# clovaai/assembled-cnn

Measured on NVIDIA H100. Metric: images/sec Assemble-ResNet-50 224^2 bf16 train step, higher is better.
Workload: dtype bf16

## Files before the change

assembled_cnn_b200/csrc/gemm.cu:

```cuda
#include <stdlib.h>

#include <algorithm>

#include "common.h"
#include "ptx.cuh"

namespace acnn {

static void input_pitches(const acnn_conv_geom& g, int64_t* pix, int64_t* row, int64_t* img) {
  *pix = g.x_pix_stride > 0 ? g.x_pix_stride : g.Cin;
  *row = g.x_row_pitch > 0 ? g.x_row_pitch : (int64_t)g.W * *pix;
  *img = g.x_img_pitch > 0 ? g.x_img_pitch : (int64_t)g.H * *row;
}

static bool is_plain(const acnn_conv_geom& g) {
  return g.kh == 1 && g.kw == 1 && g.stride == 1 && g.pad_h_lo == 0 && g.pad_w_lo == 0 &&
         g.pad_h_hi == 0 && g.pad_w_hi == 0 && g.x_pix_stride <= 0 && g.x_row_pitch <= 0 &&
         g.x_img_pitch <= 0;
}

static int make_map_im2col(CUtensorMap* m, const void* base, const acnn_conv_geom& g, int cw,
                           int pixels) {
  int64_t pix, row, img;
  input_pitches(g, &pix, &row, &img);
  cuuint64_t dims[4] = {(cuuint64_t)g.Cin, (cuuint64_t)g.W, (cuuint64_t)g.H, (cuuint64_t)g.B};
  cuuint64_t strides[3] = {(cuuint64_t)pix * 2, (cuuint64_t)row * 2, (cuuint64_t)img * 2};
  int lower[2] = {-g.pad_w_lo, -g.pad_h_lo};
  int upper[2] = {g.pad_w_hi - (g.kw - 1), g.pad_h_hi - (g.kh - 1)};
  cuuint32_t estr[4] = {1, (cuuint32_t)g.stride, (cuuint32_t)g.stride, 1};
  CUresult r = g_encode_im2col(m, CU_TENSOR_MAP_DATA_TYPE_BFLOAT16, 4, const_cast<void*>(base),
                               dims, strides, lower, upper, (cuuint32_t)cw, (cuuint32_t)pixels,
                               estr, CU_TENSOR_MAP_INTERLEAVE_NONE, swizzle_enum(cw * 2),
                               CU_TENSOR_MAP_L2_PROMOTION_L2_128B,
                               CU_TENSOR_MAP_FLOAT_OOB_FILL_NONE);
  if (r != CUDA_SUCCESS) {
    set_error("cuTensorMapEncodeIm2col failed (%d): B=%d H=%d W=%d C=%d k=%dx%d s=%d cw=%d px=%d "
              "pitches=%lld/%lld/%lld", (int)r, g.B, g.H, g.W, g.Cin, g.kh, g.kw, g.stride, cw,
              pixels, (long long)pix, (long long)row, (long long)img);
    return ACNN_ERR_CUDA;
  }
  if (g_driver_version <= 13010 && (int64_t)g.B * img * 2 < 131072) {
    reinterpret_cast<uint64_t*>(m)[1] &= ~(1ull << 21);
  }
  return ACNN_OK;
}

struct ConvGemmParams {
  int M;
  int Cout;
  int Cin;
  int Ktot;
  int kw;
  int HoWo, Wo;
  int stride, pad_h_lo, pad_w_lo;
  int b_sw_bytes;
  int stages;
  int m_tiles, n_tiles;
  void* y;
  float* ch_part;
  const float* bias;
  int has_add, has_mask;
  int out_f32;
};

constexpr int kBM = 128;
constexpr int kStageK = 64;
constexpr int kThreads = 384;
constexpr int kConsumerThreads = 256;
constexpr int kConsumerWarps = 8;
constexpr int kMaxStages = 8;
constexpr int kSmemBudget = 224 * 1024;

__host__ __device__ constexpr int plane_term_a(int t) { return t == 0 ? 2 : ((t == 1 || t == 3) ? 1 : 0); }
__host__ __device__ constexpr int plane_term_b(int t) { return t == 2 ? 2 : ((t == 1 || t == 4) ? 1 : 0); }

static inline int fprop_stage_bytes(int bn, int np) { return np * (kBM * kStageK * 2 + bn * kStageK * 2); }
static inline int fprop_stages(int bn, int np, bool has_add, bool has_mask, bool out_f32) {
  const int half_n = bn > 128 ? 128 : bn;
  const int tile = kBM * half_n * 2;
  const int fixed = 1024 + (out_f32 ? 0 : tile) + (has_add ? tile : 0) + (has_mask ? tile : 0);
  int st = (kSmemBudget - fixed) / fprop_stage_bytes(bn, np);
  if (st > kMaxStages) st = kMaxStages;
  if (st < 2) st = 2;
  return st;
}

template <int BN, int NP = 1>
struct FpropCfg {
  static constexpr int kABytes = kBM * kStageK * 2;
  static constexpr int kBBytes = BN * kStageK * 2;
  static constexpr int kStageBytes = NP * (kABytes + kBBytes);
  static_assert(2 * kStageBytes + 1024 <= kSmemBudget, "two pipeline stages must fit");
  static constexpr int kHalfN = BN > 128 ? 128 : BN;
  static constexpr int kNHalf = BN / kHalfN;
  static constexpr int kSubW = kHalfN < 64 ? kHalfN : 64;
  static constexpr int kTileBytes = kBM * kHalfN * 2;
  static_assert(NP == 1 || BN <= 128, "fp32 mode: N tile <= 128 (registers)");
  static int stages_for(bool has_add, bool has_mask, bool out_f32) {
    return fprop_stages(BN, NP, has_add, has_mask, out_f32);
  }
  static int smem_bytes(int stages, bool has_add, bool has_mask, bool out_f32) {
    return 1024 + stages * kStageBytes + (out_f32 ? 0 : kTileBytes) + (has_add ? kTileBytes : 0) +
           (has_mask ? kTileBytes : 0);
  }
};

template <int kSubW>
__device__ __forceinline__ int staged_offset(int r, int c) {
  constexpr int kRowBytes = kSubW * 2;
  const int sub = c / kSubW, cb = (c % kSubW) * 2;
  const int swz = (kRowBytes == 128) ? (r & 7) : ((r >> 1) & 3);
  return sub * (kBM * kRowBytes) + r * kRowBytes + ((((cb >> 4) ^ swz)) << 4) + (cb & 15);
}

template <int BN, int CW, bool IM2COL, int NP, bool CG2>
__global__ void __launch_bounds__(kThreads, 1)
conv_gemm_kernel(const __grid_constant__ CUtensorMap tmA, const __grid_constant__ CUtensorMap tmB,
                 const __grid_constant__ CUtensorMap tmC, const __grid_constant__ CUtensorMap tmAdd,
                 const __grid_constant__ CUtensorMap tmMask, const __grid_constant__ CUtensorMap tmA1,
                 const __grid_constant__ CUtensorMap tmA2, const __grid_constant__ CUtensorMap tmB1,
                 const __grid_constant__ CUtensorMap tmB2, const ConvGemmParams p) {
  using Cfg = FpropCfg<BN, NP>;
  constexpr int kChunks = kStageK / CW;
  constexpr int kChunkBytes = kBM * CW * 2;
  constexpr int kKSteps = CW / 16;
  constexpr int kHalfN = Cfg::kHalfN;
  constexpr int kNHalf = Cfg::kNHalf;
  constexpr int kSubW = Cfg::kSubW;
  constexpr int kSubBytes = kBM * kSubW * 2;
  constexpr int kNSub = kHalfN / kSubW;

  extern __shared__ uint8_t smem_raw[];
  __shared__ uint64_t full_bar[kMaxStages];
  __shared__ uint64_t empty_bar[kMaxStages];
  __shared__ uint64_t aux_bar;

  uint8_t* smem = reinterpret_cast<uint8_t*>((reinterpret_cast<uintptr_t>(smem_raw) + 1023) &
                                             ~static_cast<uintptr_t>(1023));
  const int kStages = p.stages;
  uint8_t* s_out = smem + kStages * Cfg::kStageBytes;
  uint8_t* s_add = s_out + (p.out_f32 ? 0 : Cfg::kTileBytes);
  uint8_t* s_mask = s_add + (p.has_add ? Cfg::kTileBytes : 0);

  const int warp = threadIdx.x >> 5;
  const int lane = threadIdx.x & 31;
  const int num_kb = (p.Ktot + kStageK - 1) / kStageK;
  constexpr int kTileM = (CG2 ? 2 : 1) * kBM;
  const uint32_t cta_rank = CG2 ? cluster_ctarank() : 0u;
  const int unit = CG2 ? static_cast<int>(blockIdx.x >> 1) : static_cast<int>(blockIdx.x);
  const int units = CG2 ? static_cast<int>(gridDim.x >> 1) : static_cast<int>(gridDim.x);
  const int n_tile = unit % p.n_tiles;
  const int m_first = unit / p.n_tiles;
  const int m_step = units / p.n_tiles;
  const int n0 = n_tile * BN;
  const int my_tiles = m_first < p.m_tiles ? (p.m_tiles - m_first + m_step - 1) / m_step : 0;
  const int m_rank_off = static_cast<int>(cta_rank) * kBM;

  if (warp == 0 && lane == 0) {
    tma_prefetch_desc(&tmA);
    tma_prefetch_desc(&tmB);
    if (NP == 3) {
      tma_prefetch_desc(&tmA1);
      tma_prefetch_desc(&tmA2);
      tma_prefetch_desc(&tmB1);
      tma_prefetch_desc(&tmB2);
    }
    if (!p.out_f32) tma_prefetch_desc(&tmC);
    if (p.has_add) tma_prefetch_desc(&tmAdd);
    if (p.has_mask) tma_prefetch_desc(&tmMask);
    for (int s = 0; s < kStages; ++s) {
      mbar_init(&full_bar[s], 1);
      mbar_init(&empty_bar[s], kConsumerWarps * (CG2 ? 2 : 1));
    }
    mbar_init(&aux_bar, 1);
    fence_barrier_init();
  }
  if (CG2) cluster_sync();
  else __syncthreads();
  pdl_entry();

  const uint32_t smem_a0 = smem_u32(smem);
  const uint32_t full0 = smem_u32(full_bar), empty0 = smem_u32(empty_bar);
  const int tail_chunks = kChunks == 1 ? 1 : ((p.Ktot - (num_kb - 1) * kStageK + CW - 1) / CW);

  if (warp == 0) {
    uint32_t stage = 0, phase = 0;
    const uint32_t b_bytes = BN * (p.b_sw_bytes < 128 ? p.b_sw_bytes : 128);
    const uint32_t full_bytes = NP * (kChunks * kChunkBytes + b_bytes);
    const uint32_t tail_bytes = NP * (tail_chunks * kChunkBytes + b_bytes);
    const int Cin = p.Cin, fkw = p.kw;
    for (int it = 0; it < my_tiles; ++it) {
      const int m0 = (m_first + it * m_step) * kTileM + m_rank_off;
      int img = 0, h0 = 0, w0 = 0;
      if (IM2COL) {
        img = m0 / p.HoWo;
        const int rem = m0 - img * p.HoWo;
        const int po = rem / p.Wo;
        const int qo = rem - po * p.Wo;
        h0 = po * p.stride - p.pad_h_lo;
        w0 = qo * p.stride - p.pad_w_lo;
      }
      int tr = 0, ts = 0, tc = 0, k0 = 0;
      for (int kb = 0; kb < num_kb; ++kb) {
        const bool last = kb == num_kb - 1;
        const int nch = (kChunks > 1 && last) ? tail_chunks : kChunks;
        mbar_wait_a(empty0 + stage * 8, phase ^ 1);
        const bool leader = elect_one();
        const uint32_t fb = full0 + stage * 8;
        const uint32_t sa = smem_a0 + stage * Cfg::kStageBytes;
        if (leader) {
          mbar_expect_tx_a(fb, (kChunks > 1 && last) ? tail_bytes : full_bytes);
          if (CG2) {
            const int half = BN / 2;
            tma_load_2d_multicast(sa + NP * Cfg::kABytes + cta_rank * half * (b_bytes / BN), &tmB,
                                  fb, k0, n0 + static_cast<int>(cta_rank) * half, (uint16_t)3);
          } else {
#pragma unroll
            for (int pl = 0; pl < NP; ++pl)
              tma_load_2d_a(sa + NP * Cfg::kABytes + pl * Cfg::kBBytes,
                            pl == 0 ? &tmB : (pl == 1 ? &tmB1 : &tmB2), fb, k0, n0);
          }
        }
#pragma unroll
        for (int j = 0; j < kChunks; ++j) {
          if (j < nch) {
            if (leader) {
#pragma unroll
              for (int pl = 0; pl < NP; ++pl) {
                const CUtensorMap* mA = pl == 0 ? &tmA : (pl == 1 ? &tmA1 : &tmA2);
                const uint32_t dst = sa + pl * Cfg::kABytes + j * kChunkBytes;
                if (IM2COL)
                  tma_load_im2col_4d_a(dst, mA, fb, tc, w0, h0, img, (uint16_t)ts, (uint16_t)tr);
                else
                  tma_load_2d_a(dst, mA, fb, k0 + j * CW, m0);
              }
            }
            tc += CW;
            if (tc >= Cin) {
              tc = 0;
              if (++ts == fkw) { ts = 0; ++tr; }
            }
          }
        }
        __syncwarp();
        k0 += kStageK;
        if (++stage == static_cast<uint32_t>(kStages)) { stage = 0; phase ^= 1; }
      }
    }
  } else if (warp >= 4) {
    const int cg = (warp >> 2) - 1;
    const int ct = static_cast<int>(threadIdx.x) - 128;
    const bool leader = ct == 0;
    const bool stats = p.ch_part != nullptr;
    const bool has_aux = p.has_add || p.has_mask;
    const int r0 = cg * 64 + (warp & 3) * 16 + (lane >> 2);
    const int cq = (lane & 3) * 2;
    const uint64_t a_desc0 = make_smem_desc(smem_a0 + cg * 64 * CW * 2, 16, 8 * CW * 2,
                                            swizzle_layout_type(CW * 2));
    const uint64_t b_desc0 = make_smem_desc(smem_a0 + NP * Cfg::kABytes, 16, 8 * p.b_sw_bytes,
                                            swizzle_layout_type(p.b_sw_bytes));
    float acc[BN / 2];
    float acc2[NP == 3 ? BN / 2 : 1];
    constexpr int kNChunk = kHalfN / 8;
    constexpr int kStatThreads = (BN == 32) ? 128 : kConsumerThreads;
    constexpr int kNRg = kStatThreads / kNChunk;
    const bool st_on = ct < kStatThreads;
    const int st_chunk = ct % kNChunk, st_rg = ct / kNChunk;
    float acc_s[kNHalf][8], acc_q[kNHalf][8];
#pragma unroll
    for (int hf = 0; hf < kNHalf; ++hf)
#pragma unroll
      for (int e = 0; e < 8; ++e) acc_s[hf][e] = acc_q[hf][e] = 0.f;
    uint32_t aux_n = 0;
    auto issue_aux = [&](int am0, int anh) {
      mbar_expect_tx(&aux_bar, (p.has_add ? Cfg::kTileBytes : 0) +
                                   (p.has_mask ? Cfg::kTileBytes : 0));
#pragma unroll
      for (int sub = 0; sub < kNSub; ++sub) {
        if (p.has_add)
          tma_load_2d(s_add + sub * kSubBytes, &tmAdd, &aux_bar, anh + sub * kSubW, am0);
        if (p.has_mask)
          tma_load_2d(s_mask + sub * kSubBytes, &tmMask, &aux_bar, anh + sub * kSubW, am0);
      }
    };
    if (leader && has_aux && my_tiles > 0) issue_aux(m_first * kTileM + m_rank_off, n0);
    const uint32_t empty_peer = CG2 ? mapa_shared(empty0, cta_rank ^ 1u) : 0u;
    auto release = [&](int st) {
      if (CG2) {
        mbar_arrive_cluster(mapa_shared(empty0, cta_rank) + st * 8);
        mbar_arrive_cluster(empty_peer + st * 8);
      } else {
        mbar_arrive(&empty_bar[st]);
      }
    };

    uint32_t stage = 0, phase = 0;
    for (int it = 0; it < my_tiles; ++it) {
      const int m0 = (m_first + it * m_step) * kTileM + m_rank_off;
      int prev = -1;
      for (int kb = 0; kb < num_kb; ++kb) {
        const bool last = kb == num_kb - 1;
        const int nch = (kChunks > 1 && last) ? tail_chunks : kChunks;
        mbar_wait_a(full0 + stage * 8, phase);
        wgmma_fence_operand(acc);
        if (NP == 3) wgmma_fence_operand(acc2);
        wgmma_fence();
        const uint64_t da0 = a_desc0 + ((stage * Cfg::kStageBytes) >> 4);
        const uint64_t db0 = b_desc0 + ((stage * Cfg::kStageBytes) >> 4);
#pragma unroll
        for (int j = 0; j < kChunks; ++j) {
          if (j < nch) {
#pragma unroll
            for (int ks = 0; ks < kKSteps; ++ks) {
#pragma unroll
              for (int t = 0; t < (NP == 3 ? 6 : 1); ++t) {
                const int pa = NP == 3 ? plane_term_a(t) : 0;
                const int pb = NP == 3 ? plane_term_b(t) : 0;
                const bool small = NP == 3 && t < 5;
                const uint64_t da = da0 + ((pa * Cfg::kABytes + j * kChunkBytes + ks * 32) >> 4);
                const uint64_t db = db0 + ((pb * Cfg::kBBytes + (j * kKSteps + ks) * 32) >> 4);
                const uint32_t accum = (j | ks | (small ? t : 0)) ? 1u : static_cast<uint32_t>(kb != 0);
                if constexpr (NP == 3) {
                  if (small) Wgmma<BN>::template mma<0, 0>(acc2, da, db, accum);
                  else Wgmma<BN>::template mma<0, 0>(acc, da, db, accum);
                } else {
                  Wgmma<BN>::template mma<0, 0>(acc, da, db, accum);
                }
              }
            }
          }
        }
        wgmma_commit();
        wgmma_fence_operand(acc);
        if (NP == 3) wgmma_fence_operand(acc2);
        wgmma_wait<1>();
        __syncwarp();
        if (prev >= 0 && lane == 0) release(prev);
        prev = static_cast<int>(stage);
        if (++stage == static_cast<uint32_t>(kStages)) { stage = 0; phase ^= 1; }
      }
      wgmma_wait<0>();
      wgmma_fence_operand(acc);
      if (NP == 3) {
        wgmma_fence_operand(acc2);
#pragma unroll
        for (int i = 0; i < BN / 2; ++i) acc[i] += acc2[i];
      }
      __syncwarp();
      if (lane == 0) release(prev);

#pragma unroll
      for (int hf = 0; hf < kNHalf; ++hf) {
        const int nh = n0 + hf * kHalfN;
        if (leader && !p.out_f32) tma_store_wait_read();
        named_bar_sync(1, kConsumerThreads);
        if (has_aux) {
          mbar_wait(&aux_bar, aux_n & 1);
          ++aux_n;
        }
#pragma unroll
        for (int jj = 0; jj < kHalfN / 8; ++jj) {
          const int j = hf * (kHalfN / 8) + jj;
          const int c = jj * 8 + cq;
          float b0 = 0.f, b1 = 0.f;
          if (p.bias) {
            b0 = __ldg(p.bias + nh + c);
            b1 = __ldg(p.bias + nh + c + 1);
          }
#pragma unroll
          for (int h = 0; h < 2; ++h) {
            const int r = r0 + h * 8;
            float v0 = acc[j * 4 + h * 2] + b0, v1 = acc[j * 4 + h * 2 + 1] + b1;
            const int off = staged_offset<kSubW>(r, c);
            if (p.has_add) bf16x2_add(v0, v1, *reinterpret_cast<const uint32_t*>(s_add + off));
            if (p.out_f32) {
              if (p.has_mask) {
                const uint32_t k2 = bf16x2_gt0_mask(*reinterpret_cast<const uint32_t*>(s_mask + off));
                if (!(k2 & 0xffffu)) v0 = 0.f;
                if (!(k2 >> 16)) v1 = 0.f;
              }
              if (m0 + r < p.M)
                *reinterpret_cast<float2*>(reinterpret_cast<float*>(p.y) +
                                           static_cast<size_t>(m0 + r) * p.Cout + nh + c) =
                    make_float2(v0, v1);
            } else {
              uint32_t pk = pack_bf16x2(v0, v1);
              if (p.has_mask) pk &= bf16x2_gt0_mask(*reinterpret_cast<const uint32_t*>(s_mask + off));
              *reinterpret_cast<uint32_t*>(s_out + off) = pk;
            }
          }
        }
        if (!p.out_f32) fence_proxy_async();
        named_bar_sync(1, kConsumerThreads);
        if (leader) {
          if (!p.out_f32) {
#pragma unroll
            for (int sub = 0; sub < kNSub; ++sub)
              tma_store_2d(&tmC, s_out + sub * kSubBytes, nh + sub * kSubW, m0);
            tma_store_commit();
          }
          if (has_aux) {
            if (hf + 1 < kNHalf) issue_aux(m0, nh + kHalfN);
            else if (it + 1 < my_tiles) issue_aux((m_first + (it + 1) * m_step) * kTileM + m_rank_off, n0);
          }
        }
        if (stats && st_on) {
          constexpr int kRowBytes = kSubW * 2;
          const int sub = st_chunk / (kSubW / 8), jj = st_chunk % (kSubW / 8);
#pragma unroll 4
          for (int i = 0; i < kBM / kNRg; ++i) {
            const int rr = st_rg + i * kNRg;
            const int sw = (kRowBytes == 128) ? (rr & 7) : ((rr >> 1) & 3);
            const uint4 u = *reinterpret_cast<const uint4*>(s_out + sub * kSubBytes +
                                                            rr * kRowBytes + ((jj ^ sw) << 4));
            const uint32_t w4[4] = {u.x, u.y, u.z, u.w};
#pragma unroll
            for (int e = 0; e < 4; ++e)
              bf16x2_sum_sq(acc_s[hf][2 * e], acc_q[hf][2 * e], acc_s[hf][2 * e + 1],
                            acc_q[hf][2 * e + 1], w4[e]);
          }
        }
      }
    }
    if (leader && !p.out_f32) tma_store_wait_all();
    if (stats && my_tiles > 0) {
      float* red_sum = reinterpret_cast<float*>(s_out);
      float* red_sq = red_sum + kNRg * BN;
      static_assert(2 * kNRg * BN * 4 <= Cfg::kTileBytes, "staging buffer too small for stats");
      named_bar_sync(1, kConsumerThreads);
      if (st_on) {
#pragma unroll
        for (int hf = 0; hf < kNHalf; ++hf)
#pragma unroll
          for (int e = 0; e < 8; ++e) {
            red_sum[st_rg * BN + hf * kHalfN + st_chunk * 8 + e] = acc_s[hf][e];
            red_sq[st_rg * BN + hf * kHalfN + st_chunk * 8 + e] = acc_q[hf][e];
          }
      }
      named_bar_sync(1, kConsumerThreads);
      for (int col = ct; col < BN; col += kConsumerThreads) {
        float ss = 0.f, qq = 0.f;
        for (int g2 = 0; g2 < kNRg; ++g2) {
          ss += red_sum[g2 * BN + col];
          qq += red_sq[g2 * BN + col];
        }
        float* row = p.ch_part +
                     static_cast<size_t>(CG2 ? m_first * 2 + static_cast<int>(cta_rank) : m_first) * 2 *
                         p.Cout;
        row[n0 + col] = ss;
        row[p.Cout + n0 + col] = qq;
      }
    }
  }
  if (CG2) cluster_sync();
}

constexpr int kHaloH = 18, kHaloW = 10, kPatchH = 16, kPatchW = 8;
constexpr int kHaloMaxB = 32;

struct HaloParams {
  int H, W, B;
  int Cin, Cout;
  int n_tiles, ph, pw;
  int m_tiles;
  int a_stages, b_slots, stationary;
  float* ch_part;
  int has_add, has_mask;
};

template <int BN, int CW>
struct HaloCfg {
  static constexpr int kRowB = CW * 2;
  static constexpr int kABytes = kHaloH * kHaloW * kRowB;
  static constexpr int kAStage = (kABytes + 1023) / 1024 * 1024;
  static constexpr int kBTile = BN * kRowB;
  static constexpr int kSubW = BN < 64 ? BN : 64;
  static constexpr int kTileBytes = kBM * BN * 2;
  static_assert(BN <= 128 && kBTile % 512 == 0, "halo kernel: N tile <= 128");
};

struct PatchIter {
  int img, row, col;
  int d_img, d_row, d_col;
  int ph, pw;
  __device__ __forceinline__ PatchIter(int first, int step, int ph_, int pw_) : ph(ph_), pw(pw_) {
    const int tpi = ph * pw;
    img = first / tpi;
    int rem = first - img * tpi;
    row = rem / pw;
    col = rem - row * pw;
    d_img = step / tpi;
    rem = step - d_img * tpi;
    d_row = rem / pw;
    d_col = rem - d_row * pw;
  }
  __device__ __forceinline__ void next() {
    col += d_col;
    if (col >= pw) { col -= pw; ++row; }
    row += d_row;
    if (row >= ph) { row -= ph; ++img; }
    img += d_img;
  }
};

template <int BN, int CW>
__global__ void __launch_bounds__(kThreads, 1)
conv_halo_kernel(const __grid_constant__ CUtensorMap tmA, const __grid_constant__ CUtensorMap tmB,
                 const __grid_constant__ CUtensorMap tmC, const __grid_constant__ CUtensorMap tmAdd,
                 const __grid_constant__ CUtensorMap tmMask, const HaloParams p) {
  using Cfg = HaloCfg<BN, CW>;
  constexpr int kRowB = Cfg::kRowB;
  constexpr int kKSteps = CW / 16;
  constexpr uint32_t kLayout = swizzle_layout_type(kRowB);
  constexpr int kSubW = Cfg::kSubW;
  constexpr int kSubBytes = kBM * kSubW * 2;
  constexpr int kNSub = BN / kSubW;

  extern __shared__ uint8_t smem_raw[];
  __shared__ uint64_t a_full[4], a_empty[4];
  __shared__ uint64_t b_full[kHaloMaxB], b_empty[kHaloMaxB];
  __shared__ uint64_t aux_bar;

  uint8_t* smem = reinterpret_cast<uint8_t*>((reinterpret_cast<uintptr_t>(smem_raw) + 1023) &
                                             ~static_cast<uintptr_t>(1023));
  const int AS = p.a_stages, NB = p.b_slots;
  uint8_t* s_out = smem + AS * Cfg::kAStage + NB * Cfg::kBTile;
  uint8_t* s_add = s_out + Cfg::kTileBytes;
  uint8_t* s_mask = s_add + (p.has_add ? Cfg::kTileBytes : 0);

  const int warp = threadIdx.x >> 5;
  const int lane = threadIdx.x & 31;
  const int nchunks = p.Cin / CW;
  const int n_tile = blockIdx.x % p.n_tiles;
  const int m_first = blockIdx.x / p.n_tiles;
  const int m_step = gridDim.x / p.n_tiles;
  const int n0 = n_tile * BN;
  const int my_tiles = m_first < p.m_tiles ? (p.m_tiles - m_first + m_step - 1) / m_step : 0;
  const int tpi = p.ph * p.pw;

  if (warp == 0 && lane == 0) {
    tma_prefetch_desc(&tmA);
    tma_prefetch_desc(&tmB);
    tma_prefetch_desc(&tmC);
    if (p.has_add) tma_prefetch_desc(&tmAdd);
    if (p.has_mask) tma_prefetch_desc(&tmMask);
    for (int s = 0; s < AS; ++s) {
      mbar_init(&a_full[s], 1);
      mbar_init(&a_empty[s], kConsumerWarps);
    }
    for (int s = 0; s < NB; ++s) {
      mbar_init(&b_full[s], 1);
      mbar_init(&b_empty[s], kConsumerWarps);
    }
    mbar_init(&aux_bar, 1);
    fence_barrier_init();
  }
  __syncthreads();
  pdl_entry();
  const uint32_t a_base = smem_u32(smem), b_base = a_base + AS * Cfg::kAStage;
  const uint32_t afull0 = smem_u32(a_full), bfull0 = smem_u32(b_full);

  if (warp == 0) {
    const uint32_t aempty0 = smem_u32(a_empty), bempty0 = smem_u32(b_empty);
    uint32_t sa = 0, a_ph = 0, sb = 0, b_ph = 0;
    if (p.stationary && my_tiles > 0) {
      if (elect_one()) {
        mbar_expect_tx_a(bfull0, static_cast<uint32_t>(nchunks) * 9 * Cfg::kBTile);
        for (int kc = 0; kc < nchunks; ++kc)
          for (int t = 0; t < 9; ++t)
            tma_load_2d_a(b_base + (kc * 9 + t) * Cfg::kBTile, &tmB, bfull0, t * p.Cin + kc * CW, n0);
      }
      __syncwarp();
    }
    for (int it = 0; it < my_tiles; ++it) {
      const int tile = m_first + it * m_step;
      const int img = tile / tpi;
      const int rem = tile - img * tpi;
      const int h0 = (rem / p.pw) * kPatchH, w0 = (rem % p.pw) * kPatchW;
      for (int kc = 0; kc < nchunks; ++kc) {
        mbar_wait_a(aempty0 + sa * 8, a_ph ^ 1);
        if (elect_one()) {
          mbar_expect_tx_a(afull0 + sa * 8, Cfg::kABytes);
          tma_load_4d_tile_a(a_base + sa * Cfg::kAStage, &tmA, afull0 + sa * 8, kc * CW, w0 - 1,
                             h0 - 1, img);
        }
        __syncwarp();
        if (++sa == static_cast<uint32_t>(AS)) { sa = 0; a_ph ^= 1; }
        if (!p.stationary) {
          for (int t = 0; t < 9; ++t) {
            mbar_wait_a(bempty0 + sb * 8, b_ph ^ 1);
            if (elect_one()) {
              mbar_expect_tx_a(bfull0 + sb * 8, Cfg::kBTile);
              tma_load_2d_a(b_base + sb * Cfg::kBTile, &tmB, bfull0 + sb * 8, t * p.Cin + kc * CW,
                            n0);
            }
            __syncwarp();
            if (++sb == static_cast<uint32_t>(NB)) { sb = 0; b_ph ^= 1; }
          }
        }
      }
    }
  } else if (warp >= 4) {
    const int cg = (warp >> 2) - 1;
    const int ct = static_cast<int>(threadIdx.x) - 128;
    const bool leader = ct == 0;
    const bool stats = p.ch_part != nullptr;
    const bool has_aux = p.has_add || p.has_mask;
    const int r0 = cg * 64 + (warp & 3) * 16 + (lane >> 2);
    const int cq = (lane & 3) * 2;
    const uint64_t a_desc0 = make_smem_desc(a_base + cg * 8 * kHaloW * kRowB, 16, kHaloW * kRowB, kLayout);
    const uint64_t b_desc0 = make_smem_desc(b_base, 16, 8 * kRowB, kLayout);
    float acc[BN / 2];
    constexpr int kNChunk = BN / 8;
    constexpr int kStatThreads = (BN == 32) ? 128 : kConsumerThreads;
    constexpr int kNRg = kStatThreads / kNChunk;
    const bool st_on = ct < kStatThreads;
    const int st_chunk = ct % kNChunk, st_rg = ct / kNChunk;
    float acc_s[8], acc_q[8];
#pragma unroll
    for (int e = 0; e < 8; ++e) acc_s[e] = acc_q[e] = 0.f;
    uint32_t aux_n = 0;
    auto issue_aux = [&](int img, int h0, int w0) {
      mbar_expect_tx(&aux_bar, (p.has_add ? Cfg::kTileBytes : 0) + (p.has_mask ? Cfg::kTileBytes : 0));
#pragma unroll
      for (int sub = 0; sub < kNSub; ++sub) {
        if (p.has_add)
          tma_load_4d_tile_a(smem_u32(s_add + sub * kSubBytes), &tmAdd, smem_u32(&aux_bar),
                             n0 + sub * kSubW, w0, h0, img);
        if (p.has_mask)
          tma_load_4d_tile_a(smem_u32(s_mask + sub * kSubBytes), &tmMask, smem_u32(&aux_bar),
                             n0 + sub * kSubW, w0, h0, img);
      }
    };
    int pend_a = -1, pend_b = -1;
    auto release_pending = [&]() {
      __syncwarp();
      if (lane == 0) {
        if (pend_a >= 0) mbar_arrive(&a_empty[pend_a]);
        if (pend_b >= 0) mbar_arrive(&b_empty[pend_b]);
      }
      pend_a = pend_b = -1;
    };
    PatchIter pi(m_first, m_step, p.ph, p.pw);
    if (leader && has_aux && my_tiles > 0) issue_aux(pi.img, pi.row * kPatchH, pi.col * kPatchW);
    if (p.stationary && my_tiles > 0) mbar_wait_a(bfull0, 0);
    uint32_t sa = 0, a_ph = 0, sb = 0, b_ph = 0;
    for (int it = 0; it < my_tiles; ++it) {
      const int img = pi.img, h0 = pi.row * kPatchH, w0 = pi.col * kPatchW;
      pi.next();
      for (int kc = 0; kc < nchunks; ++kc) {
        mbar_wait_a(afull0 + sa * 8, a_ph);
        const uint64_t a_st = a_desc0 + ((sa * Cfg::kAStage) >> 4);
        if (p.stationary) {
          wgmma_fence_operand(acc);
          wgmma_fence();
          const uint64_t b_st = b_desc0 + ((static_cast<uint32_t>(kc) * 9 * Cfg::kBTile) >> 4);
#pragma unroll
          for (int t = 0; t < 9; ++t)
#pragma unroll
            for (int ks = 0; ks < kKSteps; ++ks)
              Wgmma<BN>::template mma<0, 0>(
                  acc, a_st + ((((t / 3) * kHaloW + (t % 3)) * kRowB + ks * 32) >> 4),
                  b_st + ((t * Cfg::kBTile + ks * 32) >> 4), (t | ks) ? 1u : static_cast<uint32_t>(kc != 0));
          wgmma_commit();
          wgmma_fence_operand(acc);
          wgmma_wait<1>();
          release_pending();
          pend_a = static_cast<int>(sa);
        } else {
#pragma unroll 1
          for (int t = 0; t < 9; ++t) {
            mbar_wait_a(bfull0 + sb * 8, b_ph);
            wgmma_fence_operand(acc);
            wgmma_fence();
            const uint64_t a_tap = a_st + ((((t / 3) * kHaloW + (t % 3)) * kRowB) >> 4);
            const uint64_t b_tap = b_desc0 + ((sb * Cfg::kBTile) >> 4);
#pragma unroll
            for (int ks = 0; ks < kKSteps; ++ks)
              Wgmma<BN>::template mma<0, 0>(acc, a_tap + ((ks * 32) >> 4), b_tap + ((ks * 32) >> 4),
                                            (kc | t | ks) ? 1u : 0u);
            wgmma_commit();
            wgmma_fence_operand(acc);
            wgmma_wait<1>();
            release_pending();
            pend_b = static_cast<int>(sb);
            if (t == 8) pend_a = static_cast<int>(sa);
            if (++sb == static_cast<uint32_t>(NB)) { sb = 0; b_ph ^= 1; }
          }
        }
        if (++sa == static_cast<uint32_t>(AS)) { sa = 0; a_ph ^= 1; }
      }
      wgmma_wait<0>();
      wgmma_fence_operand(acc);
      release_pending();

      if (leader) tma_store_wait_read();
      named_bar_sync(1, kConsumerThreads);
      if (has_aux) {
        mbar_wait(&aux_bar, aux_n & 1);
        ++aux_n;
      }
#pragma unroll
      for (int j = 0; j < BN / 8; ++j) {
        const int c = j * 8 + cq;
#pragma unroll
        for (int h = 0; h < 2; ++h) {
          const int r = r0 + h * 8;
          float v0 = acc[j * 4 + h * 2], v1 = acc[j * 4 + h * 2 + 1];
          const int off = staged_offset<kSubW>(r, c);
          if (p.has_add) bf16x2_add(v0, v1, *reinterpret_cast<const uint32_t*>(s_add + off));
          uint32_t pk = pack_bf16x2(v0, v1);
          if (p.has_mask) pk &= bf16x2_gt0_mask(*reinterpret_cast<const uint32_t*>(s_mask + off));
          *reinterpret_cast<uint32_t*>(s_out + off) = pk;
        }
      }
      fence_proxy_async();
      named_bar_sync(1, kConsumerThreads);
      if (leader) {
#pragma unroll
        for (int sub = 0; sub < kNSub; ++sub)
          tma_store_4d(&tmC, s_out + sub * kSubBytes, n0 + sub * kSubW, w0, h0, img);
        tma_store_commit();
        if (has_aux && it + 1 < my_tiles) issue_aux(pi.img, pi.row * kPatchH, pi.col * kPatchW);
      }
      if (stats && st_on) {
        constexpr int kRowBytes = kSubW * 2;
        const int sub = st_chunk / (kSubW / 8), jj = st_chunk % (kSubW / 8);
#pragma unroll 4
        for (int rr = st_rg; rr < kBM; rr += kNRg) {
          if (h0 + (rr >> 3) >= p.H || w0 + (rr & 7) >= p.W) continue;
          const int sw = (kRowBytes == 128) ? (rr & 7) : ((rr >> 1) & 3);
          const uint4 u = *reinterpret_cast<const uint4*>(s_out + sub * kSubBytes + rr * kRowBytes +
                                                          ((jj ^ sw) << 4));
          const uint32_t w4[4] = {u.x, u.y, u.z, u.w};
#pragma unroll
          for (int e = 0; e < 4; ++e)
            bf16x2_sum_sq(acc_s[2 * e], acc_q[2 * e], acc_s[2 * e + 1], acc_q[2 * e + 1], w4[e]);
        }
      }
    }
    if (leader) tma_store_wait_all();
    if (stats && my_tiles > 0) {
      float* red_sum = reinterpret_cast<float*>(s_out);
      float* red_sq = red_sum + kNRg * BN;
      static_assert(2 * kNRg * BN * 4 <= Cfg::kTileBytes, "staging buffer too small for stats");
      named_bar_sync(1, kConsumerThreads);
      if (st_on) {
#pragma unroll
        for (int e = 0; e < 8; ++e) {
          red_sum[st_rg * BN + st_chunk * 8 + e] = acc_s[e];
          red_sq[st_rg * BN + st_chunk * 8 + e] = acc_q[e];
        }
      }
      named_bar_sync(1, kConsumerThreads);
      for (int col = ct; col < BN; col += kConsumerThreads) {
        float ss = 0.f, qq = 0.f;
        for (int g2 = 0; g2 < kNRg; ++g2) {
          ss += red_sum[g2 * BN + col];
          qq += red_sq[g2 * BN + col];
        }
        float* row = p.ch_part + static_cast<size_t>(m_first) * 2 * p.Cout;
        row[n0 + col] = ss;
        row[p.Cout + n0 + col] = qq;
      }
    }
  }
}

struct WgradParams {
  int P;
  int Cout;
  int Cin;
  int Ktot;
  int kw;
  int HoWo, Wo;
  int stride, pad_h_lo, pad_w_lo;
  int pix;
  int stages_total;
  int stages_per_split;
  int splits;
  float* dw;
  float* part;
};

constexpr int kWgPix = 64;

template <int BN, int NP = 1, int PIX = kWgPix>
struct WgradCfg {
  static constexpr int kABytes = PIX * 128 * 2;
  static constexpr int kBBytes = PIX * BN * 2;
  static constexpr int kStageBytes = NP * (kABytes + kBBytes);
  static constexpr int kStagesFit = (kSmemBudget - 1024) / kStageBytes;
  static constexpr int kStages =
      PIX != kWgPix ? (kStagesFit > 4 ? 4 : kStagesFit)
      : NP == 3 ? (kStagesFit > 3 ? 3 : kStagesFit)
              : ((BN >= 256) ? 4 : ((BN == 128) ? 3 : 4));
  static constexpr int kSmemBytes = kStages * kStageBytes + 1024;
  static_assert((NP == 1 || BN <= 128) && kStages >= (NP == 3 ? 2 : 3), "wgrad tile does not fit");
};

template <int BN, int CW, int CWB, bool IM2COL, int NP, int PIX>
__global__ void __launch_bounds__(kThreads, 1)
wgrad_gemm_kernel(const __grid_constant__ CUtensorMap tmX, const __grid_constant__ CUtensorMap tmDY,
                  const __grid_constant__ CUtensorMap tmX1, const __grid_constant__ CUtensorMap tmX2,
                  const __grid_constant__ CUtensorMap tmDY1,
                  const __grid_constant__ CUtensorMap tmDY2, const WgradParams p) {
  using Cfg = WgradCfg<BN, NP, PIX>;
  constexpr int kStages = Cfg::kStages;
  constexpr int kAChunks = 128 / CW;
  constexpr int kAChunkBytes = PIX * CW * 2;
  constexpr int kBChunkBytes = PIX * CWB * 2;

  extern __shared__ uint8_t smem_raw[];
  __shared__ uint64_t full_bar[kStages];
  __shared__ uint64_t empty_bar[kStages];

  uint8_t* smem = reinterpret_cast<uint8_t*>((reinterpret_cast<uintptr_t>(smem_raw) + 1023) &
                                             ~static_cast<uintptr_t>(1023));
  const int warp = threadIdx.x >> 5;
  const int lane = threadIdx.x & 31;
  const int m0 = blockIdx.x * 128;
  const int co0 = blockIdx.y * BN;
  const int ks_begin = blockIdx.z * p.stages_per_split;
  int ks_end = ks_begin + p.stages_per_split;
  if (ks_end > p.stages_total) ks_end = p.stages_total;
  const int num_ks = ks_end - ks_begin;

  int a_chunks = 0;
#pragma unroll
  for (int j = 0; j < kAChunks; ++j) a_chunks += (m0 + j * CW < p.Ktot) ? 1 : 0;
  const int b_chunks = (p.Cout - co0 < BN ? p.Cout - co0 : BN) / CWB;

  if (warp == 0 && lane == 0) {
    tma_prefetch_desc(&tmDY);
    tma_prefetch_desc(&tmX);
    for (int s = 0; s < kStages; ++s) {
      mbar_init(&full_bar[s], 1);
      mbar_init(&empty_bar[s], kConsumerWarps);
    }
    fence_barrier_init();
  }
  __syncthreads();
  pdl_entry();

  if (warp == 0) {
    int stage = 0;
    uint32_t phase = 0;
    int ch_r[kAChunks], ch_s[kAChunks], ch_c[kAChunks];
#pragma unroll
    for (int j = 0; j < kAChunks; ++j) {
      const int n = m0 + j * CW;
      const int tap = n / p.Cin;
      ch_c[j] = n - tap * p.Cin;
      ch_r[j] = tap / p.kw;
      ch_s[j] = tap - ch_r[j] * p.kw;
    }
    for (int it = 0; it < num_ks; ++it) {
      const int p0 = (ks_begin + it) * PIX;
      mbar_wait(&empty_bar[stage], phase ^ 1);
      if (elect_one()) {
        uint8_t* sa = smem + stage * Cfg::kStageBytes;
        uint8_t* sb = sa + NP * Cfg::kABytes;
        mbar_expect_tx(&full_bar[stage], NP * (a_chunks * kAChunkBytes + b_chunks * kBChunkBytes));
        int img = 0, h0 = 0, w0 = 0;
        if (IM2COL) {
          img = p0 / p.HoWo;
          const int rem = p0 - img * p.HoWo;
          const int po = rem / p.Wo;
          const int qo = rem - po * p.Wo;
          h0 = po * p.stride - p.pad_h_lo;
          w0 = qo * p.stride - p.pad_w_lo;
        }
#pragma unroll
        for (int pl = 0; pl < NP; ++pl) {
          const CUtensorMap* mX = pl == 0 ? &tmX : (pl == 1 ? &tmX1 : &tmX2);
          const CUtensorMap* mDY = pl == 0 ? &tmDY : (pl == 1 ? &tmDY1 : &tmDY2);
#pragma unroll
          for (int j = 0; j < kAChunks; ++j) {
            if (j < a_chunks) {
              uint8_t* dst = sa + pl * Cfg::kABytes + j * kAChunkBytes;
              if (IM2COL) {
                tma_load_im2col_4d(dst, mX, &full_bar[stage], ch_c[j], w0, h0, img,
                                   (uint16_t)ch_s[j], (uint16_t)ch_r[j]);
              } else {
                tma_load_2d(dst, mX, &full_bar[stage], ch_c[j], p0);
              }
            }
          }
          for (int i = 0; i < b_chunks; ++i)
            tma_load_2d(sb + pl * Cfg::kBBytes + i * kBChunkBytes, mDY, &full_bar[stage],
                        co0 + i * CWB, p0);
        }
      }
      __syncwarp();
      if (++stage == kStages) { stage = 0; phase ^= 1; }
    }
  } else if (warp >= 4) {
    const int cg = (warp >> 2) - 1;
    const uint32_t sbase = smem_u32(smem);
    const uint64_t a_desc0 = make_smem_desc(sbase + (cg * 64 / CW) * kAChunkBytes, kAChunkBytes,
                                            8 * CW * 2, swizzle_layout_type(CW * 2));
    const uint64_t b_desc0 = make_smem_desc(sbase + NP * Cfg::kABytes, kBChunkBytes, 8 * CWB * 2,
                                            swizzle_layout_type(CWB * 2));
    float acc[BN / 2];
    float acc2[NP == 3 ? BN / 2 : 1];
    int stage = 0, prev = -1;
    uint32_t phase = 0;
    for (int it = 0; it < num_ks; ++it) {
      mbar_wait(&full_bar[stage], phase);
      wgmma_fence_operand(acc);
      if (NP == 3) wgmma_fence_operand(acc2);
      wgmma_fence();
      const uint64_t da0 = a_desc0 + static_cast<uint64_t>(stage * (Cfg::kStageBytes >> 4));
      const uint64_t db0 = b_desc0 + static_cast<uint64_t>(stage * (Cfg::kStageBytes >> 4));
#pragma unroll
      for (int ks = 0; ks < PIX / 16; ++ks) {
#pragma unroll
        for (int t = 0; t < (NP == 3 ? 6 : 1); ++t) {
          const int pa = NP == 3 ? plane_term_a(t) : 0;
          const int pb = NP == 3 ? plane_term_b(t) : 0;
          const bool small = NP == 3 && t < 5;
          const uint64_t da = da0 + ((pa * Cfg::kABytes + ks * 16 * CW * 2) >> 4);
          const uint64_t db = db0 + ((pb * Cfg::kBBytes + ks * 16 * CWB * 2) >> 4);
          const uint32_t accum = (it | ks | (small ? t : 0)) ? 1u : 0u;
          if constexpr (NP == 3) {
            if (small) Wgmma<BN>::template mma<1, 1>(acc2, da, db, accum);
            else Wgmma<BN>::template mma<1, 1>(acc, da, db, accum);
          } else {
            Wgmma<BN>::template mma<1, 1>(acc, da, db, accum);
          }
        }
      }
      wgmma_commit();
      wgmma_fence_operand(acc);
      if (NP == 3) wgmma_fence_operand(acc2);
      wgmma_wait<1>();
      __syncwarp();
      if (prev >= 0 && lane == 0) mbar_arrive(&empty_bar[prev]);
      prev = stage;
      if (++stage == kStages) { stage = 0; phase ^= 1; }
    }
    wgmma_wait<0>();
    wgmma_fence_operand(acc);
    if (NP == 3) {
      wgmma_fence_operand(acc2);
#pragma unroll
      for (int i = 0; i < BN / 2; ++i) acc[i] += acc2[i];
    }
    const int rl = cg * 64 + (warp & 3) * 16 + (lane >> 2);
    const int rb = m0 + rl;
    const int cq = (lane & 3) * 2;
    float* part = p.part ? p.part + static_cast<size_t>(blockIdx.z) * p.Cout * p.Ktot : nullptr;
#pragma unroll
    for (int j = 0; j < BN / 8; ++j) {
#pragma unroll
      for (int h = 0; h < 2; ++h) {
        const int n = rb + h * 8;
#pragma unroll
        for (int e = 0; e < 2; ++e) {
          const int co = co0 + j * 8 + cq + e;
          if (n < p.Ktot && co < p.Cout) {
            const size_t i = static_cast<size_t>(co) * p.Ktot + n;
            if (part) part[i] = acc[j * 4 + h * 2 + e];
            else atomicAdd(p.dw + i, acc[j * 4 + h * 2 + e]);
          }
        }
      }
    }
  }
}

constexpr int kWgRedThreads = 128;
constexpr int kWgRedDepth = 16;

__global__ void __launch_bounds__(kWgRedThreads)
wgrad_reduce_kernel(const float* __restrict__ part, float* dw, int64_t n, int splits) {
  pdl_entry();
  const int64_t i = blockIdx.x * static_cast<int64_t>(kWgRedThreads) + threadIdx.x;
  if (i >= n) return;
  const float* src = part + i;
  float t = 0.f;
  int s = 0;
  for (; s + kWgRedDepth <= splits; s += kWgRedDepth) {
    float v[kWgRedDepth];
#pragma unroll
    for (int u = 0; u < kWgRedDepth; ++u) v[u] = __ldcs(src + (s + u) * n);
#pragma unroll
    for (int u = 0; u < kWgRedDepth; ++u) t += v[u];
  }
  for (; s < splits; ++s) t += __ldcs(src + s * n);
  dw[i] += t;
}

struct ConvMaps {
  CUtensorMap a[3], b[3], c, add, mask;
};

static int g_conv_out_bufs = 1;
static int g_conv_split_epi = 1;
static int g_conv_split_mt2 = 1;
static int g_conv_mtiles_mode = -1;
static int g_conv_pairs = 0;

template <int BN, int CW, bool IM2COL, int NP, bool CG2 = false>
static int launch_conv_gemm(const ConvMaps& tm, const ConvGemmParams& p, int per_n,
                            cudaStream_t stream) {
  using Cfg = FpropCfg<BN, NP>;
  static bool attr_set = false;
  auto kern = conv_gemm_kernel<BN, CW, IM2COL, NP, CG2>;
  if (!attr_set) {
    cudaError_t e = cudaFuncSetAttribute(kern, cudaFuncAttributeMaxDynamicSharedMemorySize,
                                         kSmemBudget + 2048);
    if (e != cudaSuccess) {
      set_error("cudaFuncSetAttribute(conv_gemm): %s", cudaGetErrorString(e));
      return ACNN_ERR_CUDA;
    }
    attr_set = true;
  }
  ConvGemmParams q = p;
  q.stages = Cfg::stages_for(p.has_add, p.has_mask, p.out_f32);
  q.m_tiles = ceil_div(p.M, (CG2 ? 2 : 1) * kBM);
  q.n_tiles = p.Cout / BN;
  const int smem = Cfg::smem_bytes(q.stages, p.has_add, p.has_mask, p.out_f32);
  if (CG2) {
    cudaLaunchConfig_t cfg{};
    cfg.gridDim = dim3(2 * per_n * q.n_tiles);
    cfg.blockDim = dim3(kThreads);
    cfg.dynamicSmemBytes = smem;
    cfg.stream = stream;
    cudaLaunchAttribute at[1];
    at[0].id = cudaLaunchAttributeClusterDimension;
    at[0].val.clusterDim.x = 2;
    at[0].val.clusterDim.y = 1;
    at[0].val.clusterDim.z = 1;
    cfg.attrs = at;
    cfg.numAttrs = 1;
    (void)cudaLaunchKernelEx(&cfg, kern, tm.a[0], tm.b[0], tm.c, tm.add, tm.mask, tm.a[1], tm.a[2],
                             tm.b[1], tm.b[2], q);
  } else {
    launch_k(kern, dim3(per_n * q.n_tiles), dim3(kThreads), smem, stream, tm.a[0], tm.b[0], tm.c,
             tm.add, tm.mask, tm.a[1], tm.a[2], tm.b[1], tm.b[2], q);
  }
  count_launch();
  return check_launch("conv_gemm_kernel");
}

struct ConvTiling {
  int bn;
  int per_n;
  int pair;
  int parts;
};

static ConvTiling conv_tiling(int M, int Cout, int Ktot, int cw, bool has_add, bool has_mask,
                              bool out_f32, int np) {
  (void)has_add;
  (void)has_mask;
  ConvTiling t;
  t.bn = (Cout % 128 == 0) ? 128 : ((Cout % 64 == 0) ? 64 : 32);
  const int n_tiles = Cout / t.bn;
  t.pair = (g_conv_pairs && t.bn == 128 && np == 1 && !out_f32 && cw == 64 && Ktot >= 512 &&
            (int64_t)ceil_div(M, 2 * kBM) * n_tiles >= num_sms() / 2) ? 1 : 0;
  const int m_tiles = ceil_div(M, (t.pair ? 2 : 1) * kBM);
  t.per_n = (t.pair ? num_sms() / 2 : num_sms()) / n_tiles;
  if (t.per_n < 1) t.per_n = 1;
  if (t.per_n > m_tiles) t.per_n = m_tiles;
  t.parts = t.pair ? 2 * t.per_n : t.per_n;
  return t;
}

template <int BN, int NP>
static int dispatch_conv_cw(int cw, bool im2col, const ConvMaps& tm, const ConvGemmParams& p,
                            int per_n, cudaStream_t s) {
  if (im2col) {
    if (cw == 64) return launch_conv_gemm<BN, 64, true, NP>(tm, p, per_n, s);
    if (cw == 32) return launch_conv_gemm<BN, 32, true, NP>(tm, p, per_n, s);
    return launch_conv_gemm<BN, 16, true, NP>(tm, p, per_n, s);
  }
  if (cw == 64) return launch_conv_gemm<BN, 64, false, NP>(tm, p, per_n, s);
  if (cw == 32) return launch_conv_gemm<BN, 32, false, NP>(tm, p, per_n, s);
  return launch_conv_gemm<BN, 16, false, NP>(tm, p, per_n, s);
}

template <int BN>
static int dispatch_conv_gemm(const ConvTiling& t, int np, int cw, bool im2col, const ConvMaps& tm,
                              const ConvGemmParams& p, cudaStream_t s) {
  if constexpr (BN == 128) {
    if (t.pair) {
      if (im2col) return launch_conv_gemm<128, 64, true, 1, true>(tm, p, t.per_n, s);
      return launch_conv_gemm<128, 64, false, 1, true>(tm, p, t.per_n, s);
    }
  }
  if constexpr (BN <= 128) {
    if (np == 3) return dispatch_conv_cw<BN, 3>(cw, im2col, tm, p, t.per_n, s);
  }
  return dispatch_conv_cw<BN, 1>(cw, im2col, tm, p, t.per_n, s);
}

static int chunk_width(int cin) { return cin % 64 == 0 ? 64 : (cin % 32 == 0 ? 32 : 16); }

static int out_hw(const acnn_conv_geom& g, int* Ho, int* Wo) {
  *Ho = (g.H + g.pad_h_lo + g.pad_h_hi - g.kh) / g.stride + 1;
  *Wo = (g.W + g.pad_w_lo + g.pad_w_hi - g.kw) / g.stride + 1;
  return (*Ho > 0 && *Wo > 0) ? 1 : 0;
}

static int64_t input_elems(const acnn_conv_geom& g) {
  int64_t pix, row, img;
  input_pitches(g, &pix, &row, &img);
  return (int64_t)g.B * img;
}

static int g_conv_halo = 1;

static int halo_bn(int Cout) { return Cout % 128 == 0 ? 128 : (Cout % 64 == 0 ? 64 : 32); }

struct HaloPlan {
  int a_stages, b_slots, stationary, smem;
};
static int g_conv_halo_split = 1;

static HaloPlan halo_plan(int bn, int cw, int Cin, bool has_add, bool has_mask) {
  HaloPlan h;
  const int row_b = cw * 2;
  const int a_stage = (kHaloH * kHaloW * row_b + 1023) / 1024 * 1024;
  const int b_tile = bn * row_b;
  const int tile = kBM * bn * 2;
  const int nchunks = Cin / cw;
  const int fixed = 1024 + tile * (1 + (has_add ? 1 : 0) + (has_mask ? 1 : 0));
  h.a_stages = 3;
  h.b_slots = (kSmemBudget - fixed - h.a_stages * a_stage) / b_tile;
  if (h.b_slots < nchunks * 9) {
    const int b2 = (kSmemBudget - fixed - 2 * a_stage) / b_tile;
    if (b2 >= nchunks * 9 || h.b_slots < 3) {
      h.a_stages = 2;
      h.b_slots = b2;
    }
  }
  if (h.b_slots > kHaloMaxB) h.b_slots = kHaloMaxB;
  h.stationary = (h.b_slots >= 2 && nchunks * 9 <= h.b_slots) ? 1 : 0;
  if (h.stationary) h.b_slots = nchunks * 9;
  h.smem = fixed + h.a_stages * a_stage + h.b_slots * b_tile;
  return h;
}

static bool use_halo(const acnn_conv_geom& g, int np, bool out_f32, bool has_bias, bool has_add,
                     bool has_mask) {
  if (g_conv_halo <= 0) return false;
  const bool applies = g.kh == 3 && g.kw == 3 && g.stride == 1 && g.pad_h_lo == 1 &&
                       g.pad_h_hi == 1 && g.pad_w_lo == 1 && g.pad_w_hi == 1 &&
                       g.x_pix_stride <= 0 && g.x_row_pitch <= 0 && g.x_img_pitch <= 0 && np == 1 &&
                       !out_f32 && !has_bias && (g.Cin % 64 == 0 || g.Cin == 32) &&
                       g.Cout % 32 == 0;
  if (!applies) return false;
  if (g_conv_halo >= 2) return true;
  const HaloPlan h = halo_plan(halo_bn(g.Cout), g.Cin % 64 == 0 ? 64 : 32, g.Cin, has_add, has_mask);
  return h.stationary && g.H >= 56;
}

static int halo_per_n(const acnn_conv_geom& g) {
  const int n_tiles = g.Cout / halo_bn(g.Cout);
  const int m_tiles = g.B * ceil_div(g.H, kPatchH) * ceil_div(g.W, kPatchW);
  int per_n = num_sms() / n_tiles;
  if (per_n < 1) per_n = 1;
  return per_n > m_tiles ? m_tiles : per_n;
}

static int make_map_4d(CUtensorMap* m, const void* base, int C, int W, int H, int B, int box_c,
                       int box_w, int box_h) {
  cuuint64_t dims[4] = {(cuuint64_t)C, (cuuint64_t)W, (cuuint64_t)H, (cuuint64_t)B};
  cuuint64_t strides[3] = {(cuuint64_t)C * 2, (cuuint64_t)W * C * 2, (cuuint64_t)H * W * C * 2};
  cuuint32_t box[4] = {(cuuint32_t)box_c, (cuuint32_t)box_w, (cuuint32_t)box_h, 1};
  cuuint32_t estr[4] = {1, 1, 1, 1};
  CUresult r = g_encode_tiled(m, CU_TENSOR_MAP_DATA_TYPE_BFLOAT16, 4, const_cast<void*>(base), dims,
                              strides, box, estr, CU_TENSOR_MAP_INTERLEAVE_NONE,
                              swizzle_enum(box_c * 2), CU_TENSOR_MAP_L2_PROMOTION_L2_128B,
                              CU_TENSOR_MAP_FLOAT_OOB_FILL_NONE);
  if (r != CUDA_SUCCESS) {
    set_error("cuTensorMapEncodeTiled (4-d) failed (%d): C=%d W=%d H=%d B=%d box=%dx%dx%d", (int)r,
              C, W, H, B, box_c, box_w, box_h);
    return ACNN_ERR_CUDA;
  }
  return ACNN_OK;
}

template <int BN, int CW>
static int launch_conv_halo(const acnn_conv_geom& g, const void* x, const void* w, void* y,
                            float* ch_part, const void* add_src, const void* mask_src,
                            cudaStream_t stream) {
  using Cfg = HaloCfg<BN, CW>;
  static bool attr_set = false;
  auto kern = conv_halo_kernel<BN, CW>;
  if (!attr_set) {
    cudaError_t e = cudaFuncSetAttribute(kern, cudaFuncAttributeMaxDynamicSharedMemorySize,
                                         kSmemBudget + 2048);
    if (e != cudaSuccess) {
      set_error("cudaFuncSetAttribute(conv_halo): %s", cudaGetErrorString(e));
      return ACNN_ERR_CUDA;
    }
    attr_set = true;
  }
  HaloParams p;
  p.H = g.H; p.W = g.W; p.B = g.B; p.Cin = g.Cin; p.Cout = g.Cout;
  p.n_tiles = g.Cout / BN;
  p.ph = ceil_div(g.H, kPatchH);
  p.pw = ceil_div(g.W, kPatchW);
  p.m_tiles = g.B * p.ph * p.pw;
  p.ch_part = ch_part;
  p.has_add = add_src != nullptr;
  p.has_mask = mask_src != nullptr;
  const HaloPlan hp = halo_plan(BN, CW, g.Cin, p.has_add != 0, p.has_mask != 0);
  p.a_stages = hp.a_stages;
  p.b_slots = hp.b_slots;
  p.stationary = hp.stationary;
  ACNN_REQUIRE(p.b_slots >= 2, "conv (halo): shared memory does not fit");
  const int smem = hp.smem;
  CUtensorMap tmA, tmB, tmC, tmAdd, tmMask;
  int rc = make_map_4d(&tmA, x, g.Cin, g.W, g.H, g.B, CW, kHaloW, kHaloH);
  if (rc) return rc;
  if ((rc = make_map_2d(&tmB, w, g.Cout, 9 * g.Cin, 9 * g.Cin, BN, CW))) return rc;
  if ((rc = make_map_4d(&tmC, y, g.Cout, g.W, g.H, g.B, Cfg::kSubW, kPatchW, kPatchH))) return rc;
  tmAdd = tmMask = tmC;
  if (add_src && (rc = make_map_4d(&tmAdd, add_src, g.Cout, g.W, g.H, g.B, Cfg::kSubW, kPatchW,
                                   kPatchH)))
    return rc;
  if (mask_src && (rc = make_map_4d(&tmMask, mask_src, g.Cout, g.W, g.H, g.B, Cfg::kSubW, kPatchW,
                                    kPatchH)))
    return rc;
  launch_k(kern, dim3(halo_per_n(g) * p.n_tiles), dim3(kThreads), smem, stream, tmA, tmB, tmC,
           tmAdd, tmMask, p);
  count_launch();
  return check_launch("conv_halo_kernel");
}

static int conv_halo_host(const acnn_conv_geom& g, const void* x, const void* w, void* y,
                          float* ch_part, const void* add_src, const void* mask_src,
                          cudaStream_t stream) {
  const int bn = halo_bn(g.Cout);
  const bool c64 = g.Cin % 64 == 0;
  if (bn == 128) {
    return c64 ? launch_conv_halo<128, 64>(g, x, w, y, ch_part, add_src, mask_src, stream)
               : launch_conv_halo<128, 32>(g, x, w, y, ch_part, add_src, mask_src, stream);
  }
  if (bn == 64) {
    return c64 ? launch_conv_halo<64, 64>(g, x, w, y, ch_part, add_src, mask_src, stream)
               : launch_conv_halo<64, 32>(g, x, w, y, ch_part, add_src, mask_src, stream);
  }
  return c64 ? launch_conv_halo<32, 64>(g, x, w, y, ch_part, add_src, mask_src, stream)
             : launch_conv_halo<32, 32>(g, x, w, y, ch_part, add_src, mask_src, stream);
}

static int conv_gemm_host(const acnn_conv_geom& g, const void* x, const void* w, void* y,
                          float* ch_part, const void* add_src, const void* mask_src,
                          const float* bias, int out_f32, int precision, int64_t w_plane_stride,
                          cudaStream_t stream) {
  ACNN_REQUIRE(g.B > 0 && g.H > 0 && g.W > 0 && g.Cin > 0 && g.Cout > 0, "conv: empty geometry");
  ACNN_REQUIRE(g.Cin % 16 == 0, "conv: Cin=%d must be a multiple of 16", g.Cin);
  ACNN_REQUIRE(g.Cout % 32 == 0, "conv: Cout=%d must be a multiple of 32", g.Cout);
  ACNN_REQUIRE(g.stride >= 1 && g.kh >= 1 && g.kw >= 1, "conv: bad kernel/stride");
  ACNN_REQUIRE(!(ch_part && out_f32), "conv: statistics only with bf16 output");
  ACNN_REQUIRE(precision == 0 || precision == 1, "conv: precision must be 0 (bf16) or 1 (fp32)");
  ACNN_REQUIRE(precision == 0 || (out_f32 && !add_src && !mask_src && !ch_part && w_plane_stride > 0),
               "conv: the fp32 (3-plane) mode needs fp32 output, a weight plane stride and no "
               "fused add / mask / statistics epilogue");
  int Ho, Wo;
  ACNN_REQUIRE(out_hw(g, &Ho, &Wo), "conv: empty output");
  ACNN_REQUIRE(g.pad_h_lo <= 128 && g.pad_w_lo <= 128 && g.kh <= 128 && g.kw <= 128,
               "conv: padding / filter exceed the TMA im2col corner range");
  int rc = load_driver_fns();
  if (rc) return rc;
  if (use_halo(g, precision ? 3 : 1, out_f32 != 0, bias != nullptr, add_src != nullptr,
               mask_src != nullptr))
    return conv_halo_host(g, x, w, y, ch_part, add_src, mask_src, stream);
  const bool plain = is_plain(g);
  const int cw = chunk_width(g.Cin);
  const int np = precision ? 3 : 1;
  ConvGemmParams p;
  p.M = g.B * Ho * Wo;
  p.Cout = g.Cout;
  p.Cin = g.Cin;
  p.Ktot = g.kh * g.kw * g.Cin;
  p.kw = g.kw;
  p.HoWo = Ho * Wo;
  p.Wo = Wo;
  p.stride = g.stride;
  p.pad_h_lo = g.pad_h_lo;
  p.pad_w_lo = g.pad_w_lo;
  p.b_sw_bytes = p.Ktot >= 64 ? 128 : p.Ktot * 2;
  p.y = y;
  p.ch_part = ch_part;
  p.bias = bias;
  p.has_add = add_src != nullptr;
  p.has_mask = mask_src != nullptr;
  p.out_f32 = out_f32;
  p.stages = p.m_tiles = p.n_tiles = 0;
  ACNN_REQUIRE(p.b_sw_bytes == 128 || p.b_sw_bytes == 64 || p.b_sw_bytes == 32,
               "conv: unsupported K=%d", p.Ktot);

  const ConvTiling t =
      conv_tiling(p.M, g.Cout, p.Ktot, cw, p.has_add, p.has_mask, out_f32 != 0, np);
  const int bn = t.bn;
  ConvMaps tm;
  const int64_t x_plane = input_elems(g);
  for (int pl = 0; pl < np; ++pl) {
    const __nv_bfloat16* xp = static_cast<const __nv_bfloat16*>(x) + pl * x_plane;
    const __nv_bfloat16* wp = static_cast<const __nv_bfloat16*>(w) + pl * w_plane_stride;
    if (plain) {
      rc = make_map_2d(&tm.a[pl], xp, p.M, g.Cin, g.Cin, kBM, cw);
    } else {
      rc = make_map_im2col(&tm.a[pl], xp, g, cw, kBM);
    }
    if (rc) return rc;
    rc = make_map_2d(&tm.b[pl], wp, g.Cout, p.Ktot, p.Ktot, t.pair ? bn / 2 : bn,
                     p.Ktot >= 64 ? 64 : p.Ktot);
    if (rc) return rc;
  }
  for (int pl = np; pl < 3; ++pl) {
    tm.a[pl] = tm.a[0];
    tm.b[pl] = tm.b[0];
  }
  tm.c = tm.add = tm.mask = tm.b[0];
  const int subw = bn < 64 ? bn : 64;
  if (!out_f32 && (rc = make_map_2d(&tm.c, y, p.M, g.Cout, g.Cout, kBM, subw))) return rc;
  if (add_src && (rc = make_map_2d(&tm.add, add_src, p.M, g.Cout, g.Cout, kBM, subw))) return rc;
  if (mask_src && (rc = make_map_2d(&tm.mask, mask_src, p.M, g.Cout, g.Cout, kBM, subw))) return rc;
  if (bn == 128) return dispatch_conv_gemm<128>(t, np, cw, !plain, tm, p, stream);
  if (bn == 64) return dispatch_conv_gemm<64>(t, np, cw, !plain, tm, p, stream);
  return dispatch_conv_gemm<32>(t, np, cw, !plain, tm, p, stream);
}

struct WgradMaps {
  CUtensorMap x[3], dy[3];
};

static int g_wgrad_overhead_stages = 16;

constexpr size_t kWgPartFloats = size_t(16) << 20;

static int g_wgrad_splits = 0;

static int g_wgrad_pix = 0;
static bool wgrad_wants_pix128(int) {
  return true;
}

struct WgradPlan {
  int P;
  int bn;
  int n_tiles, m_tiles;
  int pix;
  int stages_total;
  int splits;
  int stages_per_split;
};

static int wgrad_plan(const acnn_conv_geom& g, int precision, int deterministic, WgradPlan* w) {
  ACNN_REQUIRE(g.Cin % 16 == 0 && g.Cout % 32 == 0, "wgrad: Cin %% 16 / Cout %% 32 required");
  ACNN_REQUIRE(precision == 0 || precision == 1, "wgrad: precision must be 0 (bf16) or 1 (fp32)");
  int Ho, Wo;
  ACNN_REQUIRE(out_hw(g, &Ho, &Wo), "wgrad: empty output");
  const int np = precision ? 3 : 1;
  w->P = g.B * Ho * Wo;
  int bn = g.Cout >= 256 ? 256 : (g.Cout >= 128 ? 128 : (g.Cout >= 64 ? 64 : 32));
  if (np == 3 && bn > 128) bn = 128;
  ACNN_REQUIRE(g.Cout % bn == 0, "wgrad: Cout=%d not a multiple of its N tile %d", g.Cout, bn);
  w->bn = bn;
  w->n_tiles = g.Cout / bn;
  w->m_tiles = ceil_div(g.kh * g.kw * g.Cin, 128);
  w->pix = kWgPix;
  if (np == 1 && bn <= 128 && w->P >= 4096 &&
      (g_wgrad_pix == 128 || (g_wgrad_pix == 0 && wgrad_wants_pix128(bn))))
    w->pix = 128;
  w->stages_total = ceil_div(w->P, w->pix);
  const int tiles = w->m_tiles * w->n_tiles;
  const int64_t tile_floats = (int64_t)tiles * 128 * bn;
  int cap = (int)std::min<int64_t>(w->stages_total, (int64_t)kWgPartFloats / tile_floats);
  if (cap < 1) cap = 1;
  const int max_splits = std::min(cap, w->stages_total >= 8 ? w->stages_total / 4 : 1);
  int splits;
  if (g_wgrad_splits > 0) {
    splits = std::min(g_wgrad_splits, cap);
  } else if (g_wgrad_overhead_stages <= 0) {
    splits = std::min(ceil_div(2 * num_sms(), tiles), max_splits);
  } else {
    splits = 1;
    int64_t best = -1;
    for (int s = 1; s <= max_splits; ++s) {
      const int per = ceil_div(w->stages_total, s);
      const int s_eff = ceil_div(w->stages_total, per);
      if (s_eff != s) continue;
      const int per_sm = ceil_div(tiles * s, num_sms());
      const int64_t t = (int64_t)per_sm * per + (int64_t)per_sm * g_wgrad_overhead_stages;
      if (best < 0 || t < best) { best = t; splits = s; }
    }
  }
  if (splits < 1 || deterministic) splits = 1;
  w->stages_per_split = ceil_div(w->stages_total, splits);
  w->splits = ceil_div(w->stages_total, w->stages_per_split);
  return ACNN_OK;
}

template <int BN, int CW, int CWB, bool IM2COL, int NP, int PIX = kWgPix>
static int launch_wgrad(const WgradMaps& tm, WgradParams p, int m_tiles, int n_tiles,
                        cudaStream_t stream) {
  using Cfg = WgradCfg<BN, NP, PIX>;
  static bool attr_set = false;
  auto kern = wgrad_gemm_kernel<BN, CW, CWB, IM2COL, NP, PIX>;
  if (!attr_set) {
    cudaError_t e = cudaFuncSetAttribute(kern, cudaFuncAttributeMaxDynamicSharedMemorySize,
                                         Cfg::kSmemBytes);
    if (e != cudaSuccess) {
      set_error("cudaFuncSetAttribute(wgrad): %s", cudaGetErrorString(e));
      return ACNN_ERR_CUDA;
    }
    attr_set = true;
  }
  const int splits = p.splits;
  const int64_t n = (int64_t)p.Cout * p.Ktot;
  p.part = nullptr;
  if (splits > 1) {
    void* scratch = nullptr;
    int rc = scratch_alloc(&scratch, (size_t)splits * n * sizeof(float), stream, "wgrad");
    if (rc) return rc;
    p.part = static_cast<float*>(scratch);
  }
  dim3 grid(m_tiles, n_tiles, splits);
  launch_k(kern, dim3(grid), dim3(kThreads), Cfg::kSmemBytes, stream, tm.x[0], tm.dy[0], tm.x[1],
           tm.x[2], tm.dy[1], tm.dy[2], p);
  count_launch();
  int rc = check_launch("wgrad_gemm_kernel");
  if (!p.part) return rc;
  if (rc == ACNN_OK) {
    launch_k(wgrad_reduce_kernel, dim3((unsigned)ceil_div64(n, kWgRedThreads)), dim3(kWgRedThreads),
             0, stream, static_cast<const float*>(p.part), p.dw, n, splits);
    count_launch();
    rc = check_launch("wgrad_reduce_kernel");
  }
  const int rc2 = scratch_free(p.part, stream, "wgrad");
  return rc ? rc : rc2;
}

template <int BN, int CW, bool IM2COL>
static int dispatch_wgrad_cwb(int cwb, int np, const WgradMaps& tm, const WgradParams& p, int mt,
                              int nt, cudaStream_t s) {
  if constexpr (BN <= 128) {
    if (np == 3) {
      if constexpr (BN >= 64) {
        if (cwb == 64) return launch_wgrad<BN, CW, 64, IM2COL, 3>(tm, p, mt, nt, s);
      }
      return launch_wgrad<BN, CW, 32, IM2COL, 3>(tm, p, mt, nt, s);
    }
  }
  if constexpr (BN >= 64) {
    if (cwb == 64) {
      if constexpr (BN <= 128) {
        if (p.pix == 128) return launch_wgrad<BN, CW, 64, IM2COL, 1, 128>(tm, p, mt, nt, s);
      }
      return launch_wgrad<BN, CW, 64, IM2COL, 1>(tm, p, mt, nt, s);
    }
  }
  if constexpr (BN <= 128) {
    if (p.pix == 128) return launch_wgrad<BN, CW, 32, IM2COL, 1, 128>(tm, p, mt, nt, s);
  }
  return launch_wgrad<BN, CW, 32, IM2COL, 1>(tm, p, mt, nt, s);
}

template <int BN, bool IM2COL>
static int dispatch_wgrad_cw(int cw, int cwb, int np, const WgradMaps& tm, const WgradParams& p,
                             int mt, int nt, cudaStream_t s) {
  if (cw == 64) return dispatch_wgrad_cwb<BN, 64, IM2COL>(cwb, np, tm, p, mt, nt, s);
  if (cw == 32) return dispatch_wgrad_cwb<BN, 32, IM2COL>(cwb, np, tm, p, mt, nt, s);
  return dispatch_wgrad_cwb<BN, 16, IM2COL>(cwb, np, tm, p, mt, nt, s);
}

template <bool IM2COL>
static int dispatch_wgrad(int bn, int cw, int cwb, int np, const WgradMaps& tm, const WgradParams& p,
                          int mt, int nt, cudaStream_t s) {
  if (bn == 256) return dispatch_wgrad_cw<256, IM2COL>(cw, cwb, np, tm, p, mt, nt, s);
  if (bn == 128) return dispatch_wgrad_cw<128, IM2COL>(cw, cwb, np, tm, p, mt, nt, s);
  if (bn == 64) return dispatch_wgrad_cw<64, IM2COL>(cw, cwb, np, tm, p, mt, nt, s);
  return dispatch_wgrad_cw<32, IM2COL>(cw, cwb, np, tm, p, mt, nt, s);
}

static int conv_wgrad_host(const acnn_conv_geom& g, const void* x, const void* dy, float* dw,
                           int precision, int deterministic, cudaStream_t stream) {
  WgradPlan w;
  int rc = wgrad_plan(g, precision, deterministic, &w);
  if (rc) return rc;
  rc = load_driver_fns();
  if (rc) return rc;
  int Ho, Wo;
  out_hw(g, &Ho, &Wo);
  const bool plain = is_plain(g);
  const int np = precision ? 3 : 1;
  WgradParams p;
  p.P = w.P;
  p.Cout = g.Cout;
  p.Cin = g.Cin;
  p.Ktot = g.kh * g.kw * g.Cin;
  p.kw = g.kw;
  p.HoWo = Ho * Wo;
  p.Wo = Wo;
  p.stride = g.stride;
  p.pad_h_lo = g.pad_h_lo;
  p.pad_w_lo = g.pad_w_lo;
  p.pix = w.pix;
  p.stages_total = w.stages_total;
  p.stages_per_split = w.stages_per_split;
  p.splits = w.splits;
  p.dw = dw;
  const int cw = chunk_width(g.Cin);
  const int cwb = (g.Cout % 64 == 0) ? 64 : 32;
  WgradMaps tm;
  const int64_t x_plane = input_elems(g), dy_plane = (int64_t)p.P * g.Cout;
  for (int pl = 0; pl < np; ++pl) {
    const __nv_bfloat16* xp = static_cast<const __nv_bfloat16*>(x) + pl * x_plane;
    const __nv_bfloat16* dp = static_cast<const __nv_bfloat16*>(dy) + pl * dy_plane;
    rc = make_map_2d(&tm.dy[pl], dp, p.P, g.Cout, g.Cout, p.pix, cwb);
    if (rc) return rc;
    if (plain) {
      rc = make_map_2d(&tm.x[pl], xp, p.P, g.Cin, g.Cin, p.pix, cw);
    } else {
      rc = make_map_im2col(&tm.x[pl], xp, g, cw, p.pix);
    }
    if (rc) return rc;
  }
  for (int pl = np; pl < 3; ++pl) {
    tm.x[pl] = tm.x[0];
    tm.dy[pl] = tm.dy[0];
  }
  if (plain) return dispatch_wgrad<false>(w.bn, cw, cwb, np, tm, p, w.m_tiles, w.n_tiles, stream);
  return dispatch_wgrad<true>(w.bn, cw, cwb, np, tm, p, w.m_tiles, w.n_tiles, stream);
}

}

extern "C" {

int acnn_set_conv_mtiles(int mode) {
  const int prev = acnn::g_conv_mtiles_mode;
  acnn::g_conv_mtiles_mode = (mode == 1 || mode == 2) ? mode : -1;
  return prev;
}

int acnn_set_conv_halo(int mode) {
  const int prev = acnn::g_conv_halo;
  acnn::g_conv_halo = mode < 0 ? 0 : (mode > 2 ? 2 : mode);
  return prev;
}

int acnn_set_conv_split_epilogue(int mode) {
  const int prev = acnn::g_conv_split_epi;
  acnn::g_conv_split_epi = mode < 0 ? 0 : (mode > 2 ? 2 : mode);
  return prev;
}

int acnn_set_conv_split_mt2(int mode) {
  const int prev = acnn::g_conv_split_mt2;
  acnn::g_conv_split_mt2 = mode < 0 ? 0 : (mode > 2 ? 2 : mode);
  return prev;
}

int acnn_set_conv_halo_split(int on) {
  const int prev = acnn::g_conv_halo_split;
  acnn::g_conv_halo_split = on ? 1 : 0;
  return prev;
}

int acnn_set_conv_out_bufs(int mode) {
  const int prev = acnn::g_conv_out_bufs;
  acnn::g_conv_out_bufs = mode < 0 ? 0 : (mode > 2 ? 2 : mode);
  return prev;
}

int acnn_set_wgrad_overhead_stages(int stages) {
  const int prev = acnn::g_wgrad_overhead_stages;
  acnn::g_wgrad_overhead_stages = stages < 0 ? 0 : stages;
  return prev;
}

int acnn_set_wgrad_pixels(int pix) {
  const int prev = acnn::g_wgrad_pix;
  acnn::g_wgrad_pix = (pix == 64 || pix == 128) ? pix : 0;
  return prev;
}

int acnn_set_wgrad_splits(int n) {
  const int prev = acnn::g_wgrad_splits;
  acnn::g_wgrad_splits = n < 0 ? 0 : n;
  return prev;
}

int acnn_conv_wgrad_plan(const acnn_conv_geom* g, int precision, int deterministic, int* pix,
                         int* splits, int* stages_per_split) {
  if (!g) {
    acnn::set_error("acnn_conv_wgrad_plan: null geometry");
    return ACNN_ERR_INVALID;
  }
  acnn::WgradPlan w;
  const int rc = acnn::wgrad_plan(*g, precision, deterministic, &w);
  if (rc) return rc;
  if (pix) *pix = w.pix;
  if (splits) *splits = w.splits;
  if (stages_per_split) *stages_per_split = w.stages_per_split;
  return ACNN_OK;
}

int acnn_conv_stats_parts(const acnn_conv_geom* g) {
  if (!g) return 0;
  int Ho, Wo;
  if (!acnn::out_hw(*g, &Ho, &Wo) || g->Cout % 32 != 0) return 0;
  if (acnn::use_halo(*g, 1, false, false, false, false)) return acnn::halo_per_n(*g);
  return acnn::conv_tiling(g->B * Ho * Wo, g->Cout, g->kh * g->kw * g->Cin,
                           acnn::chunk_width(g->Cin), false, false, false, 1).parts;
}

int acnn_set_conv_cta_pairs(int on) {
  const int prev = acnn::g_conv_pairs;
  acnn::g_conv_pairs = on ? 1 : 0;
  return prev;
}

int acnn_conv_fprop(const acnn_conv_geom* g, const void* x, const void* w, void* y,
                    float* ch_part, const void* add_src, const void* mask_src, const float* bias,
                    int out_f32, int precision, int64_t w_plane_stride, void* stream) {
  if (!g || !x || !w || !y) {
    acnn::set_error("acnn_conv_fprop: null argument");
    return ACNN_ERR_INVALID;
  }
  return acnn::conv_gemm_host(*g, x, w, y, ch_part, add_src, mask_src, bias, out_f32, precision,
                              w_plane_stride, static_cast<cudaStream_t>(stream));
}

int acnn_conv_dgrad(const acnn_conv_geom* g, const void* dy, const void* w_dgrad, void* dx,
                    const void* add_src, const void* mask_src, int precision,
                    int64_t w_plane_stride, void* stream) {
  if (!g || !dy || !w_dgrad || !dx) {
    acnn::set_error("acnn_conv_dgrad: null argument");
    return ACNN_ERR_INVALID;
  }
  if (g->stride != 1) {
    acnn::set_error("acnn_conv_dgrad: stride %d (zero-insert dy first, then call with stride 1)",
                    g->stride);
    return ACNN_ERR_UNSUPPORTED;
  }
  const int Ho = g->H + g->pad_h_lo + g->pad_h_hi - g->kh + 1;
  const int Wo = g->W + g->pad_w_lo + g->pad_w_hi - g->kw + 1;
  acnn_conv_geom t;
  t.B = g->B;
  t.H = Ho;
  t.W = Wo;
  t.Cin = g->Cout;
  t.Cout = g->Cin;
  t.kh = g->kh;
  t.kw = g->kw;
  t.stride = 1;
  t.pad_h_lo = g->kh - 1 - g->pad_h_lo;
  t.pad_h_hi = g->kh - 1 - g->pad_h_hi;
  t.pad_w_lo = g->kw - 1 - g->pad_w_lo;
  t.pad_w_hi = g->kw - 1 - g->pad_w_hi;
  t.x_pix_stride = t.x_row_pitch = t.x_img_pitch = t.reserved_ = 0;
  return acnn::conv_gemm_host(t, dy, w_dgrad, dx, nullptr, add_src, mask_src, nullptr,
                              precision ? 1 : 0, precision, w_plane_stride,
                              static_cast<cudaStream_t>(stream));
}

int acnn_conv_wgrad(const acnn_conv_geom* g, const void* x, const void* dy, float* dw,
                    int precision, int deterministic, void* stream) {
  if (!g || !x || !dy || !dw) {
    acnn::set_error("acnn_conv_wgrad: null argument");
    return ACNN_ERR_INVALID;
  }
  return acnn::conv_wgrad_host(*g, x, dy, dw, precision, deterministic,
                               static_cast<cudaStream_t>(stream));
}

}
```

assembled_cnn_b200/csrc/model_plan.cu:

```cuda
#include "model_plan.h"

#include <math.h>
#include <stdarg.h>
#include <stdio.h>

#include <algorithm>

#include "common.h"

namespace acnn {
namespace model {

namespace {

struct PlanError {
  int code;
  std::string msg;
};

[[noreturn]] void fail(int code, const char* fmt, ...) {
  char buf[512];
  va_list ap;
  va_start(ap, fmt);
  vsnprintf(buf, sizeof(buf), fmt, ap);
// ... 99 lines not shown
    Variable v;
    v.name = name;
    v.kind = kind;
    v.tf_shape = tf_shape;
    v.store_shape = store_shape;
    v.size = numel(store_shape);
    for (const auto& o : p_.vars) PLAN_ASSERT(o.name != name, "duplicate variable %s", name.c_str());
    if (trainable) {
      v.buffer = ACNN_BUF_PARAMS;
      v.offset = p_.param_elems;
      v.decay = decay;
      v.zero_init = zero_init;
      p_.param_elems += round_up(v.size);
      if (need_dgrad) {
        v.dgrad_off = p_.dgrad_elems;
        p_.dgrad_elems += round_up(v.size);
      }
    } else {
      v.buffer = ACNN_BUF_STATE;
      v.offset = p_.state_elems;
      p_.state_elems += round_up(v.size);
    }
    p_.vars.push_back(v);
    return (int)p_.vars.size() - 1;
  }

  Slot slot(int buf, int64_t size) {
    Slot s;
    s.buf = buf;
    s.size = size;
    int64_t& top = buf == BUF_ZERO ? p_.zero_elems : p_.work_elems;
    s.offset = top;
    top += round_up(size, 32);
    return s;
  }

  void emit(const char* kind, std::initializer_list<KV> a) {
    Op op;
    op.kind = kind;
    for (const auto& kv : a) op.a.emplace_back(kv.first, kv.second);
    ops_->push_back(std::move(op));
  }

  int planes(int t) {
    if (!fp32_) return -1;
    auto it = planes_.find(t);
    if (it != planes_.end()) return it->second;
    Shape s{3};
    s.insert(s.end(), T(t).shape.begin(), T(t).shape.end());
    const int64_t n = numel(T(t).shape);
    const int pt = tensor("planes", s, ACNN_BF16);
    emit("split3", {{"src", vten(t)}, {"dst", vten(pt)}, {"n", vint(n)}});
    planes_[t] = pt;
    return pt;
  }

  int use(int t) {
    T(t).consumers++;
    return t;
  }
  void contribute(int t, const EmitFn& fn) {
    T(t).contribs++;
    const bool last = T(t).contribs == T(t).consumers;
    PLAN_ASSERT(T(t).contribs <= T(t).consumers, "too many gradient contributions to %s", T(t).name.c_str());
    const int out = tensor("d_" + base_of(t), T(t).shape);
    fn(out, T(t).grad, (last && T(t).relu) ? t : -1);
    T(t).grad = out;
  }
  void contribute_alias(int t, int buf) {
    T(t).contribs++;
    const bool last = T(t).contribs == T(t).consumers;
    if (T(t).grad < 0 && !(last && T(t).relu)) {
      T(t).grad = buf;
      return;
    }
    const int out = tensor("d_" + base_of(t), T(t).shape);
    emit("grad_combine", {{"a", vten(buf)}, {"add_src", vten(T(t).grad)},
                          {"mask_src", vten((last && T(t).relu) ? t : -1)}, {"out", vten(out)},
                          {"shape", vints(T(t).shape)}});
    T(t).grad = out;
  }
  int grad_of(int t) {
    PLAN_ASSERT(T(t).contribs == T(t).consumers && T(t).grad >= 0, "gradient of %s incomplete (%d/%d)",
                T(t).name.c_str(), T(t).contribs, T(t).consumers);
    return T(t).grad;
  }

  Geom geom_of(int x, int cout, int k, int stride) {
    const Shape& s = T(x).shape;
    const int lo = (k - 1) / 2, hi = k - 1 - lo;
    Geom g;
    g.B = (int)s[0]; g.H = (int)s[1]; g.W = (int)s[2]; g.Cin = (int)s[3];
    g.Cout = cout; g.kh = g.kw = k; g.stride = stride;
    g.pad_h_lo = g.pad_w_lo = lo; g.pad_h_hi = g.pad_w_hi = hi;
    return g;
  }

  int bn_layer(int C, int64_t count, bool zero_gamma = false, const char* layer_name = nullptr) {
    const std::string layer = layer_name ? layer_name : unique("batch_normalization");
    BatchNorm bn;
    bn.C = C;
    bn.count = count;
    bn.gamma = variable(full(layer + "/gamma"), {C}, "gamma", {C}, true, false, zero_gamma);
    bn.beta = variable(full(layer + "/beta"), {C}, "beta", {C});
    bn.mm = variable(full(layer + "/moving_mean"), {C}, "moving_mean", {C}, false);
    bn.mv = variable(full(layer + "/moving_variance"), {C}, "moving_variance", {C}, false);
    if (training_) bn.stats = slot(BUF_WORK, fp32_ ? 2 * C : kStatsPartsCap * 2 * C);
    bn.work = slot(BUF_WORK, 4 * C);
    p_.bns.push_back(bn);
    return (int)p_.bns.size() - 1;
  }
  Val stats_of(int bn) { return (bn >= 0 && training_ && !fp32_) ? vslot(p_.bns[bn].stats) : Val(); }

  ConvOut conv(int x, int filters, int k, int stride, bool with_bn = true, bool zero_gamma = false,
               bool need_dgrad = true) {
    const Shape xs = T(x).shape;
    if (filters % 32 || xs[3] % 16)
      fail(ACNN_ERR_UNSUPPORTED, "conv %d -> %d channels: the tensor-core tiles need input channels in "
           "multiples of 16 and output channels in multiples of 32", (int)xs[3], filters);
    const std::string layer = unique("conv2d");
    ConvOut co;
    co.x = x;
    co.geom = geom_of(x, filters, k, stride);
    co.w = variable(full(layer + "/kernel"), {k, k, xs[3], filters}, "conv_kernel", {filters, k, k, xs[3]},
                    true, true, false, need_dgrad && training_);
    co.y = tensor("y", {xs[0], co.geom.Ho(), co.geom.Wo(), filters});
    if (with_bn) co.bn = bn_layer(filters, xs[0] * co.geom.Ho() * co.geom.Wo(), zero_gamma);
    const int xp = planes(x);
    emit("conv", {{"x", vten(x)}, {"xp", vten(xp)}, {"w", vvar(co.w)}, {"y", vten(co.y)},
                  {"geom", vgeom(co.geom)}, {"stats", stats_of(co.bn)}, {"out_f32", vint(0)}});
    if (co.bn >= 0) emit_bn_finalize(co.bn, co.y, co.geom);
    if (need_dgrad) use(x);
    return co;
  }

  void emit_bn_finalize(int bn, int y, const Geom& g, const std::vector<int64_t>* x_wpad = nullptr) {
    int mode = 0;
    if (training_ && fp32_) {
      emit("bn_stats", {{"x", vten(y)}, {"bn", vbn(bn)}, {"M", vint(p_.bns[bn].count)},
                        {"C", vint(p_.bns[bn].C)}});
      mode = 1;
    }
    emit("bn_finalize", {{"bn", vbn(bn)}, {"stats_mode", vint(mode)}, {"geom", vgeom(g)},
                         {"x_wpad", x_wpad ? vints(*x_wpad) : Val()}});
  }

  static void stem_s2d_taps(int k, int* p, int* k2, int* lo2, int* hi2) {
    *p = (k - 1) / 2;
    const int rmin = (int)floor(-(double)*p / 2), rmax = (int)floor((double)(k - 1 - *p) / 2);
    *k2 = rmax - rmin + 1;
    *lo2 = -rmin;
    *hi2 = rmax;
  }

  ConvOut stem_conv(int x0, int filters, int k) {
    const Shape xs = T(x0).shape;
    const std::string layer = unique("conv2d");
    int p, k2, lo2, hi2;
    stem_s2d_taps(k, &p, &k2, &lo2, &hi2);
    const int H2 = (int)xs[1], W2 = (int)xs[2] - lo2 - hi2;
    ConvOut co;
    co.x = x0;
    co.w = variable(full(layer + "/kernel"), {k, k, 3, filters}, "conv_kernel", {filters, k, k, 3}, true,
                    true);
    Geom g;
    g.B = (int)xs[0]; g.H = H2; g.W = W2; g.Cin = 16; g.Cout = filters; g.kh = g.kw = k2; g.stride = 1;
    g.pad_h_lo = g.pad_w_lo = lo2; g.pad_h_hi = g.pad_w_hi = hi2;
    PLAN_ASSERT(g.Ho() == H2 && g.Wo() == W2, "stem geometry");
    co.geom = g;
    co.y = tensor("y", {xs[0], H2, W2, filters});
    co.bn = bn_layer(filters, xs[0] * H2 * W2);
    co.has_stem = true;
    Stem& st = co.stem;
    st.k = k; st.pad = p; st.k2 = k2; st.pad2 = lo2; st.hi2 = hi2;
    st.w2 = tensor("w_stem", {filters, k2, k2, 16});
    if (training_) st.dw2 = slot(BUF_ZERO, (int64_t)filters * k2 * k2 * 16);
    st.alg_macs = xs[0] * H2 * W2 * filters * k * k * 3;
    emit("s2d_weight_pack", {{"w", vvar(co.w)}, {"w2", vten(st.w2)}, {"cout", vint(filters)},
                             {"k", vint(k)}, {"pad", vint(p)}, {"k2", vint(k2)}, {"pad2", vint(lo2)}});
    const int xp = planes(x0);
    const int wp = planes(st.w2);
    const std::vector<int64_t> wpad{lo2, hi2};
    emit("conv", {{"x", vten(x0)}, {"xp", vten(xp)}, {"w", vten(st.w2)}, {"wp", vten(wp)},
                  {"y", vten(co.y)}, {"geom", vgeom(g)}, {"stats", stats_of(co.bn)}, {"out_f32", vint(0)},
                  {"w_is_tensor", vint(1)}, {"x_wpad", vints(wpad)}, {"alg_macs", vint(st.alg_macs)}});
    emit_bn_finalize(co.bn, co.y, g, &wpad);
    return co;
  }

  int bn_act(const ConvOut& co, bool relu, int b = -1, int bn_b = -1, int b_mode = 0, Slot gate = Slot(),
             const char* name = "u") {
    const int out = tensor(name, T(co.y).shape, -1, relu);
    emit("bn_act", {{"a", vten(co.y)}, {"bn_a", vbn(co.bn)}, {"b", vten(b)}, {"bn_b", vbn(bn_b)},
                    {"b_mode", vint(b_mode)}, {"gate", vslot(gate)}, {"relu", vint(relu)},
                    {"out", vten(out)}, {"shape", vints(T(co.y).shape)}});
    return out;
  }

  int identity_bn(int C) {
    auto it = identity_bns_.find(C);
    if (it != identity_bns_.end()) return it->second;
    BatchNorm bn;
    bn.C = C;
    bn.work = slot(BUF_WORK, 4 * C);
    p_.ones.emplace_back(bn.work.offset, C);
    p_.bns.push_back(bn);
    return identity_bns_[C] = (int)p_.bns.size() - 1;
  }

  DbMask dropblock_mask(int H, int W, int C, double gamma_scale, int block_size = 7) {
    if (H < block_size || W < block_size)
      fail(ACNN_ERR_INVALID, "dropblock: feature map %dx%d smaller than block_size %d (the reference fails "
           "the same way: nets/blocks.py:222-229)", H, W, block_size);
    const int hs = H - block_size + 1, ws = W - block_size + 1;
    DbMask m;
    m.u = tensor("dropblock_u", {hs, ws, C}, ACNN_F32);
    m.index = (int)p_.dropblock_u.size();
    p_.dropblock_u.push_back(m.u);
    m.keep = slot(BUF_WORK, (int64_t)H * W * C);
    m.scale = slot(BUF_WORK, 1);
    m.scratch = slot(BUF_WORK, (int64_t)hs * ws * C + ((int64_t)H * W * C + 255) / 256);
    m.H = H; m.W = W; m.C = C; m.gamma_scale = gamma_scale; m.block_size = block_size;
    emit("dropblock_mask", {{"keep", vslot(m.keep)}, {"scale", vslot(m.scale)}, {"scratch", vslot(m.scratch)},
                            {"H", vint(H)}, {"W", vint(W)}, {"C", vint(C)}, {"gamma_scale", vflt(gamma_scale)},
                            {"block_size", vint(block_size)}, {"u", vten(m.u)}, {"index", vint(m.index)}});
    return m;
  }
  void emit_db_apply(int x, const DbMask& m, bool relu, int out, const Shape& s) {
    emit("dropblock_apply", {{"x", vten(x)}, {"keep", vslot(m.keep)}, {"scale", vslot(m.scale)},
                             {"relu", vint(relu)}, {"out", vten(out)}, {"B", vint(s[0])},
                             {"HW", vint(s[1] * s[2])}, {"C", vint(s[3])}});
  }
  int dropblock_apply(int x, const DbMask& m, bool relu, const char* name) {
    const Shape s = T(x).shape;
    const int out = tensor(name, s, -1, relu);
    emit_db_apply(x, m, relu, out, s);
    return out;
  }
  int dropblock_bwd(int g, const DbMask& m, const Shape& shape) {
    const int dt = tensor("d_db", shape);
    emit_db_apply(g, m, false, dt, shape);
    return dt;
  }
  int cbr_db(int x, int filters, int k, int stride, double gamma_scale) {
    const ConvOut co = conv(x, filters, k, stride);
    const int t = bn_act(co, false, -1, -1, 0, Slot(), "t");
    const Shape ts = T(t).shape;
    const DbMask m = dropblock_mask((int)ts[1], (int)ts[2], (int)ts[3], gamma_scale);
    const int u = dropblock_apply(t, m, true, "u");
    tape_.push_back([=] { conv_backward(co, bn_backward(co, dropblock_bwd(grad_of(u), m, ts))); });
    return u;
  }

  int bn_backward(const ConvOut& co, int g, Slot gate = Slot(), Slot addbc = Slot()) {
    const BatchNorm& bn = p_.bns[co.bn];
    const Slot sums = slot(BUF_WORK, kBwdPartsCap * 2 * bn.C);
    const Slot coef = slot(BUF_WORK, 3 * bn.C);
    const Shape ys = T(co.y).shape;
    const int dy = tensor("dy", ys);
    emit("bn_bwd_reduce", {{"g", vten(g)}, {"y", vten(co.y)}, {"bn", vbn(co.bn)}, {"gate", vslot(gate)},
                           {"addbc", vslot(addbc)}, {"sums", vslot(sums)}, {"shape", vints(ys)}});
    emit("bn_bwd_finalize", {{"bn", vbn(co.bn)}, {"sums", vslot(sums)}, {"coef", vslot(coef)}});
    emit("bn_bwd_apply", {{"g", vten(g)}, {"y", vten(co.y)}, {"coef", vslot(coef)}, {"gate", vslot(gate)},
                          {"addbc", vslot(addbc)}, {"dy", vten(dy)}, {"shape", vints(ys)}});
    return dy;
  }
  std::pair<int, int> bn_backward2(const ConvOut& a, const ConvOut& b, int g) {
    PLAN_ASSERT(T(a.y).shape == T(b.y).shape, "bn_backward2 shapes");
    const Shape ys = T(a.y).shape;
    const Slot sa = slot(BUF_WORK, kBwdPartsCap * 2 * p_.bns[a.bn].C);
    const Slot ca = slot(BUF_WORK, 3 * p_.bns[a.bn].C);
    const int da = tensor("dy", ys);
    const Slot sb = slot(BUF_WORK, kBwdPartsCap * 2 * p_.bns[b.bn].C);
    const Slot cb = slot(BUF_WORK, 3 * p_.bns[b.bn].C);
    const int db = tensor("dy", ys);
    emit("bn_bwd_reduce2", {{"g", vten(g)}, {"y", vten(a.y)}, {"bn", vbn(a.bn)}, {"sums", vslot(sa)},
                            {"y2", vten(b.y)}, {"bn2", vbn(b.bn)}, {"sums2", vslot(sb)}, {"shape", vints(ys)}});
    emit("bn_bwd_finalize", {{"bn", vbn(a.bn)}, {"sums", vslot(sa)}, {"coef", vslot(ca)}});
    emit("bn_bwd_finalize", {{"bn", vbn(b.bn)}, {"sums", vslot(sb)}, {"coef", vslot(cb)}});
    emit("bn_bwd_apply2", {{"g", vten(g)}, {"y", vten(a.y)}, {"coef", vslot(ca)}, {"dy", vten(da)},
                           {"y2", vten(b.y)}, {"coef2", vslot(cb)}, {"dy2", vten(db)}, {"shape", vints(ys)}});
    return {da, db};
  }

  void conv_backward(const ConvOut& co, int dy, bool need_dgrad = true) {
    const Geom g = co.geom;
    const int dyp = planes(dy);
    if (co.has_stem) {
      const Stem& st = co.stem;
      const int xp = planes(co.x);
      emit("conv_wgrad", {{"x", vten(co.x)}, {"xp", vten(xp)}, {"dy", vten(dy)}, {"dyp", vten(dyp)},
                          {"geom", vgeom(g)}, {"dw_slot", vslot(st.dw2)},
                          {"x_wpad", vints({st.pad2, st.hi2})}, {"alg_macs", vint(st.alg_macs)}});
      emit("s2d_wgrad_unpack", {{"dw2", vslot(st.dw2)}, {"w", vvar(co.w)}, {"cout", vint(g.Cout)},
                                {"k", vint(st.k)}, {"pad", vint(st.pad)}, {"k2", vint(st.k2)},
                                {"pad2", vint(st.pad2)}});
      return;
    }
    const int xp = planes(co.x);
    emit("conv_wgrad", {{"x", vten(co.x)}, {"xp", vten(xp)}, {"dy", vten(dy)}, {"dyp", vten(dyp)},
                        {"geom", vgeom(g)}, {"w", vvar(co.w)}});
    if (!need_dgrad) return;
    const int w = co.w;
    if (g.stride == 1) {
      contribute(co.x, [=](int out, int add, int mask) { emit_dgrad(dy, w, out, g, add, mask, -1); });
      return;
    }
    PLAN_ASSERT(g.stride == 2, "conv stride %d", g.stride);
    const int dyz = tensor("dyz", {g.B, g.H, g.W, g.Cout});
    emit("zero_insert", {{"dy", vten(dy)}, {"out", vten(dyz)}, {"B", vint(g.B)}, {"Ho", vint(g.Ho())},
                         {"Wo", vint(g.Wo())}, {"H", vint(g.H)}, {"W", vint(g.W)}, {"C", vint(g.Cout)}});
    Geom g1 = g;
    g1.stride = 1;
    g1.pad_h_hi = g.kh - 1 - g.pad_h_lo;
    g1.pad_w_hi = g.kw - 1 - g.pad_w_lo;
    const int64_t alg = (int64_t)g.B * g.Ho() * g.Wo() * g.Cout * g.kh * g.kw * g.Cin;
    contribute(co.x, [=](int out, int add, int mask) { emit_dgrad(dyz, w, out, g1, add, mask, alg); });
  }

  void emit_dgrad(int dy, int w, int out, const Geom& g, int add, int mask, int64_t alg_macs) {
    const Val alg = alg_macs >= 0 ? vint(alg_macs) : Val();
    if (fp32_ && (add >= 0 || mask >= 0)) {
      const Shape shape = T(out).shape;
      const int tmp = tensor("dx_raw", shape);
      const int dyp = planes(dy);
      emit("conv_dgrad", {{"dy", vten(dy)}, {"dyp", vten(dyp)}, {"w", vvar(w)}, {"dx", vten(tmp)},
                          {"geom", vgeom(g)}, {"alg_macs", alg}});
      emit("grad_combine", {{"a", vten(tmp)}, {"add_src", vten(add)}, {"mask_src", vten(mask)},
                            {"out", vten(out)}, {"shape", vints(shape)}});
    } else {
      const int dyp = planes(dy);
      emit("conv_dgrad", {{"dy", vten(dy)}, {"dyp", vten(dyp)}, {"w", vvar(w)}, {"dx", vten(out)},
                          {"geom", vgeom(g)}, {"add_src", vten(add)}, {"mask_src", vten(mask)},
                          {"alg_macs", alg}});
    }
  }

  int cbr(int x, int filters, int k, int stride, bool need_dgrad = true) {
    const ConvOut co = conv(x, filters, k, stride, true, false, need_dgrad);
    const int u = bn_act(co, true);
    tape_.push_back([=] { conv_backward(co, bn_backward(co, grad_of(u)), need_dgrad); });
    return u;
  }

  int sk(int t, int filters, int stride) {
    const int B = (int)T(t).shape[0];
    const ConvOut co = conv(t, 2 * filters, 3, stride);
    const int H = (int)T(co.y).shape[1], W = (int)T(co.y).shape[2];
    const int f = filters, d = std::max(filters / 2, 32);
    int w1, w2, bnz;
    {
      Scope s(*this, "sk_block");
      w1 = variable(full("sk_fc_1/kernel"), {1, 1, f, d}, "conv_kernel", {d, 1, 1, f}, true, true);
      bnz = bn_layer(d, B, false, "batch_normalization");
      w2 = variable(full("sk_fc_2/kernel"), {1, 1, d, 2 * f}, "conv_kernel", {2 * f, 1, 1, d}, true, true);
    }
    const Slot s = slot(BUF_WORK, (int64_t)B * f), zpre = slot(BUF_WORK, (int64_t)B * d),
               z = slot(BUF_WORK, (int64_t)B * d), att = slot(BUF_WORK, (int64_t)B * f),
               scratch = slot(BUF_WORK, acnn_sk_fc_scratch_floats(B, f, d));
    const int v = tensor("v", {B, H, W, f});
    const int HW = H * W;
#define SK_DIMS {"B", vint(B)}, {"HW", vint(HW)}, {"f", vint(f)}, {"d", vint(d)}
    emit("sk_gap", {{"y", vten(co.y)}, {"bn", vbn(co.bn)}, {"s", vslot(s)}, SK_DIMS});
    emit("sk_fc", {{"s", vslot(s)}, {"w1", vvar(w1)}, {"bn", vbn(bnz)}, {"w2", vvar(w2)},
                   {"zpre", vslot(zpre)}, {"z", vslot(z)}, {"att", vslot(att)}, {"scratch", vslot(scratch)},
                   SK_DIMS});
    emit("sk_combine", {{"y", vten(co.y)}, {"bn", vbn(co.bn)}, {"att", vslot(att)}, {"v", vten(v)}, SK_DIMS});
    tape_.push_back([=] {
      const int gv = grad_of(v);
      const Slot dA = slot(BUF_WORK, (int64_t)B * f), ds = slot(BUF_WORK, (int64_t)B * f),
                 sums = slot(BUF_WORK, (kBwdPartsCap + B) * 4 * f), coef = slot(BUF_WORK, 6 * f);
      const int dy = tensor("dy", T(co.y).shape);
      emit("sk_bwd_gate", {{"dv", vten(gv)}, {"y", vten(co.y)}, {"bn", vbn(co.bn)}, {"dA", vslot(dA)}, SK_DIMS});
      emit("sk_fc_bwd", {{"dA", vslot(dA)}, {"att", vslot(att)}, {"z", vslot(z)}, {"zpre", vslot(zpre)},
                         {"bn", vbn(bnz)}, {"s", vslot(s)}, {"w1", vvar(w1)}, {"w2", vvar(w2)},
                         {"ds", vslot(ds)}, {"scratch", vslot(scratch)}, SK_DIMS});
      emit("sk_bn_bwd_reduce", {{"dv", vten(gv)}, {"y", vten(co.y)}, {"bn", vbn(co.bn)}, {"att", vslot(att)},
                                {"ds", vslot(ds)}, {"sums", vslot(sums)}, SK_DIMS});
      emit("bn_bwd_finalize", {{"bn", vbn(co.bn)}, {"sums", vslot(sums)}, {"coef", vslot(coef)}});
      emit("sk_bn_bwd_apply", {{"dv", vten(gv)}, {"y", vten(co.y)}, {"bn", vbn(co.bn)}, {"att", vslot(att)},
                               {"ds", vslot(ds)}, {"coef", vslot(coef)}, {"dy", vten(dy)}, SK_DIMS});
      conv_backward(co, dy);
    });
#undef SK_DIMS
    return v;
  }

  int blurpool(int x, int filt, int stride) {
    const Shape s = T(x).shape;
    const int B = (int)s[0], H = (int)s[1], W = (int)s[2], C = (int)s[3], pad = (filt - 1) / 2;
    if (pad >= H || pad >= W)
      fail(ACNN_ERR_INVALID, "anti-alias filter %d on a %dx%d feature map: REFLECT padding of %d needs a larger "
           "map (tf.pad fails the same way, nets/blocks.py:70-75)", filt, H, W, pad);
    const int Ho = (H + 2 * pad - filt) / stride + 1, Wo = (W + 2 * pad - filt) / stride + 1;
    const int out = tensor("blur", {B, Ho, Wo, C});
#define BLUR_A {"B", vint(B)}, {"H", vint(H)}, {"W", vint(W)}, {"C", vint(C)}, {"filt", vint(filt)}, \
               {"stride", vint(stride)}
    emit("blurpool", {{"x", vten(x)}, {"out", vten(out)}, BLUR_A});
    use(x);
    tape_.push_back([=] {
      contribute(x, [=](int o, int add, int mask) {
        emit("blurpool_bwd", {{"dout", vten(grad_of(out))}, {"dx", vten(o)}, {"add_src", vten(add)},
                              {"mask_src", vten(mask)}, BLUR_A});
      });
    });
#undef BLUR_A
    return out;
  }

  int avgpool(int x, int k, int stride, int pad_lo, int Ho, int Wo, int count_pad) {
    const Shape s = T(x).shape;
    const int B = (int)s[0], H = (int)s[1], W = (int)s[2], C = (int)s[3];
    const int out = tensor("avgp", {B, Ho, Wo, C});
#define AVG_A {"B", vint(B)}, {"H", vint(H)}, {"W", vint(W)}, {"C", vint(C)}, {"k", vint(k)},          \
              {"stride", vint(stride)}, {"pad_lo", vint(pad_lo)}, {"Ho", vint(Ho)}, {"Wo", vint(Wo)}, \
              {"count_pad", vint(count_pad)}
    emit("avgpool", {{"x", vten(x)}, {"out", vten(out)}, AVG_A});
    use(x);
    tape_.push_back([=] {
      contribute(x, [=](int o, int add, int mask) {
        emit("avgpool_bwd", {{"dout", vten(grad_of(out))}, {"dx", vten(o)}, {"add_src", vten(add)},
                             {"mask_src", vten(mask)}, AVG_A});
      });
    });
#undef AVG_A
    return out;
  }

  int maxpool(int x, int k, int stride) {
    const Shape s = T(x).shape;
    const int B = (int)s[0], H = (int)s[1], W = (int)s[2], C = (int)s[3];
    const int Ho = (H + stride - 1) / stride, Wo = (W + stride - 1) / stride;
    const int total = std::max((Ho - 1) * stride + k - H, 0);
    const int pad_lo = total / 2;
    const int out = tensor("maxp", {B, Ho, Wo, C});
#define MAX_A {"B", vint(B)}, {"H", vint(H)}, {"W", vint(W)}, {"C", vint(C)}, {"k", vint(k)},          \
              {"stride", vint(stride)}, {"pad_lo", vint(pad_lo)}, {"Ho", vint(Ho)}, {"Wo", vint(Wo)}
    emit("maxpool", {{"x", vten(x)}, {"out", vten(out)}, MAX_A});
    use(x);
    tape_.push_back([=] {
      contribute(x, [=](int o, int add, int mask) {
        emit("maxpool_bwd", {{"dout", vten(grad_of(out))}, {"x", vten(x)}, {"dx", vten(o)},
                             {"add_src", vten(add)}, {"mask_src", vten(mask)}, MAX_A});
      });
    });
#undef MAX_A
    return out;
  }

  int residual_tail_db(const ConvOut& co3, const ConvOut* sc, int x_ident, bool relu, double gamma_scale,
                       const DbMask& ms) {
    const Shape ys = T(co3.y).shape;
    const int C = (int)ys[3];
    const int t3 = bn_act(co3, false, -1, -1, 0, Slot(), "t3");
    const DbMask m3 = dropblock_mask((int)ys[1], (int)ys[2], C, gamma_scale);
    const int t3d = dropblock_apply(t3, m3, false, "t3d");
    const bool mode_bn = sc != nullptr;
    int r;
    if (mode_bn) {
      const int ts = bn_act(*sc, false, -1, -1, 0, Slot(), "ts");
      r = dropblock_apply(ts, ms, false, "tsd");
    } else {
      r = x_ident;
      use(x_ident);
    }
    ConvOut ident;
    ident.y = t3d;
    ident.bn = identity_bn(C);
    const int out = bn_act(ident, relu, r, -1, 2, Slot(), "out");
    const ConvOut scv = sc ? *sc : ConvOut();
    tape_.push_back([=] {
      const int g = grad_of(out);
      conv_backward(co3, bn_backward(co3, dropblock_bwd(g, m3, ys)));
      if (mode_bn)
        conv_backward(scv, bn_backward(scv, dropblock_bwd(g, ms, ys)));
      else
        contribute_alias(x_ident, g);
    });
    return out;
  }

  int residual_tail(const ConvOut& co3, const ConvOut* sc, int sc_tensor, int b_mode, bool relu,
                    const SeGate& se = SeGate()) {
    const int out = b_mode == 1
                        ? bn_act(co3, relu, sc->y, sc->bn, 1, se.on ? se.e : Slot(), "out")
                        : bn_act(co3, relu, sc_tensor, -1, b_mode, se.on ? se.e : Slot(), "out");
    if (b_mode == 2 || b_mode == 3) use(sc_tensor);
    const ConvOut scv = sc ? *sc : ConvOut();
    tape_.push_back([=] {
      const int g = grad_of(out);
      int dy3;
      if (se.on) {
        const Shape ys = T(co3.y).shape;
        const int B = (int)ys[0], HW = (int)(ys[1] * ys[2]), C = (int)ys[3];
        const Slot de = slot(BUF_WORK, (int64_t)B * C), dq = slot(BUF_WORK, (int64_t)B * C);
        emit("se_bwd_gate", {{"g", vten(g)}, {"y", vten(co3.y)}, {"bn", vbn(co3.bn)}, {"de", vslot(de)},
                             {"B", vint(B)}, {"HW", vint(HW)}, {"C", vint(C)}, {"r", vint(se.r)}});
        emit("se_fc_bwd", {{"de", vslot(de)}, {"e", vslot(se.e)}, {"h", vslot(se.h)}, {"q", vslot(se.q)},
                           {"w1", vvar(se.w1)}, {"w2", vvar(se.w2)}, {"dq", vslot(dq)},
                           {"scratch", vslot(se.scratch)}, {"B", vint(B)}, {"HW", vint(HW)}, {"C", vint(C)},
                           {"r", vint(se.r)}});
        dy3 = bn_backward(co3, g, se.e, dq);
      } else if (b_mode == 1 && cfg_.fuse_bn_pairs) {
        const auto d = bn_backward2(co3, scv, g);
        conv_backward(co3, d.first);
        conv_backward(scv, d.second);
        return;
      } else {
        dy3 = bn_backward(co3, g);
      }
      conv_backward(co3, dy3);
      if (b_mode == 1) {
        conv_backward(scv, bn_backward(scv, g));
      } else if (b_mode == 2) {
        contribute_alias(sc_tensor, g);
      } else if (b_mode == 3) {
        const Shape s = T(sc_tensor).shape;
        contribute(sc_tensor, [=](int o, int add, int mask) {
          emit("upsample2x_bwd", {{"dout", vten(g)}, {"dx", vten(o)}, {"add_src", vten(add)},
                                  {"mask_src", vten(mask)}, {"B", vint(s[0])}, {"H", vint(s[1])},
                                  {"W", vint(s[2])}, {"C", vint(s[3])}});
        });
      }
    });
    return out;
  }

  SeGate se(const ConvOut& co3) {
    const Shape ys = T(co3.y).shape;
    const int B = (int)ys[0], HW = (int)(ys[1] * ys[2]), C = (int)ys[3], r = C / 16;
    SeGate g;
    g.on = true;
    g.r = r;
    {
      Scope s(*this, "se_block");
      g.w1 = variable(full("seblock_dense_1/kernel"), {1, 1, C, r}, "conv_kernel", {r, 1, 1, C}, true, true);
      g.w2 = variable(full("seblock_dense_2/kernel"), {1, 1, r, C}, "conv_kernel", {C, 1, 1, r}, true, true);
    }
    g.q = slot(BUF_WORK, (int64_t)B * C);
    g.h = slot(BUF_WORK, (int64_t)B * r);
    g.e = slot(BUF_WORK, (int64_t)B * C);
    g.scratch = slot(BUF_WORK, (int64_t)B * (C + r));
    emit("se_gap", {{"y", vten(co3.y)}, {"bn", vbn(co3.bn)}, {"q", vslot(g.q)}, {"B", vint(B)},
                    {"HW", vint(HW)}, {"C", vint(C)}, {"r", vint(r)}});
    emit("se_fc", {{"q", vslot(g.q)}, {"w1", vvar(g.w1)}, {"w2", vvar(g.w2)}, {"h", vslot(g.h)},
                   {"e", vslot(g.e)}, {"B", vint(B)}, {"HW", vint(HW)}, {"C", vint(C)}, {"r", vint(r)}});
    return g;
  }

  enum Shortcut { SC_NONE, SC_PROJ, SC_RESNET_D, SC_BL };
  static bool contains(const std::string& s, const char* sub) { return s.find(sub) != std::string::npos; }

  int bottleneck(int x, int filters, Shortcut kind, int strides, bool last_relu = true, double db = -1) {
    if (!use_dropblock_) db = -1;
    const bool sconv = contains(cfg_.anti_alias_type, "sconv");
    ConvOut sc;
    bool has_sc = false;
    if (kind != SC_NONE) {
      int xs = x, k_s = 1;
      const Shape s = T(x).shape;
      const int H = (int)s[1], W = (int)s[2];
      if (kind == SC_PROJ) {
        if (contains(cfg_.anti_alias_type, "proj") && strides != 1)
          xs = blurpool(x, cfg_.anti_alias_filter_size, strides);
        else
          k_s = strides;
      } else if (kind == SC_RESNET_D) {
        xs = strides > 1 ? avgpool(x, 2, strides, 0, H / strides, W / strides, 1)
                         : avgpool(x, 2, 1, 0, H, W, 0);
      } else if (kind == SC_BL) {
        if (strides > 1)
          xs = avgpool(x, 3, strides, 1, (H + 2 - 3) / strides + 1, (W + 2 - 3) / strides + 1, 1);
      }
      sc = conv(xs, filters * 4, 1, k_s);
      has_sc = true;
    }
    DbMask ms;
    if (db >= 0 && has_sc) {
      const Shape s = T(sc.y).shape;
      ms = dropblock_mask((int)s[1], (int)s[2], (int)s[3], db);
    }
    int t = db < 0 ? cbr(x, filters, 1, 1) : cbr_db(x, filters, 1, 1, db);
    const int s3 = sconv ? 1 : strides;
    if (cfg_.use_sk_block) {
      t = sk(t, filters, s3);
      if (db >= 0) {
        const int v = t;
        const Shape vs = T(v).shape;
        const DbMask m = dropblock_mask((int)vs[1], (int)vs[2], (int)vs[3], db);
        t = dropblock_apply(v, m, false, "vd");
        use(v);
        const int td = t;
        tape_.push_back([=] {
          contribute(v, [=](int out, int add, int mask) {
            PLAN_ASSERT(add < 0 && mask < 0, "dropblock contribution with epilogue");
            emit_db_apply(grad_of(td), m, false, out, vs);
          });
        });
      }
    } else {
      t = db < 0 ? cbr(t, filters, 3, s3) : cbr_db(t, filters, 3, s3, db);
    }
    if (sconv && strides != 1) t = blurpool(t, cfg_.anti_alias_filter_size, strides);
    const ConvOut co3 = conv(t, filters * 4, 1, 1, true, cfg_.zero_gamma);
    if (db >= 0) return residual_tail_db(co3, has_sc ? &sc : nullptr, x, last_relu, db, ms);
    const SeGate g = cfg_.use_se_block ? se(co3) : SeGate();
    if (has_sc) return residual_tail(co3, &sc, -1, 1, last_relu, g);
// ... 440 lines not shown
```

assembled_cnn_b200/csrc/ptx.cuh:

```cuda
#pragma once
#include <cuda.h>
#include <cuda_runtime.h>
#include <cuda_bf16.h>
#include <stdint.h>

namespace acnn {

#ifndef ACNN_PDL_PRIMS
#define ACNN_PDL_PRIMS
__device__ __forceinline__ void pdl_trigger() {
  asm volatile("griddepcontrol.launch_dependents;\n" ::: "memory");
}
__device__ __forceinline__ void pdl_wait() { asm volatile("griddepcontrol.wait;\n" ::: "memory"); }
__device__ __forceinline__ void pdl_entry() {
  pdl_trigger();
  pdl_wait();
}
#endif

__device__ __forceinline__ uint32_t smem_u32(const void* p) {
  return static_cast<uint32_t>(__cvta_generic_to_shared(p));
}

__device__ __forceinline__ bool elect_one() {
  uint32_t pred;
  asm volatile(
      "{\n\t.reg .pred p;\n\t"
      "elect.sync _|p, 0xffffffff;\n\t"
      "selp.u32 %0, 1, 0, p;\n\t}\n"
      : "=r"(pred));
  return pred != 0;
}

__device__ __forceinline__ void mbar_init(uint64_t* bar, uint32_t count) {
  asm volatile("mbarrier.init.shared::cta.b64 [%0], %1;\n" ::"r"(smem_u32(bar)), "r"(count));
}
__device__ __forceinline__ void fence_barrier_init() {
  asm volatile("fence.mbarrier_init.release.cluster;\n" ::: "memory");
}
__device__ __forceinline__ void mbar_expect_tx(uint64_t* bar, uint32_t bytes) {
  asm volatile("mbarrier.arrive.expect_tx.shared::cta.b64 _, [%0], %1;\n" ::"r"(smem_u32(bar)),
               "r"(bytes)
               : "memory");
}
__device__ __forceinline__ void mbar_arrive(uint64_t* bar) {
  asm volatile("mbarrier.arrive.shared::cta.b64 _, [%0];\n" ::"r"(smem_u32(bar)) : "memory");
}
__device__ __forceinline__ bool mbar_try_wait(uint64_t* bar, uint32_t parity) {
  uint32_t ok;
  asm volatile(
      "{\n\t.reg .pred p;\n\t"
      "mbarrier.try_wait.parity.shared::cta.b64 p, [%1], %2;\n\t"
      "selp.u32 %0, 1, 0, p;\n\t}\n"
      : "=r"(ok)
      : "r"(smem_u32(bar)), "r"(parity)
      : "memory");
  return ok != 0;
}
__device__ __forceinline__ void mbar_wait(uint64_t* bar, uint32_t parity) {
  uint32_t spins = 0;
  while (!mbar_try_wait(bar, parity)) {
    if (++spins > (1u << 26)) __trap();
  }
}

__device__ __forceinline__ void mbar_expect_tx_a(uint32_t bar, uint32_t bytes) {
  asm volatile("mbarrier.arrive.expect_tx.shared::cta.b64 _, [%0], %1;\n" ::"r"(bar), "r"(bytes)
               : "memory");
}
__device__ __forceinline__ void mbar_wait_a(uint32_t bar, uint32_t parity) {
  uint32_t spins = 0;
  for (;;) {
    uint32_t ok;
    asm volatile(
        "{\n\t.reg .pred p;\n\t"
        "mbarrier.try_wait.parity.shared::cta.b64 p, [%1], %2;\n\t"
        "selp.u32 %0, 1, 0, p;\n\t}\n"
        : "=r"(ok)
        : "r"(bar), "r"(parity)
        : "memory");
    if (ok) break;
    if (++spins > (1u << 26)) __trap();
  }
}

__device__ __forceinline__ void fence_proxy_async() {
  asm volatile("fence.proxy.async.shared::cta;\n" ::: "memory");
}

__device__ __forceinline__ void tma_prefetch_desc(const CUtensorMap* m) {
  asm volatile("prefetch.tensormap [%0];\n" ::"l"(reinterpret_cast<uint64_t>(m)) : "memory");
}
__device__ __forceinline__ void tma_load_2d(void* smem_dst, const CUtensorMap* m, uint64_t* bar,
                                            int32_t c0, int32_t c1) {
  asm volatile(
      "cp.async.bulk.tensor.2d.shared::cluster.global.mbarrier::complete_tx::bytes"
      " [%0], [%1, {%3, %4}], [%2];\n" ::"r"(smem_u32(smem_dst)),
      "l"(reinterpret_cast<uint64_t>(m)), "r"(smem_u32(bar)), "r"(c0), "r"(c1)
      : "memory");
}
__device__ __forceinline__ void tma_load_im2col_4d(void* smem_dst, const CUtensorMap* m,
                                                   uint64_t* bar, int32_t c, int32_t w, int32_t h,
                                                   int32_t n, uint16_t off_w, uint16_t off_h) {
  asm volatile(
      "cp.async.bulk.tensor.4d.shared::cluster.global.im2col.mbarrier::complete_tx::bytes"
      " [%0], [%1, {%3, %4, %5, %6}], [%2], {%7, %8};\n" ::"r"(smem_u32(smem_dst)),
      "l"(reinterpret_cast<uint64_t>(m)), "r"(smem_u32(bar)), "r"(c), "r"(w), "r"(h), "r"(n),
      "h"(off_w), "h"(off_h)
      : "memory");
}

__device__ __forceinline__ void tma_load_2d_a(uint32_t smem_dst, const CUtensorMap* m, uint32_t bar,
                                              int32_t c0, int32_t c1) {
  asm volatile(
      "cp.async.bulk.tensor.2d.shared::cluster.global.mbarrier::complete_tx::bytes"
      " [%0], [%1, {%3, %4}], [%2];\n" ::"r"(smem_dst),
      "l"(reinterpret_cast<uint64_t>(m)), "r"(bar), "r"(c0), "r"(c1)
      : "memory");
}
__device__ __forceinline__ void tma_load_im2col_4d_a(uint32_t smem_dst, const CUtensorMap* m,
                                                     uint32_t bar, int32_t c, int32_t w, int32_t h,
                                                     int32_t n, uint16_t off_w, uint16_t off_h) {
  asm volatile(
      "cp.async.bulk.tensor.4d.shared::cluster.global.im2col.mbarrier::complete_tx::bytes"
      " [%0], [%1, {%3, %4, %5, %6}], [%2], {%7, %8};\n" ::"r"(smem_dst),
      "l"(reinterpret_cast<uint64_t>(m)), "r"(bar), "r"(c), "r"(w), "r"(h), "r"(n), "h"(off_w),
      "h"(off_h)
      : "memory");
}

__device__ __forceinline__ void tma_load_4d_tile_a(uint32_t smem_dst, const CUtensorMap* m,
                                                   uint32_t bar, int32_t c, int32_t w, int32_t h,
                                                   int32_t n) {
  asm volatile(
      "cp.async.bulk.tensor.4d.shared::cluster.global.tile.mbarrier::complete_tx::bytes"
      " [%0], [%1, {%3, %4, %5, %6}], [%2];\n" ::"r"(smem_dst),
      "l"(reinterpret_cast<uint64_t>(m)), "r"(bar), "r"(c), "r"(w), "r"(h), "r"(n)
      : "memory");
}
__device__ __forceinline__ void tma_store_4d(const CUtensorMap* m, const void* smem_src, int32_t c,
                                             int32_t w, int32_t h, int32_t n) {
  asm volatile(
      "cp.async.bulk.tensor.4d.global.shared::cta.tile.bulk_group [%0, {%2, %3, %4, %5}], [%1];\n" ::"l"(
          reinterpret_cast<uint64_t>(m)),
      "r"(smem_u32(smem_src)), "r"(c), "r"(w), "r"(h), "r"(n)
      : "memory");
}

__device__ __forceinline__ void tma_store_2d(const CUtensorMap* m, const void* smem_src, int32_t c0,
                                             int32_t c1) {
  asm volatile(
      "cp.async.bulk.tensor.2d.global.shared::cta.bulk_group [%0, {%2, %3}], [%1];\n" ::"l"(
          reinterpret_cast<uint64_t>(m)),
      "r"(smem_u32(smem_src)), "r"(c0), "r"(c1)
      : "memory");
}
__device__ __forceinline__ void tma_store_commit() {
  asm volatile("cp.async.bulk.commit_group;\n" ::: "memory");
}
__device__ __forceinline__ void tma_store_wait_read() {
  asm volatile("cp.async.bulk.wait_group.read 0;\n" ::: "memory");
}
__device__ __forceinline__ void tma_store_wait_read1() {
  asm volatile("cp.async.bulk.wait_group.read 1;\n" ::: "memory");
}
__device__ __forceinline__ void tma_store_wait_all() {
  asm volatile("cp.async.bulk.wait_group 0;\n" ::: "memory");
}

__device__ __forceinline__ void wgmma_fence() { asm volatile("wgmma.fence.sync.aligned;\n" ::: "memory"); }
__device__ __forceinline__ void wgmma_commit() {
  asm volatile("wgmma.commit_group.sync.aligned;\n" ::: "memory");
}
template <int N>
__device__ __forceinline__ void wgmma_wait() {
  asm volatile("wgmma.wait_group.sync.aligned %0;\n" ::"n"(N) : "memory");
}
template <int R>
__device__ __forceinline__ void wgmma_fence_operand(float (&d)[R]) {
#pragma unroll
  for (int i = 0; i < R; ++i) asm volatile("" : "+f"(d[i])::"memory");
}
template <int N>
struct Wgmma;
template <>
struct Wgmma<32> {
  template <int TA, int TB>
  __device__ static __forceinline__ void mma(float (&d)[16], uint64_t da, uint64_t db, uint32_t accumulate) {
    asm volatile(
        "{\n\t.reg .pred p;\n\t"
        "setp.ne.b32 p, %18, 0;\n\t"
        "wgmma.mma_async.sync.aligned.m64n32k16.f32.bf16.bf16 "
        "{%0, %1, %2, %3, %4, %5, %6, %7, %8, %9, %10, %11, %12, %13, %14, %15}, "
        "%16, %17, p, 1, 1, %19, %20;\n\t}\n"
        : "+f"(d[0]), "+f"(d[1]), "+f"(d[2]), "+f"(d[3]), "+f"(d[4]), "+f"(d[5]), "+f"(d[6]), "+f"(d[7]), "+f"(d[8]), "+f"(d[9]), "+f"(d[10]), "+f"(d[11]), "+f"(d[12]), "+f"(d[13]), "+f"(d[14]), "+f"(d[15])
        : "l"(da), "l"(db), "r"(accumulate), "n"(TA), "n"(TB));
  }
};
template <>
struct Wgmma<64> {
  template <int TA, int TB>
  __device__ static __forceinline__ void mma(float (&d)[32], uint64_t da, uint64_t db, uint32_t accumulate) {
    asm volatile(
        "{\n\t.reg .pred p;\n\t"
        "setp.ne.b32 p, %34, 0;\n\t"
        "wgmma.mma_async.sync.aligned.m64n64k16.f32.bf16.bf16 "
        "{%0, %1, %2, %3, %4, %5, %6, %7, %8, %9, %10, %11, %12, %13, %14, %15, %16, %17, %18, %19, %20, %21, %22, %23, %24, %25, %26, %27, %28, %29, %30, %31}, "
        "%32, %33, p, 1, 1, %35, %36;\n\t}\n"
        : "+f"(d[0]), "+f"(d[1]), "+f"(d[2]), "+f"(d[3]), "+f"(d[4]), "+f"(d[5]), "+f"(d[6]), "+f"(d[7]), "+f"(d[8]), "+f"(d[9]), "+f"(d[10]), "+f"(d[11]), "+f"(d[12]), "+f"(d[13]), "+f"(d[14]), "+f"(d[15]), "+f"(d[16]), "+f"(d[17]), "+f"(d[18]), "+f"(d[19]), "+f"(d[20]), "+f"(d[21]), "+f"(d[22]), "+f"(d[23]), "+f"(d[24]), "+f"(d[25]), "+f"(d[26]), "+f"(d[27]), "+f"(d[28]), "+f"(d[29]), "+f"(d[30]), "+f"(d[31])
        : "l"(da), "l"(db), "r"(accumulate), "n"(TA), "n"(TB));
  }
};
template <>
struct Wgmma<128> {
  template <int TA, int TB>
  __device__ static __forceinline__ void mma(float (&d)[64], uint64_t da, uint64_t db, uint32_t accumulate) {
    asm volatile(
        "{\n\t.reg .pred p;\n\t"
        "setp.ne.b32 p, %66, 0;\n\t"
        "wgmma.mma_async.sync.aligned.m64n128k16.f32.bf16.bf16 "
        "{%0, %1, %2, %3, %4, %5, %6, %7, %8, %9, %10, %11, %12, %13, %14, %15, %16, %17, %18, %19, %20, %21, %22, %23, %24, %25, %26, %27, %28, %29, %30, %31, %32, %33, %34, %35, %36, %37, %38, %39, %40, %41, %42, %43, %44, %45, %46, %47, %48, %49, %50, %51, %52, %53, %54, %55, %56, %57, %58, %59, %60, %61, %62, %63}, "
        "%64, %65, p, 1, 1, %67, %68;\n\t}\n"
        : "+f"(d[0]), "+f"(d[1]), "+f"(d[2]), "+f"(d[3]), "+f"(d[4]), "+f"(d[5]), "+f"(d[6]), "+f"(d[7]), "+f"(d[8]), "+f"(d[9]), "+f"(d[10]), "+f"(d[11]), "+f"(d[12]), "+f"(d[13]), "+f"(d[14]), "+f"(d[15]), "+f"(d[16]), "+f"(d[17]), "+f"(d[18]), "+f"(d[19]), "+f"(d[20]), "+f"(d[21]), "+f"(d[22]), "+f"(d[23]), "+f"(d[24]), "+f"(d[25]), "+f"(d[26]), "+f"(d[27]), "+f"(d[28]), "+f"(d[29]), "+f"(d[30]), "+f"(d[31]), "+f"(d[32]), "+f"(d[33]), "+f"(d[34]), "+f"(d[35]), "+f"(d[36]), "+f"(d[37]), "+f"(d[38]), "+f"(d[39]), "+f"(d[40]), "+f"(d[41]), "+f"(d[42]), "+f"(d[43]), "+f"(d[44]), "+f"(d[45]), "+f"(d[46]), "+f"(d[47]), "+f"(d[48]), "+f"(d[49]), "+f"(d[50]), "+f"(d[51]), "+f"(d[52]), "+f"(d[53]), "+f"(d[54]), "+f"(d[55]), "+f"(d[56]), "+f"(d[57]), "+f"(d[58]), "+f"(d[59]), "+f"(d[60]), "+f"(d[61]), "+f"(d[62]), "+f"(d[63])
        : "l"(da), "l"(db), "r"(accumulate), "n"(TA), "n"(TB));
  }
};
template <>
struct Wgmma<256> {
  template <int TA, int TB>
  __device__ static __forceinline__ void mma(float (&d)[128], uint64_t da, uint64_t db, uint32_t accumulate) {
    asm volatile(
        "{\n\t.reg .pred p;\n\t"
        "setp.ne.b32 p, %130, 0;\n\t"
        "wgmma.mma_async.sync.aligned.m64n256k16.f32.bf16.bf16 "
        "{%0, %1, %2, %3, %4, %5, %6, %7, %8, %9, %10, %11, %12, %13, %14, %15, %16, %17, %18, %19, %20, %21, %22, %23, %24, %25, %26, %27, %28, %29, %30, %31, %32, %33, %34, %35, %36, %37, %38, %39, %40, %41, %42, %43, %44, %45, %46, %47, %48, %49, %50, %51, %52, %53, %54, %55, %56, %57, %58, %59, %60, %61, %62, %63, %64, %65, %66, %67, %68, %69, %70, %71, %72, %73, %74, %75, %76, %77, %78, %79, %80, %81, %82, %83, %84, %85, %86, %87, %88, %89, %90, %91, %92, %93, %94, %95, %96, %97, %98, %99, %100, %101, %102, %103, %104, %105, %106, %107, %108, %109, %110, %111, %112, %113, %114, %115, %116, %117, %118, %119, %120, %121, %122, %123, %124, %125, %126, %127}, "
        "%128, %129, p, 1, 1, %131, %132;\n\t}\n"
        : "+f"(d[0]), "+f"(d[1]), "+f"(d[2]), "+f"(d[3]), "+f"(d[4]), "+f"(d[5]), "+f"(d[6]), "+f"(d[7]), "+f"(d[8]), "+f"(d[9]), "+f"(d[10]), "+f"(d[11]), "+f"(d[12]), "+f"(d[13]), "+f"(d[14]), "+f"(d[15]), "+f"(d[16]), "+f"(d[17]), "+f"(d[18]), "+f"(d[19]), "+f"(d[20]), "+f"(d[21]), "+f"(d[22]), "+f"(d[23]), "+f"(d[24]), "+f"(d[25]), "+f"(d[26]), "+f"(d[27]), "+f"(d[28]), "+f"(d[29]), "+f"(d[30]), "+f"(d[31]), "+f"(d[32]), "+f"(d[33]), "+f"(d[34]), "+f"(d[35]), "+f"(d[36]), "+f"(d[37]), "+f"(d[38]), "+f"(d[39]), "+f"(d[40]), "+f"(d[41]), "+f"(d[42]), "+f"(d[43]), "+f"(d[44]), "+f"(d[45]), "+f"(d[46]), "+f"(d[47]), "+f"(d[48]), "+f"(d[49]), "+f"(d[50]), "+f"(d[51]), "+f"(d[52]), "+f"(d[53]), "+f"(d[54]), "+f"(d[55]), "+f"(d[56]), "+f"(d[57]), "+f"(d[58]), "+f"(d[59]), "+f"(d[60]), "+f"(d[61]), "+f"(d[62]), "+f"(d[63]), "+f"(d[64]), "+f"(d[65]), "+f"(d[66]), "+f"(d[67]), "+f"(d[68]), "+f"(d[69]), "+f"(d[70]), "+f"(d[71]), "+f"(d[72]), "+f"(d[73]), "+f"(d[74]), "+f"(d[75]), "+f"(d[76]), "+f"(d[77]), "+f"(d[78]), "+f"(d[79]), "+f"(d[80]), "+f"(d[81]), "+f"(d[82]), "+f"(d[83]), "+f"(d[84]), "+f"(d[85]), "+f"(d[86]), "+f"(d[87]), "+f"(d[88]), "+f"(d[89]), "+f"(d[90]), "+f"(d[91]), "+f"(d[92]), "+f"(d[93]), "+f"(d[94]), "+f"(d[95]), "+f"(d[96]), "+f"(d[97]), "+f"(d[98]), "+f"(d[99]), "+f"(d[100]), "+f"(d[101]), "+f"(d[102]), "+f"(d[103]), "+f"(d[104]), "+f"(d[105]), "+f"(d[106]), "+f"(d[107]), "+f"(d[108]), "+f"(d[109]), "+f"(d[110]), "+f"(d[111]), "+f"(d[112]), "+f"(d[113]), "+f"(d[114]), "+f"(d[115]), "+f"(d[116]), "+f"(d[117]), "+f"(d[118]), "+f"(d[119]), "+f"(d[120]), "+f"(d[121]), "+f"(d[122]), "+f"(d[123]), "+f"(d[124]), "+f"(d[125]), "+f"(d[126]), "+f"(d[127])
        : "l"(da), "l"(db), "r"(accumulate), "n"(TA), "n"(TB));
  }
};

__device__ __forceinline__ uint64_t make_smem_desc(uint32_t smem_addr, uint32_t lbo_bytes,
                                                   uint32_t sbo_bytes, uint32_t layout_type) {
  uint64_t d = 0;
  d |= static_cast<uint64_t>((smem_addr >> 4) & 0x3FFF);
  d |= static_cast<uint64_t>((lbo_bytes >> 4) & 0x3FFF) << 16;
  d |= static_cast<uint64_t>((sbo_bytes >> 4) & 0x3FFF) << 32;
  d |= static_cast<uint64_t>(layout_type & 3) << 62;
  return d;
}
__host__ __device__ constexpr uint32_t swizzle_layout_type(int bytes) {
  return bytes == 128 ? 1u : (bytes == 64 ? 2u : 3u);
}

__device__ __forceinline__ void named_bar_sync(int id, int count) {
  asm volatile("bar.sync %0, %1;\n" ::"r"(id), "r"(count) : "memory");
}

__device__ __forceinline__ float bf16_lo(uint32_t pair) { return __uint_as_float(pair << 16); }
__device__ __forceinline__ float bf16_hi(uint32_t pair) { return __uint_as_float(pair & 0xffff0000u); }
__device__ __forceinline__ void bf16x2_add(float& c0, float& c1, uint32_t pair) {
  c0 += bf16_lo(pair);
  c1 += bf16_hi(pair);
}
__device__ __forceinline__ void bf16x2_sum_sq(float& s0, float& q0, float& s1, float& q1,
                                              uint32_t pair) {
  const float lo = bf16_lo(pair), hi = bf16_hi(pair);
  s0 += lo;
  q0 = __fmaf_rn(lo, lo, q0);
  s1 += hi;
  q1 = __fmaf_rn(hi, hi, q1);
}
__device__ __forceinline__ uint32_t bf16x2_gt0_mask(uint32_t pair) {
  uint32_t m;
  asm("set.gt.u32.bf16x2 %0, %1, %2;\n" : "=r"(m) : "r"(pair), "r"(0u));
  return m;
}

__device__ __forceinline__ float bf16_round(float x) {
  return __bfloat162float(__float2bfloat16_rn(x));
}
__device__ __forceinline__ uint32_t pack_bf16x2(float lo, float hi) {
  __nv_bfloat162 h = __floats2bfloat162_rn(lo, hi);
  return *reinterpret_cast<uint32_t*>(&h);
}

}

namespace acnn {

__device__ __forceinline__ uint32_t cluster_ctarank() {
  uint32_t r;
  asm volatile("mov.u32 %0, %%cluster_ctarank;\n" : "=r"(r));
  return r;
}
__device__ __forceinline__ void cluster_sync() {
  asm volatile("barrier.cluster.arrive.release.aligned;\n" ::: "memory");
  asm volatile("barrier.cluster.wait.acquire.aligned;\n" ::: "memory");
}
__device__ __forceinline__ uint32_t mapa_shared(uint32_t addr, uint32_t rank) {
  uint32_t r;
  asm volatile("mapa.shared::cluster.u32 %0, %1, %2;\n" : "=r"(r) : "r"(addr), "r"(rank));
  return r;
}
__device__ __forceinline__ void mbar_arrive_cluster(uint32_t cluster_addr) {
  asm volatile("mbarrier.arrive.release.cluster.shared::cluster.b64 _, [%0];\n" ::"r"(cluster_addr)
               : "memory");
}
__device__ __forceinline__ void tma_load_2d_multicast(uint32_t smem_dst, const CUtensorMap* m,
                                                      uint32_t bar, int32_t c0, int32_t c1,
                                                      uint16_t mask) {
  asm volatile(
      "cp.async.bulk.tensor.2d.shared::cluster.global.mbarrier::complete_tx::bytes.multicast::cluster"
      " [%0], [%1, {%3, %4}], [%2], %5;\n" ::"r"(smem_dst),
      "l"(reinterpret_cast<uint64_t>(m)), "r"(bar), "r"(c0), "r"(c1), "h"(mask)
      : "memory");
}

}
```

assembled_cnn_b200/plan.py:

```python
from __future__ import annotations

import os
import math
from collections import OrderedDict
from dataclasses import dataclass, field

BLOCK_SIZES = {
    1: {50: [3, 4, 6, 3], 101: [3, 4, 23, 3], 152: [3, 8, 36, 3], 200: [3, 24, 36, 3]},
    2: {50: [3, 4, 6, 3], 101: [4, 8, 18, 3], 152: [5, 12, 30, 3]},
}
ALIGN = 256
def _sk_job_floats(M, N, K, share):
    tiles = -(-M // 64) * -(-N // 64)
    s = max(1, min(share // tiles, K // 32, 8))
    kper = -(-(-(-K // s)) // 16) * 16
    return -(-K // kper) * M * N


def sk_fc_scratch_floats(B, f, d, G=132):
    fwd = max(_sk_job_floats(B, d, f, G), _sk_job_floats(B, 2 * f, d, G))
    bwd = max(_sk_job_floats(2 * f, d, B, G // 2) + _sk_job_floats(B, d, 2 * f, G // 2),
              _sk_job_floats(d, f, B, G // 2) + _sk_job_floats(B, f, d, G // 2))
    return B * (2 * f + d) + max(fwd, bwd)

# ... 207 lines not shown
        if mixup_type not in (0, 1, 2):
            raise ValueError("mixup_type must be 0, 1 or 2")
        self.cfg = cfg
        self.B = batch
        self.training = training
        self.mixup_type = mixup_type if training else 0
        self.with_loss = with_loss or training
        self.plan = Plan()
        self.tape = []
        self._scope = ["resnet_model"]
        self._counters = {}
        self._tid = 0
        self.ops = self.plan.forward
        p = self.plan
        p.meta.update(batch=batch, height=height, width=width, training=training,
                      mixup_type=self.mixup_type, label_smoothing=label_smoothing,
                      num_classes=cfg.num_classes, ld_logits=_round_up(cfg.num_classes, 128),
                      bn_momentum=cfg.bn_momentum, dtype=dtype, use_dropblock=self.use_dropblock,
                      kd_temp=self.kd_temp, dropblock_u=[], ones=[],
                      input_batch=batch * 2 if self.mixup_type == 1 else batch)
        self._build(height, width)

    def _unique(self, base):
        key = ("/".join(self._scope), base)
        n = self._counters.get(key, 0)
        self._counters[key] = n + 1
        return base if n == 0 else "%s_%d" % (base, n)

    class _Scope:
        def __init__(self, b, name):
            self.b, self.name = b, name

        def __enter__(self):
            self.b._scope.append(self.b._unique(self.name))

        def __exit__(self, *a):
            self.b._scope.pop()

    def scope(self, name):
        return PlanBuilder._Scope(self, name)

    def _full(self, name):
        return "/".join(self._scope + [name])

    def tensor(self, base, shape, dtype=None, relu=False):
        dtype = dtype or self.adt
        self._tid += 1
        name = "%s#%d" % (base, self._tid)
        t = Tensor(name, tuple(shape), dtype, relu)
        self.plan.tensors[name] = t
        return t

    def _param(self, name, tf_shape, kind, store_shape, *, trainable=True, decay=False,
               zero_init=False, need_dgrad=False):
        p = self.plan
        size = 1
        for s in store_shape:
            size *= s
        if trainable:
            par = Param(name, tuple(tf_shape), kind, p.param_elems, size, tuple(store_shape), True,
                        decay, zero_init)
            p.param_elems += _round_up(size)
            if need_dgrad:
                par.dgrad_off = p.dgrad_elems
                p.dgrad_elems += _round_up(size)
            assert name not in p.params, name
            p.params[name] = par
        else:
            par = Param(name, tuple(tf_shape), kind, p.state_elems, size, tuple(store_shape), False)
            p.state_elems += _round_up(size)
            p.state[name] = par
        return par

    def slot(self, buf, size):
        p = self.plan
        if buf == "zero":
            s = Slot("zero", p.zero_elems, size)
            p.zero_elems += _round_up(size, 32)
        else:
            s = Slot("work", p.work_elems, size)
            p.work_elems += _round_up(size, 32)
        return s

    def emit(self, kind, **a):
        self.ops.append(Op(kind, a))

    def planes(self, name):
        if not self.fp32:
            return None
        pl = self._planes.get(name)
        if pl is None:
            t = self.plan.tensors[name]
            n = 1
            for d in t.shape:
                n *= d
            pt = self.tensor("planes", (3,) + tuple(t.shape), "bf16")
            self.emit("split3", src=name, dst=pt.name, n=n)
            self._planes[name] = pl = pt.name
        return pl

    def use(self, t: Tensor):
        t.consumers += 1
        return t

    def contribute(self, t: Tensor, emit_fn):
        t.contribs += 1
        last = t.contribs == t.consumers
        assert t.contribs <= t.consumers, t.name
        out = self.tensor("d_" + t.name.split("#")[0], t.shape)
        emit_fn(out.name, t.grad, t.name if (last and t.relu) else None)
        t.grad = out.name

    def contribute_alias(self, t: Tensor, buf: str):
        t.contribs += 1
        last = t.contribs == t.consumers
        if t.grad is None and not (last and t.relu):
            t.grad = buf
            return
        out = self.tensor("d_" + t.name.split("#")[0], t.shape)
        self.emit("grad_combine", a=buf, add_src=t.grad, mask_src=t.name if (last and t.relu) else None,
                  out=out.name, shape=t.shape)
        t.grad = out.name

    def grad_of(self, t: Tensor) -> str:
        assert t.contribs == t.consumers and t.grad is not None, \
            "gradient of %s incomplete (%d/%d)" % (t.name, t.contribs, t.consumers)
        return t.grad

    def _geom(self, x: Tensor, cout, k, stride):
        B, H, W, C = x.shape
        lo = (k - 1) // 2
        hi = k - 1 - lo
        return Geom(B, H, W, C, cout, k, k, stride, lo, hi, lo, hi)

    def bn_layer(self, C, count, zero_gamma=False, layer=None):
        layer = layer or self._unique("batch_normalization")
        g = self._param(self._full(layer + "/gamma"), (C,), "gamma", (C,), zero_init=zero_gamma)
        b = self._param(self._full(layer + "/beta"), (C,), "beta", (C,))
        mm = self._param(self._full(layer + "/moving_mean"), (C,), "moving_mean", (C,), trainable=False)
        mv = self._param(self._full(layer + "/moving_variance"), (C,), "moving_variance", (C,),
                         trainable=False)
        stats = None
        if self.training:
            stats = self.slot("work", 2 * C if self.fp32 else STATS_PARTS_CAP * 2 * C)
        bn = BN(C, g.name, b.name, mm.name, mv.name, count, stats, self.slot("work", 4 * C))
        self.plan.bns.append(bn)
        return bn

    def conv(self, x: Tensor, filters, k, stride, *, with_bn=True, zero_gamma=False,
             need_dgrad=True) -> ConvOut:
        B, H, W, Cin = x.shape
        if filters % 32 or Cin % 16:
            raise NotImplementedError("conv %d -> %d channels: the tensor-core tiles need input channels in "
                                      "multiples of 16 and output channels in multiples of 32" % (Cin, filters))
        layer = self._unique("conv2d")
        g = self._geom(x, filters, k, stride)
        w = self._param(self._full(layer + "/kernel"), (k, k, Cin, filters), "conv_kernel",
                        (filters, k, k, Cin), decay=True, need_dgrad=need_dgrad and self.training)
        y = self.tensor("y", (B, g.Ho, g.Wo, filters))
        bn = self.bn_layer(filters, B * g.Ho * g.Wo, zero_gamma) if with_bn else None
        self.emit("conv", x=x.name, xp=self.planes(x.name), w=w.name, y=y.name, geom=g,
                  stats=bn.stats if (bn and self.training and not self.fp32) else None, bias=None,
                  out_f32=False)
        if bn:
            self.emit_bn_finalize(bn, y, g)
        if need_dgrad:
            self.use(x)
        return ConvOut(x, y, g, w.name, bn)

    def emit_bn_finalize(self, bn: BN, y: Tensor, geom: Geom, x_wpad=None):
        mode = 0
        if self.training and self.fp32:
            self.emit("bn_stats", x=y.name, bn=bn, M=bn.count, C=bn.C)
            mode = 1
        self.emit("bn_finalize", bn=bn, stats_mode=mode, geom=geom, x_wpad=x_wpad)

    @staticmethod
    def stem_s2d_taps(k):
        p = (k - 1) // 2
        rmin = math.floor(-p / 2)
        rmax = math.floor((k - 1 - p) / 2)
        return p, rmax - rmin + 1, -rmin, rmax

    def stem_conv(self, x0: Tensor, filters, k) -> ConvOut:
        B, H2, Wp, C16 = x0.shape
        layer = self._unique("conv2d")
        p, k2, lo2, hi2 = self.stem_s2d_taps(k)
        W2 = Wp - lo2 - hi2
        w = self._param(self._full(layer + "/kernel"), (k, k, 3, filters), "conv_kernel",
                        (filters, k, k, 3), decay=True)
        g = Geom(B, H2, W2, 16, filters, k2, k2, 1, lo2, hi2, lo2, hi2)
        assert g.Ho == H2 and g.Wo == W2
        y = self.tensor("y", (B, H2, W2, filters))
        bn = self.bn_layer(filters, B * H2 * W2)
        stem = dict(k=k, pad=p, k2=k2, pad2=lo2, w2=self.tensor("w_stem", (filters, k2, k2, 16)),
                    dw2=self.slot("zero", filters * k2 * k2 * 16) if self.training else None)
        self.emit("s2d_weight_pack", w=w.name, w2=stem["w2"].name, cout=filters, **{
            "k": k, "pad": p, "k2": k2, "pad2": lo2})
        stem["x_wpad"] = (lo2, hi2)
        self.emit("conv", x=x0.name, xp=self.planes(x0.name), w=stem["w2"].name,
                  wp=self.planes(stem["w2"].name), y=y.name, geom=g,
                  stats=bn.stats if (self.training and not self.fp32) else None, bias=None,
                  out_f32=False, w_is_tensor=True, x_wpad=(lo2, hi2),
                  alg_macs=B * H2 * W2 * filters * k * k * 3)
        stem["alg_macs"] = B * H2 * W2 * filters * k * k * 3
        self.emit_bn_finalize(bn, y, g, (lo2, hi2))
        return ConvOut(x0, y, g, w.name, bn, stem)

    def bn_act(self, co: ConvOut, *, relu, b=None, b_mode=0, gate=None, name="u") -> Tensor:
        out = self.tensor(name, co.y.shape, relu=relu)
        self.emit("bn_act", a=co.y.name, bn_a=co.bn,
                  b=(b.y.name if b_mode == 1 else (b.name if b is not None else None)),
                  bn_b=(b.bn if b_mode == 1 else None), b_mode=b_mode, gate=gate, relu=relu,
                  out=out.name, shape=co.y.shape)
        return out

    def identity_bn(self, C):
        bn = self._identity_bns.get(C)
        if bn is None:
            work = self.slot("work", 4 * C)
            self.plan.meta["ones"].append((work.offset, C))
            bn = self._identity_bns[C] = BN(C, None, None, None, None, 0, None, work)
        return bn

    def dropblock_mask(self, H, W, C, gamma_scale, block_size=7):
        if H < block_size or W < block_size:
            raise ValueError("dropblock: feature map %dx%d smaller than block_size %d (the reference "
                             "fails the same way: nets/blocks.py:222-229)" % (H, W, block_size))
        hs, ws = H - block_size + 1, W - block_size + 1
        u = self.tensor("dropblock_u", (hs, ws, C), "f32")
        index = len(self.plan.meta["dropblock_u"])
        self.plan.meta["dropblock_u"].append(u.name)
        m = dict(keep=self.slot("work", H * W * C), scale=self.slot("work", 1),
                 scratch=self.slot("work", hs * ws * C + (H * W * C + 255) // 256),
                 H=H, W=W, C=C, gamma_scale=gamma_scale, block_size=block_size, u=u.name,
                 index=index)
        self.emit("dropblock_mask", **m)
        return m

    def dropblock_apply(self, x: Tensor, m, relu, name="db") -> Tensor:
        B, H, W, C = x.shape
        out = self.tensor(name, x.shape, relu=relu)
        self.emit("dropblock_apply", x=x.name, keep=m["keep"], scale=m["scale"], relu=relu,
                  out=out.name, B=B, HW=H * W, C=C)
        return out

    def dropblock_bwd(self, g: str, m, shape) -> str:
        B, H, W, C = shape
        dt = self.tensor("d_db", shape)
        self.emit("dropblock_apply", x=g, keep=m["keep"], scale=m["scale"], relu=False,
                  out=dt.name, B=B, HW=H * W, C=C)
        return dt.name

    def cbr_db(self, x: Tensor, filters, k, stride, gamma_scale) -> Tensor:
        co = self.conv(x, filters, k, stride)
        t = self.bn_act(co, relu=False, name="t")
        m = self.dropblock_mask(t.shape[1], t.shape[2], t.shape[3], gamma_scale)
        u = self.dropblock_apply(t, m, relu=True, name="u")
        self.tape.append(lambda: self.conv_backward(co, self.bn_backward(
            co, self.dropblock_bwd(self.grad_of(u), m, t.shape))))
        return u

    def bn_backward(self, co: ConvOut, g: str, gate=None, addbc=None) -> str:
        bn, y = co.bn, co.y
        sums = self.slot("work", BWD_PARTS_CAP * 2 * bn.C)
        coef = self.slot("work", 3 * bn.C)
        dy = self.tensor("dy", y.shape)
        self.emit("bn_bwd_reduce", g=g, y=y.name, bn=bn, gate=gate, addbc=addbc, sums=sums,
                  shape=y.shape)
        self.emit("bn_bwd_finalize", bn=bn, sums=sums, coef=coef)
        self.emit("bn_bwd_apply", g=g, y=y.name, coef=coef, gate=gate, addbc=addbc, dy=dy.name,
                  shape=y.shape)
        return dy.name

    def bn_backward2(self, co_a: ConvOut, co_b: ConvOut, g: str):
        assert co_a.y.shape == co_b.y.shape
        outs = []
        for co in (co_a, co_b):
            outs.append((self.slot("work", BWD_PARTS_CAP * 2 * co.bn.C), self.slot("work", 3 * co.bn.C),
                         self.tensor("dy", co.y.shape)))
        (sa, ca, da), (sb, cb, db) = outs
        self.emit("bn_bwd_reduce2", g=g, y=co_a.y.name, bn=co_a.bn, sums=sa, y2=co_b.y.name,
                  bn2=co_b.bn, sums2=sb, shape=co_a.y.shape)
        self.emit("bn_bwd_finalize", bn=co_a.bn, sums=sa, coef=ca)
        self.emit("bn_bwd_finalize", bn=co_b.bn, sums=sb, coef=cb)
        self.emit("bn_bwd_apply2", g=g, y=co_a.y.name, coef=ca, dy=da.name, y2=co_b.y.name, coef2=cb,
                  dy2=db.name, shape=co_a.y.shape)
        return da.name, db.name

    def conv_backward(self, co: ConvOut, dy: str, need_dgrad=True):
        g = co.geom
        dyp = self.planes(dy)
        if co.stem is not None:
            self.emit("conv_wgrad", x=co.x.name, xp=self.planes(co.x.name), dy=dy, dyp=dyp, geom=g,
                      dw_slot=co.stem["dw2"], x_wpad=co.stem["x_wpad"],
                      alg_macs=co.stem["alg_macs"])
            self.emit("s2d_wgrad_unpack", dw2=co.stem["dw2"], w=co.w, cout=g.Cout, k=co.stem["k"],
                      pad=co.stem["pad"], k2=co.stem["k2"], pad2=co.stem["pad2"])
            return
        self.emit("conv_wgrad", x=co.x.name, xp=self.planes(co.x.name), dy=dy, dyp=dyp, geom=g,
                  w=co.w)
        if not need_dgrad:
            return
        if g.stride == 1:
            self.contribute(co.x, lambda out, add, mask: self.emit_dgrad(
                dy, co.w, out, g, add, mask))
        else:
            assert g.stride == 2
            dyz = self.tensor("dyz", (g.B, g.H, g.W, g.Cout))
            self.emit("zero_insert", dy=dy, out=dyz.name, B=g.B, Ho=g.Ho, Wo=g.Wo, H=g.H, W=g.W,
                      C=g.Cout)
            g1 = Geom(g.B, g.H, g.W, g.Cin, g.Cout, g.kh, g.kw, 1, g.pad_h_lo,
                      g.kh - 1 - g.pad_h_lo, g.pad_w_lo, g.kw - 1 - g.pad_w_lo)
            alg = g.B * g.Ho * g.Wo * g.Cout * g.kh * g.kw * g.Cin
            self.contribute(co.x, lambda out, add, mask: self.emit_dgrad(
                dyz.name, co.w, out, g1, add, mask, alg_macs=alg))

    def emit_dgrad(self, dy, w, out, g, add, mask, alg_macs=None):
        if self.fp32 and (add is not None or mask is not None):
            shape = self.plan.tensors[out].shape
            tmp = self.tensor("dx_raw", shape)
            self.emit("conv_dgrad", dy=dy, dyp=self.planes(dy), w=w, dx=tmp.name, geom=g,
                      add_src=None, mask_src=None, alg_macs=alg_macs)
            self.emit("grad_combine", a=tmp.name, add_src=add, mask_src=mask, out=out, shape=shape)
        else:
            self.emit("conv_dgrad", dy=dy, dyp=self.planes(dy), w=w, dx=out, geom=g, add_src=add,
                      mask_src=mask, alg_macs=alg_macs)

    def cbr(self, x: Tensor, filters, k, stride, need_dgrad=True) -> Tensor:
        co = self.conv(x, filters, k, stride, need_dgrad=need_dgrad)
        u = self.bn_act(co, relu=True)
        self.tape.append(lambda: self.conv_backward(co, self.bn_backward(co, self.grad_of(u)),
                                                    need_dgrad))
        return u

    def stem_cbr(self, x0: Tensor, filters, k) -> Tensor:
        co = self.stem_conv(x0, filters, k)
        u = self.bn_act(co, relu=True)
        self.tape.append(lambda: self.conv_backward(co, self.bn_backward(co, self.grad_of(u))))
        return u

    def sk(self, t: Tensor, filters, stride) -> Tensor:
        B = t.shape[0]
        co = self.conv(t, 2 * filters, 3, stride)
        H, W = co.y.shape[1:3]
        f, d = filters, max(int(filters / 2), 32)
        with self.scope("sk_block"):
            w1 = self._param(self._full("sk_fc_1/kernel"), (1, 1, f, d), "conv_kernel", (d, 1, 1, f),
                             decay=True)
            bnz = self.bn_layer(d, B, layer="batch_normalization")
            w2 = self._param(self._full("sk_fc_2/kernel"), (1, 1, d, 2 * f), "conv_kernel",
                             (2 * f, 1, 1, d), decay=True)
        s = self.slot("work", B * f)
        zpre = self.slot("work", B * d)
        z = self.slot("work", B * d)
        att = self.slot("work", B * f)
        scratch = self.slot("work", sk_fc_scratch_floats(B, f, d))
        v = self.tensor("v", (B, H, W, f))
        dims = dict(B=B, HW=H * W, f=f, d=d)
        self.emit("sk_gap", y=co.y.name, bn=co.bn, s=s, **dims)
        self.emit("sk_fc", s=s, w1=w1.name, bn=bnz, w2=w2.name, zpre=zpre, z=z, att=att,
                  scratch=scratch, **dims)
        self.emit("sk_combine", y=co.y.name, bn=co.bn, att=att, v=v.name, **dims)

        def bwd():
            gv = self.grad_of(v)
            dA = self.slot("work", B * f)
            ds = self.slot("work", B * f)
            sums = self.slot("work", (BWD_PARTS_CAP + B) * 4 * f)
            coef = self.slot("work", 6 * f)
            dy = self.tensor("dy", co.y.shape)
            self.emit("sk_bwd_gate", dv=gv, y=co.y.name, bn=co.bn, dA=dA, **dims)
            self.emit("sk_fc_bwd", dA=dA, att=att, z=z, zpre=zpre, bn=bnz, s=s, w1=w1.name,
                      w2=w2.name, ds=ds, scratch=scratch, **dims)
            self.emit("sk_bn_bwd_reduce", dv=gv, y=co.y.name, bn=co.bn, att=att, ds=ds, sums=sums,
                      **dims)
            self.emit("bn_bwd_finalize", bn=co.bn, sums=sums, coef=coef)
            self.emit("sk_bn_bwd_apply", dv=gv, y=co.y.name, bn=co.bn, att=att, ds=ds, coef=coef,
                      dy=dy.name, **dims)
            self.conv_backward(co, dy.name)
        self.tape.append(bwd)
        return v

    def blurpool(self, x: Tensor, filt, stride) -> Tensor:
        B, H, W, C = x.shape
        pad = (filt - 1) // 2
        if pad >= H or pad >= W:
            raise ValueError("anti-alias filter %d on a %dx%d feature map: REFLECT padding of %d needs a larger "
                             "map (tf.pad fails the same way, nets/blocks.py:70-75)" % (filt, H, W, pad))
        Ho, Wo = (H + 2 * pad - filt) // stride + 1, (W + 2 * pad - filt) // stride + 1
        out = self.tensor("blur", (B, Ho, Wo, C))
        a = dict(B=B, H=H, W=W, C=C, filt=filt, stride=stride)
        self.emit("blurpool", x=x.name, out=out.name, **a)
        self.use(x)
        self.tape.append(lambda: self.contribute(x, lambda o, add, mask: self.emit(
            "blurpool_bwd", dout=self.grad_of(out), dx=o, add_src=add, mask_src=mask, **a)))
        return out

    def avgpool(self, x: Tensor, k, stride, pad_lo, Ho, Wo, count_pad) -> Tensor:
        B, H, W, C = x.shape
        out = self.tensor("avgp", (B, Ho, Wo, C))
        a = dict(B=B, H=H, W=W, C=C, k=k, stride=stride, pad_lo=pad_lo, Ho=Ho, Wo=Wo,
                 count_pad=count_pad)
        self.emit("avgpool", x=x.name, out=out.name, **a)
        self.use(x)
        self.tape.append(lambda: self.contribute(x, lambda o, add, mask: self.emit(
            "avgpool_bwd", dout=self.grad_of(out), dx=o, add_src=add, mask_src=mask, **a)))
        return out

    def maxpool(self, x: Tensor, k, stride) -> Tensor:
        B, H, W, C = x.shape
        Ho, Wo = -(-H // stride), -(-W // stride)
        total = max((Ho - 1) * stride + k - H, 0)
        pad_lo = total // 2
        out = self.tensor("maxp", (B, Ho, Wo, C))
        a = dict(B=B, H=H, W=W, C=C, k=k, stride=stride, pad_lo=pad_lo, Ho=Ho, Wo=Wo)
        self.emit("maxpool", x=x.name, out=out.name, **a)
        self.use(x)
        self.tape.append(lambda: self.contribute(x, lambda o, add, mask: self.emit(
            "maxpool_bwd", dout=self.grad_of(out), x=x.name, dx=o, add_src=add, mask_src=mask, **a)))
        return out

    def residual_tail_db(self, co3: ConvOut, *, shortcut, mode, relu, gamma_scale, ms=None) -> Tensor:
        B, H, W, C = co3.y.shape
        t3 = self.bn_act(co3, relu=False, name="t3")
        m3 = self.dropblock_mask(H, W, C, gamma_scale)
        t3d = self.dropblock_apply(t3, m3, relu=False, name="t3d")
        if mode == "bn":
            ts = self.bn_act(shortcut, relu=False, name="ts")
            r = self.dropblock_apply(ts, ms, relu=False, name="tsd")
        else:
            assert mode == "identity"
            r = shortcut
            self.use(shortcut)
        ident = ConvOut(None, t3d, None, None, self.identity_bn(C))
        out = self.bn_act(ident, relu=relu, b=r, b_mode=2, name="out")

        def bwd():
            g = self.grad_of(out)
            self.conv_backward(co3, self.bn_backward(co3, self.dropblock_bwd(g, m3, co3.y.shape)))
            if mode == "bn":
                self.conv_backward(shortcut, self.bn_backward(
                    shortcut, self.dropblock_bwd(g, ms, co3.y.shape)))
            else:
                self.contribute_alias(shortcut, g)
        self.tape.append(bwd)
        return out

    def residual_tail(self, co3: ConvOut, *, shortcut, mode, relu, se=None) -> Tensor:
        b_mode = {"bn": 1, "identity": 2, "up2": 3, None: 0}[mode]
        gate = se["e"] if se else None
        out = self.bn_act(co3, relu=relu, b=shortcut, b_mode=b_mode, gate=gate, name="out")
        if mode in ("identity", "up2"):
            self.use(shortcut)

        def bwd():
            g = self.grad_of(out)
            if se:
                B, H, W, C = co3.y.shape
                dims = dict(B=B, HW=H * W, C=C, r=se["r"])
                de = self.slot("work", B * C)
                dq = self.slot("work", B * C)
                self.emit("se_bwd_gate", g=g, y=co3.y.name, bn=co3.bn, de=de, **dims)
                self.emit("se_fc_bwd", de=de, e=se["e"], h=se["h"], q=se["q"], w1=se["w1"],
                          w2=se["w2"], dq=dq, scratch=se["scratch"], **dims)
                dy3 = self.bn_backward(co3, g, gate=se["e"], addbc=dq)
            elif mode == "bn" and self.fuse_bn_pairs:
                dy3, dys = self.bn_backward2(co3, shortcut, g)
                self.conv_backward(co3, dy3)
                self.conv_backward(shortcut, dys)
                return
            else:
                dy3 = self.bn_backward(co3, g)
            self.conv_backward(co3, dy3)
            if mode == "bn":
                self.conv_backward(shortcut, self.bn_backward(shortcut, g))
            elif mode == "identity":
                self.contribute_alias(shortcut, g)
            elif mode == "up2":
                B, H, W, C = shortcut.shape
                self.contribute(shortcut, lambda o, add, mask: self.emit(
                    "upsample2x_bwd", dout=g, dx=o, add_src=add, mask_src=mask, B=B, H=H, W=W, C=C))
        self.tape.append(bwd)
        return out

    def se(self, co3: ConvOut) -> dict:
        B, H, W, C = co3.y.shape
        r = C // 16
        with self.scope("se_block"):
            w1 = self._param(self._full("seblock_dense_1/kernel"), (1, 1, C, r), "conv_kernel",
                             (r, 1, 1, C), decay=True)
            w2 = self._param(self._full("seblock_dense_2/kernel"), (1, 1, r, C), "conv_kernel",
                             (C, 1, 1, r), decay=True)
        q, h, e = self.slot("work", B * C), self.slot("work", B * r), self.slot("work", B * C)
        scratch = self.slot("work", B * (C + r))
        dims = dict(B=B, HW=H * W, C=C, r=r)
        self.emit("se_gap", y=co3.y.name, bn=co3.bn, q=q, **dims)
        self.emit("se_fc", q=q, w1=w1.name, w2=w2.name, h=h, e=e, **dims)
        return dict(q=q, h=h, e=e, w1=w1.name, w2=w2.name, r=r, scratch=scratch)

    def bottleneck(self, x: Tensor, filters, shortcut_kind, strides, last_relu=True, db=None) -> Tensor:
        cfg = self.cfg
        if not self.use_dropblock:
            db = None
        sconv = "sconv" in cfg.anti_alias_type
        sc = None
        if shortcut_kind is not None:
            xs = x
            k_s = 1
            if shortcut_kind == "proj":
                if "proj" in cfg.anti_alias_type and strides != 1:
                    xs = self.blurpool(x, cfg.anti_alias_filter_size, strides)
                else:
                    k_s = strides
            elif shortcut_kind == "resnet_d":
                B, H, W, C = x.shape
                if strides > 1:
                    xs = self.avgpool(x, 2, strides, 0, H // strides, W // strides, 1)
                else:
                    xs = self.avgpool(x, 2, 1, 0, H, W, 0)
            elif shortcut_kind == "bl":
                B, H, W, C = x.shape
                if strides > 1:
                    xs = self.avgpool(x, 3, strides, 1, (H + 2 - 3) // strides + 1,
                                      (W + 2 - 3) // strides + 1, 1)
            sc = self.conv(xs, filters * 4, 1, k_s)
        ms = None
        if db is not None and sc is not None:
            ms = self.dropblock_mask(sc.y.shape[1], sc.y.shape[2], sc.y.shape[3], db)
        t = self.cbr(x, filters, 1, 1) if db is None else self.cbr_db(x, filters, 1, 1, db)
        s3 = 1 if sconv else strides
        if cfg.use_sk_block:
            t = self.sk(t, filters, s3)
            if db is not None:
                v = t
                m = self.dropblock_mask(v.shape[1], v.shape[2], v.shape[3], db)
                t = self.dropblock_apply(v, m, relu=False, name="vd")
                self.use(v)
                self.tape.append(lambda v=v, m=m, t=t: self.contribute(
                    v, lambda out, add, mask: self._emit_db_contrib(self.grad_of(t), m, v, out, add,
                                                                     mask)))
        else:
            t = self.cbr(t, filters, 3, s3) if db is None else self.cbr_db(t, filters, 3, s3, db)
        if sconv and strides != 1:
            t = self.blurpool(t, cfg.anti_alias_filter_size, strides)
        co3 = self.conv(t, filters * 4, 1, 1, zero_gamma=cfg.zero_gamma)
        if db is not None:
            return self.residual_tail_db(co3, shortcut=sc if sc is not None else x,
                                         mode="bn" if sc is not None else "identity",
                                         relu=last_relu, gamma_scale=db, ms=ms)
        se = self.se(co3) if cfg.use_se_block else None
        if sc is not None:
            return self.residual_tail(co3, shortcut=sc, mode="bn", relu=last_relu, se=se)
        return self.residual_tail(co3, shortcut=x, mode="identity", relu=last_relu, se=se)

    def _emit_db_contrib(self, g, m, v, out, add, mask):
        assert add is None and mask is None
        B, H, W, C = v.shape
        self.emit("dropblock_apply", x=g, keep=m["keep"], scale=m["scale"], relu=False, out=out,
                  B=B, HW=H * W, C=C)

    def block_layer(self, x, filters, num_blocks, strides, *, use_resnet_d=False, use_bl=False,
                    last_relu=True, db=None):
        kind = "resnet_d" if use_resnet_d else ("bl" if use_bl else "proj")
        x = self.bottleneck(x, filters, kind, strides, db=db)
        for i in range(1, num_blocks):
            x = self.bottleneck(x, filters, None, 1,
                                last_relu=last_relu if i == num_blocks - 1 else True, db=db)
        return x

    def _build(self, H, W):
        cfg, p, B = self.cfg, self.plan, self.B
        meta = p.meta
        nf = 64
        Bin = meta["input_batch"]
        images = self.tensor("images", (Bin, H, W, 3), "f32")
        meta["images"] = images.name
        _, _, wlo, whi = self.stem_s2d_taps(3 if cfg.use_resnet_d else 7)
        x0 = self.tensor("x0", (B, H // 2, W // 2 + wlo + whi, 16))
        self.emit("prep_weights")
        lam1 = lam2 = None
        if self.mixup_type:
            lam1 = self.tensor("lam1", (Bin // 2,), "f32")
            meta["lam1"] = lam1.name
            if self.mixup_type == 2:
                lam2 = self.tensor("lam2", (Bin // 2,), "f32")
                meta["lam2"] = lam2.name
        self.emit("pack_input", images=images.name, lam1=lam1 and lam1.name,
                  lam2=lam2 and lam2.name, mode=self.mixup_type, out=x0.name, Bin=Bin, H=H, W=W,
                  wpad=(wlo, whi))

        d = cfg.use_resnet_d
        if d and cfg.resnet_version == 1:
            x = self.stem_cbr(x0, nf // 2, 3)
            x = self.cbr(x, nf // 2, 3, 1)
            co = self.conv(x, nf, 3, 1, with_bn=False)
            co.bn = self.bn_layer(nf, B * (H // 2) * (W // 2))
            self._attach_bn(co)
        elif d:
            with self.scope("stage0"):
                x = self.stem_cbr(x0, nf // 2, 3)
                x = self.cbr(x, nf // 2, 3, 1)
                co = self.conv(x, nf, 3, 1, with_bn=False)
            with self.scope("stage0"):
                co.bn = self.bn_layer(nf, B * (H // 2) * (W // 2))
                self._attach_bn(co)
        elif cfg.resnet_version == 2:
# ... 219 lines not shown
```

Before: 5417.

## Add sub-pixel phase-decomposed halo kernel for stride-2 3x3 conv dgrad

Stride-2 dgrad no longer zero-inserts dy and runs a stride-1 conv over the 4x larger tensor. A new phase mode of the halo kernel computes the four output parity phases directly from the un-inserted dy, using only the taps each phase needs (1, 2, 2 and 4 of 9) and writing them through 5D TMA stores. This removes the zero-insert pass, its scratch buffer, and roughly three quarters of wasted MMAs on zeros. The cost is extra kernel complexity, a cap of N tile 64 on phase mode, and a fallback to the old path when shape conditions fail.

After: 5476, median of 6. +1.1%, better.

```diff
diff --git a/assembled_cnn_b200/csrc/gemm.cu b/assembled_cnn_b200/csrc/gemm.cu
--- a/assembled_cnn_b200/csrc/gemm.cu
+++ b/assembled_cnn_b200/csrc/gemm.cu
@@ -1,6 +1,7 @@
 #include <stdlib.h>
 
 #include <algorithm>
+#include <type_traits>
 
 #include "common.h"
 #include "ptx.cuh"
@@ -458,6 +459,19 @@
 constexpr int kHaloH = 18, kHaloW = 10, kPatchH = 16, kPatchW = 8;
 constexpr int kHaloMaxB = 32;
 
+__host__ __device__ constexpr int phase_ntaps(int ph) { return ((ph >> 1) + 1) * ((ph & 1) + 1); }
+__host__ __device__ constexpr int phase_tap_r(int ph, int j) {
+  return (ph >> 1) ? 2 * (j / ((ph & 1) + 1)) : 1;
+}
+__host__ __device__ constexpr int phase_tap_s(int ph, int j) { return (ph & 1) ? 2 * (j % 2) : 1; }
+__host__ __device__ constexpr int phase_tap_k(int ph, int j) {
+  return phase_tap_r(ph, j) * 3 + phase_tap_s(ph, j);
+}
+__host__ __device__ constexpr int phase_tap_shift(int ph, int j) {
+  return (1 + ((ph >> 1) + phase_tap_r(ph, j) - 1) / 2) * kHaloW + 1 +
+         ((ph & 1) + phase_tap_s(ph, j) - 1) / 2;
+}
+
 struct HaloParams {
   int H, W, B;
   int Cin, Cout;
@@ -503,7 +517,14 @@
   }
 };
 
-template <int BN, int CW>
+template <int BN>
+struct HaloPhaseCfg {
+  static_assert(BN <= 64, "phase mode: N tile <= 64 (accumulator registers)");
+  static constexpr int kG = 128 / BN;
+  static constexpr int kUnits = 4 / kG;
+};
+
+template <int BN, int CW, bool kPh>
 __global__ void __launch_bounds__(kThreads, 1)
 conv_halo_kernel(const __grid_constant__ CUtensorMap tmA, const __grid_constant__ CUtensorMap tmB,
                  const __grid_constant__ CUtensorMap tmC, const __grid_constant__ CUtensorMap tmAdd,
@@ -515,6 +536,8 @@
   constexpr int kSubW = Cfg::kSubW;
   constexpr int kSubBytes = kBM * kSubW * 2;
   constexpr int kNSub = BN / kSubW;
+  constexpr int kG = kPh ? HaloPhaseCfg<(kPh ? BN : 32)>::kG : 1;
+  constexpr int kUnits = kPh ? HaloPhaseCfg<(kPh ? BN : 32)>::kUnits : 1;
 
   extern __shared__ uint8_t smem_raw[];
   __shared__ uint64_t a_full[4], a_empty[4];
@@ -525,8 +548,8 @@
                                              ~static_cast<uintptr_t>(1023));
   const int AS = p.a_stages, NB = p.b_slots;
   uint8_t* s_out = smem + AS * Cfg::kAStage + NB * Cfg::kBTile;
-  uint8_t* s_add = s_out + Cfg::kTileBytes;
-  uint8_t* s_mask = s_add + (p.has_add ? Cfg::kTileBytes : 0);
+  uint8_t* s_add = s_out + kG * Cfg::kTileBytes;
+  uint8_t* s_mask = s_add + (p.has_add ? kG * Cfg::kTileBytes : 0);
 
   const int warp = threadIdx.x >> 5;
   const int lane = threadIdx.x & 31;
@@ -577,25 +600,27 @@
       const int img = tile / tpi;
       const int rem = tile - img * tpi;
       const int h0 = (rem / p.pw) * kPatchH, w0 = (rem % p.pw) * kPatchW;
-      for (int kc = 0; kc < nchunks; ++kc) {
-        mbar_wait_a(aempty0 + sa * 8, a_ph ^ 1);
-        if (elect_one()) {
-          mbar_expect_tx_a(afull0 + sa * 8, Cfg::kABytes);
-          tma_load_4d_tile_a(a_base + sa * Cfg::kAStage, &tmA, afull0 + sa * 8, kc * CW, w0 - 1,
-                             h0 - 1, img);
-        }
-        __syncwarp();
-        if (++sa == static_cast<uint32_t>(AS)) { sa = 0; a_ph ^= 1; }
-        if (!p.stationary) {
-          for (int t = 0; t < 9; ++t) {
-            mbar_wait_a(bempty0 + sb * 8, b_ph ^ 1);
-            if (elect_one()) {
-              mbar_expect_tx_a(bfull0 + sb * 8, Cfg::kBTile);
-              tma_load_2d_a(b_base + sb * Cfg::kBTile, &tmB, bfull0 + sb * 8, t * p.Cin + kc * CW,
-                            n0);
+      for (int u = 0; u < kUnits; ++u) {
+        for (int kc = 0; kc < nchunks; ++kc) {
+          mbar_wait_a(aempty0 + sa * 8, a_ph ^ 1);
+          if (elect_one()) {
+            mbar_expect_tx_a(afull0 + sa * 8, Cfg::kABytes);
+            tma_load_4d_tile_a(a_base + sa * Cfg::kAStage, &tmA, afull0 + sa * 8, kc * CW, w0 - 1,
+                               h0 - 1, img);
+          }
+          __syncwarp();
+          if (++sa == static_cast<uint32_t>(AS)) { sa = 0; a_ph ^= 1; }
+          if (!kPh && !p.stationary) {
+            for (int t = 0; t < 9; ++t) {
+              mbar_wait_a(bempty0 + sb * 8, b_ph ^ 1);
+              if (elect_one()) {
+                mbar_expect_tx_a(bfull0 + sb * 8, Cfg::kBTile);
+                tma_load_2d_a(b_base + sb * Cfg::kBTile, &tmB, bfull0 + sb * 8, t * p.Cin + kc * CW,
+                              n0);
+              }
+              __syncwarp();
+              if (++sb == static_cast<uint32_t>(NB)) { sb = 0; b_ph ^= 1; }
             }
-            __syncwarp();
-            if (++sb == static_cast<uint32_t>(NB)) { sb = 0; b_ph ^= 1; }
           }
         }
       }
@@ -604,7 +629,7 @@
     const int cg = (warp >> 2) - 1;
     const int ct = static_cast<int>(threadIdx.x) - 128;
     const bool leader = ct == 0;
-    const bool stats = p.ch_part != nullptr;
+    const bool stats = !kPh && p.ch_part != nullptr;
     const bool has_aux = p.has_add || p.has_mask;
     const int r0 = cg * 64 + (warp & 3) * 16 + (lane >> 2);
     const int cq = (lane & 3) * 2;
@@ -620,18 +645,6 @@
 #pragma unroll
     for (int e = 0; e < 8; ++e) acc_s[e] = acc_q[e] = 0.f;
     uint32_t aux_n = 0;
-    auto issue_aux = [&](int img, int h0, int w0) {
-      mbar_expect_tx(&aux_bar, (p.has_add ? Cfg::kTileBytes : 0) + (p.has_mask ? Cfg::kTileBytes : 0));
-#pragma unroll
-      for (int sub = 0; sub < kNSub; ++sub) {
-        if (p.has_add)
-          tma_load_4d_tile_a(smem_u32(s_add + sub * kSubBytes), &tmAdd, smem_u32(&aux_bar),
-                             n0 + sub * kSubW, w0, h0, img);
-        if (p.has_mask)
-          tma_load_4d_tile_a(smem_u32(s_mask + sub * kSubBytes), &tmMask, smem_u32(&aux_bar),
-                             n0 + sub * kSubW, w0, h0, img);
-      }
-    };
     int pend_a = -1, pend_b = -1;
     auto release_pending = [&]() {
       __syncwarp();
@@ -642,100 +655,235 @@
       pend_a = pend_b = -1;
     };
     PatchIter pi(m_first, m_step, p.ph, p.pw);
-    if (leader && has_aux && my_tiles > 0) issue_aux(pi.img, pi.row * kPatchH, pi.col * kPatchW);
-    if (p.stationary && my_tiles > 0) mbar_wait_a(bfull0, 0);
-    uint32_t sa = 0, a_ph = 0, sb = 0, b_ph = 0;
-    for (int it = 0; it < my_tiles; ++it) {
-      const int img = pi.img, h0 = pi.row * kPatchH, w0 = pi.col * kPatchW;
-      pi.next();
-      for (int kc = 0; kc < nchunks; ++kc) {
-        mbar_wait_a(afull0 + sa * 8, a_ph);
-        const uint64_t a_st = a_desc0 + ((sa * Cfg::kAStage) >> 4);
-        if (p.stationary) {
-          wgmma_fence_operand(acc);
-          wgmma_fence();
-          const uint64_t b_st = b_desc0 + ((static_cast<uint32_t>(kc) * 9 * Cfg::kBTile) >> 4);
-#pragma unroll
-          for (int t = 0; t < 9; ++t)
-#pragma unroll
-            for (int ks = 0; ks < kKSteps; ++ks)
-              Wgmma<BN>::template mma<0, 0>(
-                  acc, a_st + ((((t / 3) * kHaloW + (t % 3)) * kRowB + ks * 32) >> 4),
-                  b_st + ((t * Cfg::kBTile + ks * 32) >> 4), (t | ks) ? 1u : static_cast<uint32_t>(kc != 0));
-          wgmma_commit();
-          wgmma_fence_operand(acc);
-          wgmma_wait<1>();
+    if constexpr (kPh) {
+      float accs[kG][BN / 2];
+      auto issue_aux = [&](int img, int h0, int w0, int u) {
+        mbar_expect_tx(&aux_bar, kG * ((p.has_add ? Cfg::kTileBytes : 0) +
+                                       (p.has_mask ? Cfg::kTileBytes : 0)));
+#pragma unroll
+        for (int g = 0; g < kG; ++g) {
+          const int ph = u * kG + g;
+#pragma unroll
+          for (int sub = 0; sub < kNSub; ++sub) {
+            const int c = (ph & 1) * p.Cout + n0 + sub * kSubW;
+            const int off = g * Cfg::kTileBytes + sub * kSubBytes;
+            if (p.has_add)
+              tma_load_5d_tile_a(smem_u32(s_add + off), &tmAdd, smem_u32(&aux_bar), c, w0, ph >> 1,
+                                 h0, img);
+            if (p.has_mask)
+              tma_load_5d_tile_a(smem_u32(s_mask + off), &tmMask, smem_u32(&aux_bar), c, w0,
+                                 ph >> 1, h0, img);
+          }
+        }
+      };
+      auto mma_phase = [&](auto ph_c, float(&acc)[BN / 2], uint64_t a_st, uint64_t b_st,
+                           uint32_t acc0) {
+        constexpr int kP = decltype(ph_c)::value;
+#pragma unroll
+        for (int t = 0; t < phase_ntaps(kP); ++t)
+#pragma unroll
+          for (int ks = 0; ks < kKSteps; ++ks)
+            Wgmma<BN>::template mma<0, 0>(
+                acc, a_st + ((phase_tap_shift(kP, t) * kRowB + ks * 32) >> 4),
+                b_st + ((phase_tap_k(kP, t) * Cfg::kBTile + ks * 32) >> 4),
+                (t | ks) ? 1u : acc0);
+      };
+      auto mma_unit = [&](auto u_c, uint64_t a_st, uint64_t b_st, uint32_t acc0) {
+        constexpr int kU = decltype(u_c)::value;
+        mma_phase(std::integral_constant<int, kU * kG>{}, accs[0], a_st, b_st, acc0);
+        mma_phase(std::integral_constant<int, kU * kG + 1>{}, accs[1], a_st, b_st, acc0);
+        if constexpr (kG == 4) {
+          mma_phase(std::integral_constant<int, 2>{}, accs[2], a_st, b_st, acc0);
+          mma_phase(std::integral_constant<int, 3>{}, accs[3], a_st, b_st, acc0);
+        }
+      };
+      if (leader && has_aux && my_tiles > 0) issue_aux(pi.img, pi.row * kPatchH, pi.col * kPatchW, 0);
+      if (my_tiles > 0) mbar_wait_a(bfull0, 0);
+      uint32_t sa = 0, a_ph = 0;
+      for (int it = 0; it < my_tiles; ++it) {
+        const int img = pi.img, h0 = pi.row * kPatchH, w0 = pi.col * kPatchW;
+        pi.next();
+#pragma unroll 1
+        for (int u = 0; u < kUnits; ++u) {
+          for (int kc = 0; kc < nchunks; ++kc) {
+            mbar_wait_a(afull0 + sa * 8, a_ph);
+            const uint64_t a_st = a_desc0 + ((sa * Cfg::kAStage) >> 4);
+            const uint64_t b_st = b_desc0 + ((static_cast<uint32_t>(kc) * 9 * Cfg::kBTile) >> 4);
+            const uint32_t acc0 = static_cast<uint32_t>(kc != 0);
+#pragma unroll
+            for (int g = 0; g < kG; ++g) wgmma_fence_operand(accs[g]);
+            wgmma_fence();
+            if constexpr (kUnits == 1) {
+              mma_unit(std::integral_constant<int, 0>{}, a_st, b_st, acc0);
+            } else {
+              if (u == 0)
+                mma_unit(std::integral_constant<int, 0>{}, a_st, b_st, acc0);
+              else
+                mma_unit(std::integral_constant<int, 1>{}, a_st, b_st, acc0);
+            }
+            wgmma_commit();
+#pragma unroll
+            for (int g = 0; g < kG; ++g) wgmma_fence_operand(accs[g]);
+            wgmma_wait<1>();
+            release_pending();
+            pend_a = static_cast<int>(sa);
+            if (++sa == static_cast<uint32_t>(AS)) { sa = 0; a_ph ^= 1; }
+          }
+          wgmma_wait<0>();
+#pragma unroll
+          for (int g = 0; g < kG; ++g) wgmma_fence_operand(accs[g]);
           release_pending();
-          pend_a = static_cast<int>(sa);
-        } else {
-#pragma unroll 1
-          for (int t = 0; t < 9; ++t) {
-            mbar_wait_a(bfull0 + sb * 8, b_ph);
+
+          if (leader) tma_store_wait_read();
+          named_bar_sync(1, kConsumerThreads);
+          if (has_aux) {
+            mbar_wait(&aux_bar, aux_n & 1);
+            ++aux_n;
+          }
+#pragma unroll
+          for (int g = 0; g < kG; ++g) {
+#pragma unroll
+            for (int j = 0; j < BN / 8; ++j) {
+              const int c = j * 8 + cq;
+#pragma unroll
+              for (int h = 0; h < 2; ++h) {
+                const int r = r0 + h * 8;
+                float v0 = accs[g][j * 4 + h * 2], v1 = accs[g][j * 4 + h * 2 + 1];
+                const int off = g * Cfg::kTileBytes + staged_offset<kSubW>(r, c);
+                if (p.has_add) bf16x2_add(v0, v1, *reinterpret_cast<const uint32_t*>(s_add + off));
+                uint32_t pk = pack_bf16x2(v0, v1);
+                if (p.has_mask) pk &= bf16x2_gt0_mask(*reinterpret_cast<const uint32_t*>(s_mask + off));
+                *reinterpret_cast<uint32_t*>(s_out + off) = pk;
+              }
+            }
+          }
+          fence_proxy_async();
+          named_bar_sync(1, kConsumerThreads);
+          if (leader) {
+#pragma unroll
+            for (int g = 0; g < kG; ++g) {
+              const int ph = u * kG + g;
+#pragma unroll
+              for (int sub = 0; sub < kNSub; ++sub)
+                tma_store_5d(&tmC, s_out + g * Cfg::kTileBytes + sub * kSubBytes,
+                             (ph & 1) * p.Cout + n0 + sub * kSubW, w0, ph >> 1, h0, img);
+            }
+            tma_store_commit();
+            if (has_aux && u + 1 < kUnits)
+              issue_aux(img, h0, w0, u + 1);
+            else if (has_aux && it + 1 < my_tiles)
+              issue_aux(pi.img, pi.row * kPatchH, pi.col * kPatchW, 0);
+          }
+        }
+      }
+    } else {
+      auto issue_aux = [&](int img, int h0, int w0) {
+        mbar_expect_tx(&aux_bar, (p.has_add ? Cfg::kTileBytes : 0) + (p.has_mask ? Cfg::kTileBytes : 0));
+#pragma unroll
+        for (int sub = 0; sub < kNSub; ++sub) {
+          if (p.has_add)
+            tma_load_4d_tile_a(smem_u32(s_add + sub * kSubBytes), &tmAdd, smem_u32(&aux_bar),
+                               n0 + sub * kSubW, w0, h0, img);
+          if (p.has_mask)
+            tma_load_4d_tile_a(smem_u32(s_mask + sub * kSubBytes), &tmMask, smem_u32(&aux_bar),
+                               n0 + sub * kSubW, w0, h0, img);
+        }
+      };
+      if (leader && has_aux && my_tiles > 0) issue_aux(pi.img, pi.row * kPatchH, pi.col * kPatchW);
+      if (p.stationary && my_tiles > 0) mbar_wait_a(bfull0, 0);
+      uint32_t sa = 0, a_ph = 0, sb = 0, b_ph = 0;
+      for (int it = 0; it < my_tiles; ++it) {
+        const int img = pi.img, h0 = pi.row * kPatchH, w0 = pi.col * kPatchW;
+        pi.next();
+        for (int kc = 0; kc < nchunks; ++kc) {
+          mbar_wait_a(afull0 + sa * 8, a_ph);
+          const uint64_t a_st = a_desc0 + ((sa * Cfg::kAStage) >> 4);
+          if (p.stationary) {
             wgmma_fence_operand(acc);
             wgmma_fence();
-            const uint64_t a_tap = a_st + ((((t / 3) * kHaloW + (t % 3)) * kRowB) >> 4);
-            const uint64_t b_tap = b_desc0 + ((sb * Cfg::kBTile) >> 4);
-#pragma unroll
-            for (int ks = 0; ks < kKSteps; ++ks)
-              Wgmma<BN>::template mma<0, 0>(acc, a_tap + ((ks * 32) >> 4), b_tap + ((ks * 32) >> 4),
-                                            (kc | t | ks) ? 1u : 0u);
+            const uint64_t b_st = b_desc0 + ((static_cast<uint32_t>(kc) * 9 * Cfg::kBTile) >> 4);
+#pragma unroll
+            for (int t = 0; t < 9; ++t)
+#pragma unroll
+              for (int ks = 0; ks < kKSteps; ++ks)
+                Wgmma<BN>::template mma<0, 0>(
+                    acc, a_st + ((((t / 3) * kHaloW + (t % 3)) * kRowB + ks * 32) >> 4),
+                    b_st + ((t * Cfg::kBTile + ks * 32) >> 4), (t | ks) ? 1u : static_cast<uint32_t>(kc != 0));
             wgmma_commit();
             wgmma_fence_operand(acc);
             wgmma_wait<1>();
             release_pending();
-            pend_b = static_cast<int>(sb);
-            if (t == 8) pend_a = static_cast<int>(sa);
-            if (++sb == static_cast<uint32_t>(NB)) { sb = 0; b_ph ^= 1; }
-          }
-        }
-        if (++sa == static_cast<uint32_t>(AS)) { sa = 0; a_ph ^= 1; }
-      }
-      wgmma_wait<0>();
-      wgmma_fence_operand(acc);
-      release_pending();
-
-      if (leader) tma_store_wait_read();
-      named_bar_sync(1, kConsumerThreads);
-      if (has_aux) {
-        mbar_wait(&aux_bar, aux_n & 1);
-        ++aux_n;
-      }
-#pragma unroll
-      for (int j = 0; j < BN / 8; ++j) {
-        const int c = j * 8 + cq;
-#pragma unroll
-        for (int h = 0; h < 2; ++h) {
-          const int r = r0 + h * 8;
-          float v0 = acc[j * 4 + h * 2], v1 = acc[j * 4 + h * 2 + 1];
-          const int off = staged_offset<kSubW>(r, c);
-          if (p.has_add) bf16x2_add(v0, v1, *reinterpret_cast<const uint32_t*>(s_add + off));
-          uint32_t pk = pack_bf16x2(v0, v1);
-          if (p.has_mask) pk &= bf16x2_gt0_mask(*reinterpret_cast<const uint32_t*>(s_mask + off));
-          *reinterpret_cast<uint32_t*>(s_out + off) = pk;
-        }
-      }
-      fence_proxy_async();
-      named_bar_sync(1, kConsumerThreads);
-      if (leader) {
-#pragma unroll
-        for (int sub = 0; sub < kNSub; ++sub)
-          tma_store_4d(&tmC, s_out + sub * kSubBytes, n0 + sub * kSubW, w0, h0, img);
-        tma_store_commit();
-        if (has_aux && it + 1 < my_tiles) issue_aux(pi.img, pi.row * kPatchH, pi.col * kPatchW);
-      }
-      if (stats && st_on) {
-        constexpr int kRowBytes = kSubW * 2;
-        const int sub = st_chunk / (kSubW / 8), jj = st_chunk % (kSubW / 8);
+            pend_a = static_cast<int>(sa);
+          } else {
+#pragma unroll 1
+            for (int t = 0; t < 9; ++t) {
+              mbar_wait_a(bfull0 + sb * 8, b_ph);
+              wgmma_fence_operand(acc);
+              wgmma_fence();
+              const uint64_t a_tap = a_st + ((((t / 3) * kHaloW + (t % 3)) * kRowB) >> 4);
+              const uint64_t b_tap = b_desc0 + ((sb * Cfg::kBTile) >> 4);
+#pragma unroll
+              for (int ks = 0; ks < kKSteps; ++ks)
+                Wgmma<BN>::template mma<0, 0>(acc, a_tap + ((ks * 32) >> 4), b_tap + ((ks * 32) >> 4),
+                                              (kc | t | ks) ? 1u : 0u);
+              wgmma_commit();
+              wgmma_fence_operand(acc);
+              wgmma_wait<1>();
+              release_pending();
+              pend_b = static_cast<int>(sb);
+              if (t == 8) pend_a = static_cast<int>(sa);
+              if (++sb == static_cast<uint32_t>(NB)) { sb = 0; b_ph ^= 1; }
+            }
+          }
+          if (++sa == static_cast<uint32_t>(AS)) { sa = 0; a_ph ^= 1; }
+        }
+        wgmma_wait<0>();
+        wgmma_fence_operand(acc);
+        release_pending();
+
+        if (leader) tma_store_wait_read();
+        named_bar_sync(1, kConsumerThreads);
+        if (has_aux) {
+          mbar_wait(&aux_bar, aux_n & 1);
+          ++aux_n;
+        }
+#pragma unroll
+        for (int j = 0; j < BN / 8; ++j) {
+          const int c = j * 8 + cq;
+#pragma unroll
+          for (int h = 0; h < 2; ++h) {
+            const int r = r0 + h * 8;
+            float v0 = acc[j * 4 + h * 2], v1 = acc[j * 4 + h * 2 + 1];
+            const int off = staged_offset<kSubW>(r, c);
+            if (p.has_add) bf16x2_add(v0, v1, *reinterpret_cast<const uint32_t*>(s_add + off));
+            uint32_t pk = pack_bf16x2(v0, v1);
+            if (p.has_mask) pk &= bf16x2_gt0_mask(*reinterpret_cast<const uint32_t*>(s_mask + off));
+            *reinterpret_cast<uint32_t*>(s_out + off) = pk;
+          }
+        }
+        fence_proxy_async();
+        named_bar_sync(1, kConsumerThreads);
+        if (leader) {
+#pragma unroll
+          for (int sub = 0; sub < kNSub; ++sub)
+            tma_store_4d(&tmC, s_out + sub * kSubBytes, n0 + sub * kSubW, w0, h0, img);
+          tma_store_commit();
+          if (has_aux && it + 1 < my_tiles) issue_aux(pi.img, pi.row * kPatchH, pi.col * kPatchW);
+        }
+        if (stats && st_on) {
+          constexpr int kRowBytes = kSubW * 2;
+          const int sub = st_chunk / (kSubW / 8), jj = st_chunk % (kSubW / 8);
 #pragma unroll 4
-        for (int rr = st_rg; rr < kBM; rr += kNRg) {
-          if (h0 + (rr >> 3) >= p.H || w0 + (rr & 7) >= p.W) continue;
-          const int sw = (kRowBytes == 128) ? (rr & 7) : ((rr >> 1) & 3);
-          const uint4 u = *reinterpret_cast<const uint4*>(s_out + sub * kSubBytes + rr * kRowBytes +
-                                                          ((jj ^ sw) << 4));
-          const uint32_t w4[4] = {u.x, u.y, u.z, u.w};
-#pragma unroll
-          for (int e = 0; e < 4; ++e)
-            bf16x2_sum_sq(acc_s[2 * e], acc_q[2 * e], acc_s[2 * e + 1], acc_q[2 * e + 1], w4[e]);
+          for (int rr = st_rg; rr < kBM; rr += kNRg) {
+            if (h0 + (rr >> 3) >= p.H || w0 + (rr & 7) >= p.W) continue;
+            const int sw = (kRowBytes == 128) ? (rr & 7) : ((rr >> 1) & 3);
+            const uint4 u = *reinterpret_cast<const uint4*>(s_out + sub * kSubBytes + rr * kRowBytes +
+                                                            ((jj ^ sw) << 4));
+            const uint32_t w4[4] = {u.x, u.y, u.z, u.w};
+#pragma unroll
+            for (int e = 0; e < 4; ++e)
+              bf16x2_sum_sq(acc_s[2 * e], acc_q[2 * e], acc_s[2 * e + 1], acc_q[2 * e + 1], w4[e]);
+          }
         }
       }
     }
@@ -1113,19 +1261,22 @@
 
 static int g_conv_halo = 1;
 
-static int halo_bn(int Cout) { return Cout % 128 == 0 ? 128 : (Cout % 64 == 0 ? 64 : 32); }
+static int halo_bn(int Cout, bool phases = false) {
+  return Cout % 128 == 0 && !phases ? 128 : (Cout % 64 == 0 ? 64 : 32);
+}
 
 struct HaloPlan {
   int a_stages, b_slots, stationary, smem;
 };
 static int g_conv_halo_split = 1;
 
-static HaloPlan halo_plan(int bn, int cw, int Cin, bool has_add, bool has_mask) {
+static HaloPlan halo_plan(int bn, int cw, int Cin, bool has_add, bool has_mask,
+                          bool phases = false) {
   HaloPlan h;
   const int row_b = cw * 2;
   const int a_stage = (kHaloH * kHaloW * row_b + 1023) / 1024 * 1024;
   const int b_tile = bn * row_b;
-  const int tile = kBM * bn * 2;
+  const int tile = kBM * bn * 2 * (phases ? 128 / bn : 1);
   const int nchunks = Cin / cw;
   const int fixed = 1024 + tile * (1 + (has_add ? 1 : 0) + (has_mask ? 1 : 0));
   h.a_stages = 3;
@@ -1145,7 +1296,7 @@
 }
 
 static bool use_halo(const acnn_conv_geom& g, int np, bool out_f32, bool has_bias, bool has_add,
-                     bool has_mask) {
+                     bool has_mask, bool phases = false) {
   if (g_conv_halo <= 0) return false;
   const bool applies = g.kh == 3 && g.kw == 3 && g.stride == 1 && g.pad_h_lo == 1 &&
                        g.pad_h_hi == 1 && g.pad_w_lo == 1 && g.pad_w_hi == 1 &&
@@ -1153,13 +1304,15 @@
                        !out_f32 && !has_bias && (g.Cin % 64 == 0 || g.Cin == 32) &&
                        g.Cout % 32 == 0;
   if (!applies) return false;
+  const HaloPlan h = halo_plan(halo_bn(g.Cout, phases), g.Cin % 64 == 0 ? 64 : 32, g.Cin, has_add,
+                               has_mask, phases);
+  if (phases && !h.stationary) return false;
   if (g_conv_halo >= 2) return true;
-  const HaloPlan h = halo_plan(halo_bn(g.Cout), g.Cin % 64 == 0 ? 64 : 32, g.Cin, has_add, has_mask);
   return h.stationary && g.H >= 56;
 }
 
-static int halo_per_n(const acnn_conv_geom& g) {
-  const int n_tiles = g.Cout / halo_bn(g.Cout);
+static int halo_per_n(const acnn_conv_geom& g, bool phases = false) {
+  const int n_tiles = g.Cout / halo_bn(g.Cout, phases);
   const int m_tiles = g.B * ceil_div(g.H, kPatchH) * ceil_div(g.W, kPatchW);
   int per_n = num_sms() / n_tiles;
   if (per_n < 1) per_n = 1;
@@ -1184,13 +1337,31 @@
   return ACNN_OK;
 }
 
-template <int BN, int CW>
+static int make_map_phases(CUtensorMap* m, const void* base, int C, int W, int H, int B, int box_c) {
+  cuuint64_t dims[5] = {(cuuint64_t)2 * C, (cuuint64_t)W / 2, 2, (cuuint64_t)H / 2, (cuuint64_t)B};
+  cuuint64_t strides[4] = {(cuuint64_t)2 * C * 2, (cuuint64_t)W * C * 2, (cuuint64_t)2 * W * C * 2,
+                           (cuuint64_t)H * W * C * 2};
+  cuuint32_t box[5] = {(cuuint32_t)box_c, (cuuint32_t)kPatchW, 1, (cuuint32_t)kPatchH, 1};
+  cuuint32_t estr[5] = {1, 1, 1, 1, 1};
+  CUresult r = g_encode_tiled(m, CU_TENSOR_MAP_DATA_TYPE_BFLOAT16, 5, const_cast<void*>(base), dims,
+                              strides, box, estr, CU_TENSOR_MAP_INTERLEAVE_NONE,
+                              swizzle_enum(box_c * 2), CU_TENSOR_MAP_L2_PROMOTION_L2_128B,
+                              CU_TENSOR_MAP_FLOAT_OOB_FILL_NONE);
+  if (r != CUDA_SUCCESS) {
+    set_error("cuTensorMapEncodeTiled (phases) failed (%d): C=%d W=%d H=%d B=%d box_c=%d", (int)r,
+              C, W, H, B, box_c);
+    return ACNN_ERR_CUDA;
+  }
+  return ACNN_OK;
+}
+
+template <int BN, int CW, bool kPh>
 static int launch_conv_halo(const acnn_conv_geom& g, const void* x, const void* w, void* y,
                             float* ch_part, const void* add_src, const void* mask_src,
                             cudaStream_t stream) {
   using Cfg = HaloCfg<BN, CW>;
   static bool attr_set = false;
-  auto kern = conv_halo_kernel<BN, CW>;
+  auto kern = conv_halo_kernel<BN, CW, kPh>;
   if (!attr_set) {
     cudaError_t e = cudaFuncSetAttribute(kern, cudaFuncAttributeMaxDynamicSharedMemorySize,
                                          kSmemBudget + 2048);
@@ -1209,45 +1380,50 @@
   p.ch_part = ch_part;
   p.has_add = add_src != nullptr;
   p.has_mask = mask_src != nullptr;
-  const HaloPlan hp = halo_plan(BN, CW, g.Cin, p.has_add != 0, p.has_mask != 0);
+  const HaloPlan hp = halo_plan(BN, CW, g.Cin, p.has_add != 0, p.has_mask != 0, kPh);
   p.a_stages = hp.a_stages;
   p.b_slots = hp.b_slots;
   p.stationary = hp.stationary;
   ACNN_REQUIRE(p.b_slots >= 2, "conv (halo): shared memory does not fit");
+  ACNN_REQUIRE(!kPh || (!ch_part && p.stationary),
+               "conv (halo): the stride-2 dgrad needs stationary weights and has no statistics");
   const int smem = hp.smem;
   CUtensorMap tmA, tmB, tmC, tmAdd, tmMask;
+  auto out_map = [&](CUtensorMap* m, const void* base) {
+    return kPh ? make_map_phases(m, base, g.Cout, 2 * g.W, 2 * g.H, g.B, Cfg::kSubW)
+               : make_map_4d(m, base, g.Cout, g.W, g.H, g.B, Cfg::kSubW, kPatchW, kPatchH);
+  };
   int rc = make_map_4d(&tmA, x, g.Cin, g.W, g.H, g.B, CW, kHaloW, kHaloH);
   if (rc) return rc;
   if ((rc = make_map_2d(&tmB, w, g.Cout, 9 * g.Cin, 9 * g.Cin, BN, CW))) return rc;
-  if ((rc = make_map_4d(&tmC, y, g.Cout, g.W, g.H, g.B, Cfg::kSubW, kPatchW, kPatchH))) return rc;
+  if ((rc = out_map(&tmC, y))) return rc;
   tmAdd = tmMask = tmC;
-  if (add_src && (rc = make_map_4d(&tmAdd, add_src, g.Cout, g.W, g.H, g.B, Cfg::kSubW, kPatchW,
-                                   kPatchH)))
-    return rc;
-  if (mask_src && (rc = make_map_4d(&tmMask, mask_src, g.Cout, g.W, g.H, g.B, Cfg::kSubW, kPatchW,
-                                    kPatchH)))
-    return rc;
-  launch_k(kern, dim3(halo_per_n(g) * p.n_tiles), dim3(kThreads), smem, stream, tmA, tmB, tmC,
+  if (add_src && (rc = out_map(&tmAdd, add_src))) return rc;
+  if (mask_src && (rc = out_map(&tmMask, mask_src))) return rc;
+  launch_k(kern, dim3(halo_per_n(g, kPh) * p.n_tiles), dim3(kThreads), smem, stream, tmA, tmB, tmC,
            tmAdd, tmMask, p);
   count_launch();
   return check_launch("conv_halo_kernel");
 }
 
+template <bool kPh>
 static int conv_halo_host(const acnn_conv_geom& g, const void* x, const void* w, void* y,
                           float* ch_part, const void* add_src, const void* mask_src,
                           cudaStream_t stream) {
-  const int bn = halo_bn(g.Cout);
+  const int bn = halo_bn(g.Cout, kPh);
   const bool c64 = g.Cin % 64 == 0;
-  if (bn == 128) {
-    return c64 ? launch_conv_halo<128, 64>(g, x, w, y, ch_part, add_src, mask_src, stream)
-               : launch_conv_halo<128, 32>(g, x, w, y, ch_part, add_src, mask_src, stream);
+  if constexpr (!kPh) {
+    if (bn == 128) {
+      return c64 ? launch_conv_halo<128, 64, kPh>(g, x, w, y, ch_part, add_src, mask_src, stream)
+                 : launch_conv_halo<128, 32, kPh>(g, x, w, y, ch_part, add_src, mask_src, stream);
+    }
   }
   if (bn == 64) {
-    return c64 ? launch_conv_halo<64, 64>(g, x, w, y, ch_part, add_src, mask_src, stream)
-               : launch_conv_halo<64, 32>(g, x, w, y, ch_part, add_src, mask_src, stream);
-  }
-  return c64 ? launch_conv_halo<32, 64>(g, x, w, y, ch_part, add_src, mask_src, stream)
-             : launch_conv_halo<32, 32>(g, x, w, y, ch_part, add_src, mask_src, stream);
+    return c64 ? launch_conv_halo<64, 64, kPh>(g, x, w, y, ch_part, add_src, mask_src, stream)
+               : launch_conv_halo<64, 32, kPh>(g, x, w, y, ch_part, add_src, mask_src, stream);
+  }
+  return c64 ? launch_conv_halo<32, 64, kPh>(g, x, w, y, ch_part, add_src, mask_src, stream)
+             : launch_conv_halo<32, 32, kPh>(g, x, w, y, ch_part, add_src, mask_src, stream);
 }
 
 static int conv_gemm_host(const acnn_conv_geom& g, const void* x, const void* w, void* y,
@@ -1271,7 +1447,7 @@
   if (rc) return rc;
   if (use_halo(g, precision ? 3 : 1, out_f32 != 0, bias != nullptr, add_src != nullptr,
                mask_src != nullptr))
-    return conv_halo_host(g, x, w, y, ch_part, add_src, mask_src, stream);
+    return conv_halo_host<false>(g, x, w, y, ch_part, add_src, mask_src, stream);
   const bool plain = is_plain(g);
   const int cw = chunk_width(g.Cin);
   const int np = precision ? 3 : 1;
@@ -1533,6 +1709,66 @@
   return dispatch_wgrad<true>(w.bn, cw, cwb, np, tm, p, w.m_tiles, w.n_tiles, stream);
 }
 
+static acnn_conv_geom dgrad_geom(const acnn_conv_geom& g) {
+  acnn_conv_geom t;
+  t.B = g.B;
+  t.H = g.H + g.pad_h_lo + g.pad_h_hi - g.kh + 1;
+  t.W = g.W + g.pad_w_lo + g.pad_w_hi - g.kw + 1;
+  t.Cin = g.Cout;
+  t.Cout = g.Cin;
+  t.kh = g.kh;
+  t.kw = g.kw;
+  t.stride = 1;
+  t.pad_h_lo = g.kh - 1 - g.pad_h_lo;
+  t.pad_h_hi = g.kh - 1 - g.pad_h_hi;
+  t.pad_w_lo = g.kw - 1 - g.pad_w_lo;
+  t.pad_w_hi = g.kw - 1 - g.pad_w_hi;
+  t.x_pix_stride = t.x_row_pitch = t.x_img_pitch = t.reserved_ = 0;
+  return t;
+}
+
+static int conv_dgrad_host(const acnn_conv_geom& g, const void* dy, const void* w, void* dx,
+                           const void* add_src, const void* mask_src, int precision,
+                           int64_t w_plane_stride, cudaStream_t stream) {
+  if (g.stride == 1)
+    return conv_gemm_host(dgrad_geom(g), dy, w, dx, nullptr, add_src, mask_src, nullptr,
+                          precision ? 1 : 0, precision, w_plane_stride, stream);
+  int Ho, Wo;
+  ACNN_REQUIRE(out_hw(g, &Ho, &Wo), "conv_dgrad: empty output");
+  ACNN_REQUIRE(g.Cout % 8 == 0, "conv_dgrad: Cout=%d must be a multiple of 8", g.Cout);
+  acnn_conv_geom g1 = g;
+  g1.stride = 1;
+  g1.pad_h_hi = g.kh - 1 - g.pad_h_lo;
+  g1.pad_w_hi = g.kw - 1 - g.pad_w_lo;
+  const acnn_conv_geom t = dgrad_geom(g1);
+  if (g.kh == 3 && g.kw == 3 && g.pad_h_lo == 1 && g.pad_w_lo == 1 && g.H % 2 == 0 &&
+      g.W % 2 == 0 && 2 * Ho == g.H && 2 * Wo == g.W) {
+    acnn_conv_geom tp = t;
+    tp.H = Ho;
+    tp.W = Wo;
+    if (use_halo(tp, precision ? 3 : 1, precision != 0, false, add_src != nullptr,
+                 mask_src != nullptr, true)) {
+      const int rc = load_driver_fns();
+      if (rc) return rc;
+      return conv_halo_host<true>(tp, dy, w, dx, nullptr, add_src, mask_src, stream);
+    }
+  }
+  const int np = precision ? 3 : 1;
+  const int64_t n_dy = (int64_t)g.B * Ho * Wo * g.Cout, n_z = (int64_t)g.B * g.H * g.W * g.Cout;
+  void* dyz = nullptr;
+  int rc = scratch_alloc(&dyz, (size_t)(np * n_z * 2), stream, "conv_dgrad (stride 2)");
+  if (rc) return rc;
+  for (int pl = 0; pl < np && !rc; ++pl)
+    rc = acnn_zero_insert2x(static_cast<const uint16_t*>(dy) + pl * n_dy,
+                            static_cast<uint16_t*>(dyz) + pl * n_z, g.B, Ho, Wo, g.H, g.W, g.Cout,
+                            ACNN_BF16, stream);
+  if (!rc)
+    rc = conv_gemm_host(t, dyz, w, dx, nullptr, add_src, mask_src, nullptr, precision ? 1 : 0,
+                        precision, w_plane_stride, stream);
+  const int rf = scratch_free(dyz, stream, "conv_dgrad (stride 2)");
+  return rc ? rc : rf;
+}
+
 }
 
 extern "C" {
@@ -1639,30 +1875,12 @@
     acnn::set_error("acnn_conv_dgrad: null argument");
     return ACNN_ERR_INVALID;
   }
-  if (g->stride != 1) {
-    acnn::set_error("acnn_conv_dgrad: stride %d (zero-insert dy first, then call with stride 1)",
-                    g->stride);
+  if (g->stride != 1 && g->stride != 2) {
+    acnn::set_error("acnn_conv_dgrad: stride %d", g->stride);
     return ACNN_ERR_UNSUPPORTED;
   }
-  const int Ho = g->H + g->pad_h_lo + g->pad_h_hi - g->kh + 1;
-  const int Wo = g->W + g->pad_w_lo + g->pad_w_hi - g->kw + 1;
-  acnn_conv_geom t;
-  t.B = g->B;
-  t.H = Ho;
-  t.W = Wo;
-  t.Cin = g->Cout;
-  t.Cout = g->Cin;
-  t.kh = g->kh;
-  t.kw = g->kw;
-  t.stride = 1;
-  t.pad_h_lo = g->kh - 1 - g->pad_h_lo;
-  t.pad_h_hi = g->kh - 1 - g->pad_h_hi;
-  t.pad_w_lo = g->kw - 1 - g->pad_w_lo;
-  t.pad_w_hi = g->kw - 1 - g->pad_w_hi;
-  t.x_pix_stride = t.x_row_pitch = t.x_img_pitch = t.reserved_ = 0;
-  return acnn::conv_gemm_host(t, dy, w_dgrad, dx, nullptr, add_src, mask_src, nullptr,
-                              precision ? 1 : 0, precision, w_plane_stride,
-                              static_cast<cudaStream_t>(stream));
+  return acnn::conv_dgrad_host(*g, dy, w_dgrad, dx, add_src, mask_src, precision, w_plane_stride,
+                               static_cast<cudaStream_t>(stream));
 }
 
 int acnn_conv_wgrad(const acnn_conv_geom* g, const void* x, const void* dy, float* dw,
diff --git a/assembled_cnn_b200/csrc/model_plan.cu b/assembled_cnn_b200/csrc/model_plan.cu
--- a/assembled_cnn_b200/csrc/model_plan.cu
+++ b/assembled_cnn_b200/csrc/model_plan.cu
@@ -425,7 +425,7 @@
                         {"geom", vgeom(g)}, {"w", vvar(co.w)}});
     if (!need_dgrad) return;
     const int w = co.w;
-    if (g.stride == 1) {
+    if (g.stride == 1 || !fp32_) {
       contribute(co.x, [=](int out, int add, int mask) { emit_dgrad(dy, w, out, g, add, mask, -1); });
       return;
     }
diff --git a/assembled_cnn_b200/csrc/ptx.cuh b/assembled_cnn_b200/csrc/ptx.cuh
--- a/assembled_cnn_b200/csrc/ptx.cuh
+++ b/assembled_cnn_b200/csrc/ptx.cuh
@@ -144,6 +144,24 @@
       "cp.async.bulk.tensor.4d.global.shared::cta.tile.bulk_group [%0, {%2, %3, %4, %5}], [%1];\n" ::"l"(
           reinterpret_cast<uint64_t>(m)),
       "r"(smem_u32(smem_src)), "r"(c), "r"(w), "r"(h), "r"(n)
+      : "memory");
+}
+
+__device__ __forceinline__ void tma_load_5d_tile_a(uint32_t smem_dst, const CUtensorMap* m,
+                                                   uint32_t bar, int32_t c0, int32_t c1, int32_t c2,
+                                                   int32_t c3, int32_t c4) {
+  asm volatile(
+      "cp.async.bulk.tensor.5d.shared::cluster.global.tile.mbarrier::complete_tx::bytes"
+      " [%0], [%1, {%3, %4, %5, %6, %7}], [%2];\n" ::"r"(smem_dst),
+      "l"(reinterpret_cast<uint64_t>(m)), "r"(bar), "r"(c0), "r"(c1), "r"(c2), "r"(c3), "r"(c4)
+      : "memory");
+}
+__device__ __forceinline__ void tma_store_5d(const CUtensorMap* m, const void* smem_src, int32_t c0,
+                                             int32_t c1, int32_t c2, int32_t c3, int32_t c4) {
+  asm volatile(
+      "cp.async.bulk.tensor.5d.global.shared::cta.tile.bulk_group [%0, {%2, %3, %4, %5, %6}], [%1];\n" ::"l"(
+          reinterpret_cast<uint64_t>(m)),
+      "r"(smem_u32(smem_src)), "r"(c0), "r"(c1), "r"(c2), "r"(c3), "r"(c4)
       : "memory");
 }
 
diff --git a/assembled_cnn_b200/plan.py b/assembled_cnn_b200/plan.py
--- a/assembled_cnn_b200/plan.py
+++ b/assembled_cnn_b200/plan.py
@@ -533,7 +533,7 @@
                   w=co.w)
         if not need_dgrad:
             return
-        if g.stride == 1:
+        if g.stride == 1 or not self.fp32:
             self.contribute(co.x, lambda out, add, mask: self.emit_dgrad(
                 dy, co.w, out, g, add, mask))
         else:
```
